# connortannahill/MM-ADMM

Measured on AMD Instinct MI355X. Metric: ADMM iterations/sec on 1M-node 2D mesh; achieved HBM GB/s in SpMV, higher is better.
Workload: dtype f64

## Files before the change

include/mmadmm.h:

```cpp
#ifndef MMADMM_H
#define MMADMM_H
#include <stdint.h>

#ifdef __cplusplus
extern "C" {
#endif

#define MMADMM_OK 0
#define MMADMM_ERR_INVALID 1
#define MMADMM_ERR_HIP 2
#define MMADMM_ERR_INVERTED 3
#define MMADMM_ERR_IO 4
#define MMADMM_ERR_RCCL 5
#define MMADMM_ERR_NOCONV 6
#define MMADMM_ERR_NONFINITE 7

#define MMADMM_BOUNDARY_FREE 0
#define MMADMM_BOUNDARY_FIXED 1
#define MMADMM_INTERIOR 2

typedef struct mmadmm_engine* mmadmm_handle;
typedef struct mmadmm_meshbuf* mmadmm_mesh;

typedef void (*mmadmm_monitor_fn)(int dim, const double* x, double* M_rowmajor, void* user);

typedef struct mmadmm_params {
  double dt;
  double tau;
  double rho;
  int grad_use;
  int device;
  int rank;
  int nranks;
  int partition;
} mmadmm_params;

typedef struct mmadmm_stats {
  long long steps;
  long long admm_iters;
  long long bfgs_iters;
  int max_bfgs;
  double last_primal;
  double last_dual;
  double t_prox_ms;
  double t_xupdate_ms;
  double t_step_ms;
  long long n_prox;
  long long n_xupdate;
  long long n_steps_timed;
  double prox_bytes;
  double xupdate_bytes;
  long long newton_iters;
  long long jacobians;
  long long cg_iters;
  double t_jac_ms;
  double t_solve_ms;
  double t_be_ms;
  long long regrids;
  long long regrid_rows;
  double regrid_gather_bytes;
  long long regrid_cand;
  long long regrid_fallbacks;
  int monitor_iso;
  double t_exchange_ms;
  long long n_exchange;
  double halo_send_bytes;
  double halo_recv_bytes;
  int interior_nodes;
  int overlap;
} mmadmm_stats;

int mmadmm_regrid(mmadmm_handle h, double t);
int mmadmm_set_regrid(mmadmm_handle h, int every_step);

int mmadmm_regrid_values(mmadmm_handle h, const double* M);
int mmadmm_regrid_values_device(mmadmm_handle h, const double* d_M, void* producer_stream);
int mmadmm_regrid_field(mmadmm_handle h, const double* u, double alpha);
int mmadmm_regrid_field_device(mmadmm_handle h, const double* d_u, double alpha, void* producer_stream);
int mmadmm_field_hessian(mmadmm_handle h, const double* u, double* H);
int mmadmm_field_hessian_device(mmadmm_handle h, const double* d_u, double* d_H, void* stream);
int mmadmm_get_device(mmadmm_handle h, const char* what, double* d_out, void* consumer_stream);
int mmadmm_field_monitor(int dim, int nP, const double* Xp, int nF, const int32_t* F, const double* u,
                         double alpha, double* H, double* M);

int mmadmm_regrid_field_huang(mmadmm_handle h, const double* u, double alpha, double* alpha_used);
int mmadmm_regrid_field_huang_device(mmadmm_handle h, const double* d_u, double alpha, void* producer_stream,
                                     double* alpha_used);
int mmadmm_field_solve_info(mmadmm_handle h, int* passes, int* syncs);
int mmadmm_field_monitor_huang(int dim, int nP, const double* Xp, int nF, const int32_t* F, const double* u,
                               double alpha, double* alpha_used, double* H, double* M);
int mmadmm_field_root(int n, int count, const double* d, double* out);

int mmadmm_regrid_fields(mmadmm_handle h, int C, const double* U, const double* w, double alpha);
int mmadmm_regrid_fields_device(mmadmm_handle h, int C, const double* d_U, const double* w, double alpha,
                                void* producer_stream);
int mmadmm_regrid_fields_huang(mmadmm_handle h, int C, const double* U, const double* w, double alpha,
                               double* alpha_used);
int mmadmm_regrid_fields_huang_device(mmadmm_handle h, int C, const double* d_U, const double* w, double alpha,
                                      void* producer_stream, double* alpha_used);
int mmadmm_field_hessians(mmadmm_handle h, int C, const double* U, const double* w, double* H, double* A);
int mmadmm_field_hessians_device(mmadmm_handle h, int C, const double* d_U, const double* w, double* d_H, double* d_A,
                                 void* stream);
int mmadmm_fields_monitor(int dim, int nP, const double* Xp, int nF, const int32_t* F, int C, const double* U,
                          const double* w, double alpha, int normalise, double* alpha_used, double* H, double* A,
                          double* M);

int mmadmm_transfer(mmadmm_handle h, const double* Xold, const double* Xnew, int C, const double* uold, double* unew,
                    int32_t* where, int* counts);
int mmadmm_transfer_device(mmadmm_handle h, const double* d_Xold, const double* d_Xnew, int C, const double* d_uold,
                           double* d_unew, int32_t* d_where, int* counts, void* stream);
int mmadmm_transfer_field(int dim, int nP, const double* Xold, int nF, const int32_t* F, const double* Xnew, int C,
                          const double* uold, double* unew, int32_t* where, int* counts);
int mmadmm_face_neighbours(int dim, int nP, int nF, const int32_t* F, int32_t* nbr);

#define MMADMM_QUALITY_IDENTITY 0
#define MMADMM_QUALITY_VALUES 1
#define MMADMM_QUALITY_LAST 2
int mmadmm_quality(mmadmm_handle h, const double* X, int source, const double* M, double* q, double* summary);
int mmadmm_quality_device(mmadmm_handle h, const double* d_X, int source, const double* d_M, double* d_q,
                          double* summary, void* stream);
int mmadmm_mesh_quality(int dim, int nP, const double* Xp, const double* Xc, int nF, const int32_t* F,
                        const double* Ehat, const double* M, double* q, double* summary);

const char* mmadmm_last_error(void);
int mmadmm_version(void);
int mmadmm_build_info(char* out, int len);

int mmadmm_builtin_monitor(int dim, int mon_type, mmadmm_monitor_fn* fn, void** user);
int mmadmm_monitor_grid(int dim, int nP, const double* Xp, mmadmm_monitor_fn fn, void* user, int* rows,
                        double* vals);

int mmadmm_mesh_reorient(int dim, int nP, const double* Xp, int nF, int32_t* F);

int mmadmm_create(int dim, int nP, const double* Xp, const double* Xc, int nF, const int32_t* F,
                  const int32_t* mask, const mmadmm_params* p, mmadmm_monitor_fn fn, void* user,
                  mmadmm_handle* out);
int mmadmm_step(mmadmm_handle h, int n_iters, double tol, double* Ih, int* admm_iters);
int mmadmm_euler_step(mmadmm_handle h, double* Ih);
int mmadmm_backward_euler_step(mmadmm_handle h, double dt, double tol, double* Ih, int* newton_iters);
int mmadmm_get_jacobian(mmadmm_handle h, long long* nnz, int32_t* ia, int32_t* ja, double* a);
int mmadmm_be_begin(mmadmm_handle h, double dt, double* Ih);
int mmadmm_be_residual(mmadmm_handle h, double dt, double* F, double* norm1, double* Ih);
int mmadmm_be_fsubjac(mmadmm_handle h, double* a);
int mmadmm_be_add(mmadmm_handle h, const double* dx);
int mmadmm_energy(mmadmm_handle h, double* E);
int mmadmm_done(mmadmm_handle h);
int mmadmm_get(mmadmm_handle h, const char* what, double* out);
int mmadmm_get_simplices(mmadmm_handle h, int32_t* F);
int mmadmm_sizes(mmadmm_handle h, int* nP, int* nF, int* grid_rows);
int mmadmm_set_timing(mmadmm_handle h, int on);
int mmadmm_stats_get(mmadmm_handle h, mmadmm_stats* s);
int mmadmm_stats_reset(mmadmm_handle h);
int mmadmm_options_get(mmadmm_handle h, char* buf, int cap);
int mmadmm_sync(mmadmm_handle h);
int mmadmm_destroy(mmadmm_handle h);

int mmadmm_mesh_rect(int dim, int nx, int ny, int nz, double xa, double xb, double ya, double yb,
                     double za, double zb, int btype, mmadmm_mesh* out);
int mmadmm_mesh_levelset2d(int nx, int ny, double xa, double xb, double ya, double yb, int btype,
                           int compact_mask, mmadmm_mesh* out);
int mmadmm_mesh_levelset3d(int nx, int ny, int nz, double xa, double xb, double ya, double yb, double za,
                           double zb, int btype, int compact_mask, mmadmm_mesh* out);
int mmadmm_mesh_shoulder(int dim, int nx, int ny, int nz, double xa, double xb, double ya, double yb, double za,
                         double zb, int btype, mmadmm_mesh* out);
int mmadmm_mesh_reference_points(mmadmm_mesh h, double* Xc);
int mmadmm_mesh_hexdisc(int N, double r, double cx, double cy, int btype, mmadmm_mesh* out);
int mmadmm_mesh_read(int dim, const char* tri, const char* pnts, const char* mask, mmadmm_mesh* out);
int mmadmm_mesh_sizes(mmadmm_mesh m, int* dim, int* nP, int* nF, int* mask_len);
int mmadmm_mesh_copy(mmadmm_mesh m, double* Xp, int32_t* F, int32_t* mask);
int mmadmm_mesh_free(mmadmm_mesh m);
int mmadmm_write_points(const char* path, int dim, int nP, const double* Xp);
int mmadmm_write_simplices(const char* path, int dim, int nF, const int32_t* F);

int mmadmm_debug_blockgrad(mmadmm_handle h, int s, const double* z, const double* dxpu, int flags,
                           double* out);

#define MMADMM_PART_RCB 0
#define MMADMM_PART_RANGES 1
#define MMADMM_UNIQUE_ID_BYTES 128
typedef struct mmadmm_comm_s* mmadmm_comm;
typedef struct mmadmm_plan_s* mmadmm_plan;
int mmadmm_layout_check(unsigned* host_word);
int mmadmm_comm_unique_id(void* out, int len);
int mmadmm_comm_create_rccl(int nranks, int rank, const void* uid, int device, mmadmm_comm* out);
int mmadmm_comm_create_rccl_timeout(int nranks, int rank, const void* uid, int device, double timeout_s,
                                    mmadmm_comm* out);
int mmadmm_comm_create_loopback(int nranks, mmadmm_comm* out);
typedef int (*mmadmm_allgather_fn)(void* user, const double* send, double* recv, long long count);
typedef int (*mmadmm_exchange_fn)(void* user, int npeers, const int* peer_rank, const double* send,
                                  const long long* send_off, const long long* send_count, double* recv,
                                  const long long* recv_off, const long long* recv_count);
int mmadmm_comm_create_host(int nranks, int rank, mmadmm_allgather_fn allgather, mmadmm_exchange_fn exchange,
                            void* user, mmadmm_comm* out);
int mmadmm_comm_destroy(mmadmm_comm c);
int mmadmm_comm_nranks(mmadmm_comm c, int* nranks);
int mmadmm_create_partitioned(int dim, int nP, const double* Xp, const double* Xc, int nF, const int32_t* F,
                              const int32_t* mask, const mmadmm_params* p, mmadmm_monitor_fn fn, void* user,
                              mmadmm_comm comm, mmadmm_handle* out);
int mmadmm_local_nodes(mmadmm_handle h, int* n_local, int32_t* global_ids);
int mmadmm_plan_create(int dim, int nP, const double* Xp, int nF, const int32_t* F, int nranks, int rank, int method,
                       mmadmm_plan* out);
int mmadmm_plan_sizes(mmadmm_plan h, int* nLocalNodes, int* nLocalSimplices, int* nSources, int* nSend, int* nRecv,
                      int* nPeers, int* nInterface);
int mmadmm_plan_get(mmadmm_plan h, int32_t* localNodes, int32_t* localSimplices, int32_t* incPtr, int32_t* incSrc,
                    int32_t* sendOff, int32_t* peers);
int mmadmm_plan_destroy(mmadmm_plan h);

int mmadmm_devmath(int op, int n, const double* in, double* out);

#ifdef __cplusplus
}
#endif
#endif
```

mm-admm_amd/csrc/host/engine.cpp:

```cpp
#include <algorithm>
#include <chrono>
#include <cmath>
#include <cstring>
#include <limits>
#include <memory>
#include <mutex>
#include <string>
#include <vector>

#include "../../../include/mmx_sparse.h"
#include "../kernels/admm_kernels.h"
#include "../kernels/field_kernels.h"
#include "../kernels/quality_kernels.h"
#include "../kernels/regrid_kernels.h"
#include "../kernels/transfer_kernels.h"
#include "comm.h"
#include "common.h"
#include "partition.h"
#include "transfer.h"
#include "xup_records.h"

#define MMX_SP(expr)                                                                     \
  do {                                                                                   \
    const int rc_ = (expr);                                                              \
    if (rc_ != MMADMM_OK) throw ::mmx::Error(rc_, std::string(#expr) + ": " + mmadmm_last_error()); \
  } while (0)

namespace mmx {

namespace {
thread_local std::string g_last_error;
}
void set_last_error(const std::string& msg) { g_last_error = msg; }


struct EngineBase {
  virtual ~EngineBase() = default;
  int dim = 2;
  virtual void step(int nIters, double tol, double* Ih, int* iters) = 0;
  virtual double eulerStep() = 0;
  virtual double backwardEulerStep(double dt, double tol, int* newton) = 0;
  virtual void jacobian(long long* nnz, int32_t* ia, int32_t* ja, double* a) = 0;
  virtual void newtonOp(int op, double dt, const double* in, double* out, double* sc) = 0;
  virtual double energy() = 0;
  virtual void done() = 0;
  virtual void get(const std::string& what, double* out) = 0;
  virtual void getSimplices(int32_t* F) = 0;
  virtual void localNodes(int* n, int32_t* ids) = 0;
  virtual void sizes(int* nP, int* nF, int* gridRows) = 0;
  virtual void setTiming(bool on) = 0;
  virtual void stats(mmadmm_stats* s) = 0;
  virtual void resetStats() = 0;
  virtual void sync() = 0;
  virtual void regrid(double t) = 0;
  virtual void setRegrid(bool on) = 0;
  virtual void regridFrom(int src, const double* p, bool onDevice, double alpha, void* stream) = 0;
  virtual void fieldHessian(const double* u, double* H, bool onDevice, void* stream) = 0;
  virtual void regridFromFields(int src, const double* U, int C, const double* w, bool onDevice, double alpha,
                                void* stream) = 0;
  virtual void fieldHessians(const double* U, int C, const double* w, double* H, double* A, bool onDevice,
                             void* stream) = 0;
  virtual double fieldAlphaUsed() const = 0;
  virtual void fieldSolveInfo(int* passes, int* syncs) const = 0;
  virtual void getDevice(const std::string& what, double* dOut, void* stream) = 0;
  virtual void transfer(const double* Xold, const double* Xnew, int C, const double* uold, double* unew, int32_t* where,
                        int* counts, bool onDevice, void* stream) = 0;
  virtual void quality(const double* X, int source, const double* M, double* q, double* summary, bool onDevice,
                       void* stream) = 0;
  virtual void debugBlockGrad(int s, const double* z, const double* dx, int flags, double* out) = 0;
  virtual std::string options() const = 0;
};

enum MonSource {
  kMonBuiltin7 = 0,
  kMonCallback = 1,
  kMonValues = 2,
  kMonField = 3,
  kMonFieldHuang = 4,
  kMonFields = 5,
  kMonFieldsHuang = 6
};

void reorient_simplices(int D, const double* Vp, int nF, int32_t* F) {
  for (int s = 0; s < nF; ++s) {
    double E[3][3] = {{0}};
    const int32_t* f = F + (size_t)s * (D + 1);
    for (int j = 0; j < D; ++j)
      for (int r = 0; r < D; ++r) E[r][j] = Vp[(size_t)f[j + 1] * D + r] - Vp[(size_t)f[0] * D + r];
    double det;
    if (D == 2) {
      det = E[0][0] * E[1][1] - E[1][0] * E[0][1];
    } else {
      const double h0 = E[0][0] * (E[1][1] * E[2][2] - E[1][2] * E[2][1]);
      const double h1 = E[0][1] * (E[1][0] * E[2][2] - E[1][2] * E[2][0]);
      const double h2 = E[0][2] * (E[1][0] * E[2][1] - E[1][1] * E[2][0]);
      det = h0 - h1 + h2;
    }
    if (det < 0) std::swap(F[(size_t)s * (D + 1) + 1], F[(size_t)s * (D + 1) + 2]);
  }
}

template <int D>
class Engine final : public EngineBase {
 public:
  static constexpr int K = D * (D + 1);

  Engine(int nP, const double* Xp, const double* Xc, int nF, const int32_t* F, const int32_t* mask,
         const mmadmm_params& p, mmadmm_monitor_fn fn, void* user, Comm* comm)
      : Fh_(orientedSimplices(nP, Xp, nF, F)),
        plan_(make_partition_plan(D, nP, Xp, nF, Fh_.data(), std::max(1, p.nranks), p.nranks > 1 ? p.rank : 0,
                                  p.partition)),
        knobs_(EngineKnobs::from_env(D, (int)plan_.localSimplices.size(), std::max(1, p.nranks))) {
    dim = D;
    prm_ = p;
    nranks_ = std::max(1, p.nranks);
    rank_ = nranks_ > 1 ? p.rank : 0;
    comm_ = comm;
    nP_ = (int)plan_.localNodes.size();
    nF_ = (int)plan_.localSimplices.size();
    maxBlocks_ = std::max<size_t>(4096, std::max((nF_ + 15) / 16, (nP_ + 255) / 256 + 16));
    knobs_.check_xup_sweep(maxBlocks_);
    if (nranks_ > 1 && !comm_) throw Error(MMADMM_ERR_INVALID, "partitioned engine needs a communicator");
    if (p.device >= 0) MMX_HIP(hipSetDevice(p.device));
    MMX_HIP(hipStreamCreateWithFlags(&st_, hipStreamNonBlocking));
    if (nranks_ > 1) {
      MMX_HIP(hipStreamCreateWithFlags(&st2_, hipStreamNonBlocking));
      MMX_HIP(hipEventCreateWithFlags(&evProx_, hipEventDisableTiming));
      MMX_HIP(hipEventCreateWithFlags(&evEx_, hipEventDisableTiming));
    }
    compMesh_ = (Xc != nullptr);
    std::vector<double> Vp(Xp, Xp + (size_t)nP * D);
    maskH_.assign(mask, mask + nP);
    build_monitor_grid(D, Vp.data(), nP, fn, user, grid_);
    monFn_ = fn;
    monUser_ = user;
    const double w = 0.5 * sqrt(p.rho);
    w_ = w;
    double Ehat[3][3] = {{0}};
    if (D == 2) {
      Ehat[0][0] = 1.0;
      Ehat[1][0] = 0.0;
      Ehat[0][1] = 1.0 / 2.0;
      Ehat[1][1] = sqrt(3) / 2.0;
    } else {
      const double v[3][3] = {{-2.0, 0.0, -2.0}, {0.0, -2.0, -2.0}, {-2.0, -2.0, 0.0}};
      for (int r = 0; r < 3; ++r)
        for (int c = 0; c < 3; ++c) Ehat[r][c] = v[r][c];
    }
    const double dFact = (D == 2) ? 2.0 : 6.0;
    const double s1 = pow((dFact / std::abs(hostDet(Ehat))), 1.0 / ((double)D));
    for (int r = 0; r < D; ++r)
      for (int c = 0; c < D; ++c) Ehat[r][c] *= s1;
    const double s2 = (double)pow(nF, 1.0 / D);
    for (int r = 0; r < D; ++r)
      for (int c = 0; c < D; ++c) Ehat[r][c] /= s2;
    for (int r = 0; r < D; ++r)
      for (int c = 0; c < D; ++c) EhatH_[r * D + c] = Ehat[r][c];
    const double d = (double)D, pp = 1.5;
    powd_ = pow(d, d * pp / 2.0);
    if (nranks_ > 1) {
      std::vector<std::vector<int>> owned(nranks_);
      for (int v = 0; v < nP; ++v) owned[plan_.nodeOwner[v]].push_back(v);
      size_t mx = 1;
      for (auto& o : owned) mx = std::max(mx, o.size());
      maxOwned_ = (int)mx;
      std::vector<int> all((size_t)nranks_ * mx, -1), mine;
      for (int q = 0; q < nranks_; ++q) std::copy(owned[q].begin(), owned[q].end(), all.begin() + (size_t)q * mx);
      for (int v : owned[rank_])
        mine.push_back((int)(std::lower_bound(plan_.localNodes.begin(), plan_.localNodes.end(), v) - plan_.localNodes.begin()));
      nOwned_ = (int)mine.size();
      ownAllGid_.upload(all.data(), all.size(), st_);
      ownAllGidH_ = all;
      ownLocal_.upload(mine.data(), std::max<size_t>(mine.size(), 1), st_);
      streamWait();
    }
    const int nl = nP_;
    std::vector<double> invdiag(nl);
    const double dtsq = p.dt * p.dt;
    for (int v = 0; v < nl; ++v) {
      double S = 0.0;
      for (int c = 0; c < plan_.valence[v]; ++c) S = (c == 0) ? (w * w) * 1.0 : S + (w * w) * 1.0;
      invdiag[v] = 1.0 / (p.tau + dtsq * S);
    }
    std::vector<uint8_t> sbits(nF_), interior(nl);
    for (int v = 0; v < nl; ++v) interior[v] = maskH_[plan_.localNodes[v]] == MMADMM_INTERIOR ? 1 : 0;
    for (int s = 0; s < nF_; ++s) {
      unsigned b = 0;
      for (int n = 0; n < D + 1; ++n) {
        const int t = maskH_[plan_.localNodes[plan_.Flocal[(size_t)s * (D + 1) + n]]];
        if (t == MMADMM_BOUNDARY_FIXED) b |= 1u << n;
        if (t != MMADMM_INTERIOR) b |= 1u << (4 + n);
      }
      sbits[s] = (uint8_t)b;
    }
    std::vector<double> Vl((size_t)nl * D), Vcl;
    for (int v = 0; v < nl; ++v)
      for (int c = 0; c < D; ++c) Vl[(size_t)v * D + c] = Vp[(size_t)plan_.localNodes[v] * D + c];
    if (compMesh_) {
      Vcl.resize((size_t)nl * D);
      for (int v = 0; v < nl; ++v)
        for (int c = 0; c < D; ++c) Vcl[(size_t)v * D + c] = Xc[(size_t)plan_.localNodes[v] * D + c];
    }
    F_.upload(plan_.Flocal.data(), plan_.Flocal.size(), st_);
    sbits_.upload(sbits.data(), sbits.size(), st_);
    interior_.upload(interior.data(), interior.size(), st_);
    incPtr_.upload(plan_.incPtr.data(), plan_.incPtr.size(), st_);
    incOff_.upload(plan_.incSrc.data(), plan_.incSrc.size(), st_);
    if (knobs_.tslot) tslot_.alloc(std::max<size_t>((size_t)nF_ * K, 1));
    {
      std::vector<long long> key(nl);
      for (int v = 0; v < nl; ++v) {
        long long k = (long long)nF_;
        for (int t = plan_.incPtr[v]; t < plan_.incPtr[v + 1]; ++t)
          if (plan_.incSrc[t] >= 0) k = std::min<long long>(k, plan_.incSrc[t] / K);
        key[v] = k;
      }
      std::vector<int32_t> inner, bound;
      for (int v = 0; v < nl; ++v) {
        bool remote = false;
        for (int t = plan_.incPtr[v]; t < plan_.incPtr[v + 1]; ++t) remote |= plan_.incSrc[t] < 0;
        (remote && knobs_.overlap ? bound : inner).push_back(v);
      }
      nInner_ = (int)inner.size();
      const bool slabs = knobs_.xupOrder;
      auto order = [&](std::vector<int32_t>& ord) {
        const int n = (int)ord.size();
        if (slabs) {
          const int n8 = ((n + 255) / 256 + 7) / 8 * 256;
          std::stable_sort(ord.begin(), ord.end(), [&](int a, int b) { return Vl[(size_t)a * D + 1] < Vl[(size_t)b * D + 1]; });
          for (int c = 0; c < 8; ++c) {
            const int lo = std::min(n, c * n8), hi = std::min(n, (c + 1) * n8);
            std::stable_sort(ord.begin() + lo, ord.begin() + hi, [&](int a, int b) { return key[a] < key[b]; });
          }
        } else {
          std::stable_sort(ord.begin(), ord.end(), [&](int a, int b) { return key[a] < key[b]; });
        }
      };
      order(inner);
      order(bound);
      std::vector<int32_t> ord(inner);
      ord.insert(ord.end(), bound.begin(), bound.end());
      nodeOrder_.upload(ord.data(), std::max<size_t>(ord.size(), 1), st_);
      XupRecords recs;
      if (knobs_.xupRec) {
        const int ch = std::max(D == 2 ? MMX_XU_CH2D : 8, knobs_.xupCh);
        recs = build_xup_records(nl, ord.data(), plan_.incPtr.data(), plan_.incSrc.data(), invdiag.data(), ch);
        xrec_.upload(recs.rec.data(), recs.rec.size(), st_);
        xinv_.upload(recs.invdiag.data(), recs.invdiag.size(), st_);
        xslot_.upload(recs.slot.data(), recs.slot.size(), st_);
        xslotStride_ = (int)recs.stride;
        xslotCh_ = ch;
        const int chs = D == 2 ? MMX_XU_CH2D : knobs_.xupCh;
        xupTail_ = 0;
        for (int v = 0; v < nl; ++v) xupTail_ += std::max(0, plan_.incPtr[v + 1] - plan_.incPtr[v] - chs);
      }
      streamWait();
    }
    invdiag_.upload(invdiag.data(), invdiag.size(), st_);
    if (compMesh_) Vc_.upload(Vcl.data(), Vcl.size(), st_);
    uploadGridCoords();
    gvals_.upload(grid_.vals.data(), grid_.vals.size(), st_);
    if (D == 3) {
      gpad_.alloc(gvals_.n / 9 * 10);
      launch_pad_rows(gvals_.p, (long long)(gvals_.n / 9), gpad_.p, st_);
    }
    updateIso();
    Vp_.upload(Vl.data(), Vl.size(), st_);
    x_.upload(Vl.data(), Vl.size(), st_);
    xPrev_.upload(Vl.data(), Vl.size(), st_);
    xBar_.upload(Vl.data(), Vl.size(), st_);
    if (nranks_ > 1) {
      expOff_.upload(plan_.sendOff.data(), std::max<size_t>(plan_.sendOff.size(), 1), st_);
      export_.alloc((size_t)std::max<size_t>(plan_.sendOff.size(), 1) * D);
      remote_.alloc((size_t)std::max(plan_.recvRows, 1) * D);
    }
    z_.alloc((size_t)nF_ * K * (kZUInterleaved ? 2 : 1));
    gcache_.alloc((size_t)nF_ * K);
    tieList_.alloc((size_t)nF_ / 16 + 1);
    tieCount_.alloc(3);
    MMX_HIP(hipMemsetAsync(tieCount_.p, 0, 3 * sizeof(unsigned), st_));
    if (!kZUInterleaved) u_.alloc((size_t)nF_ * K);
    gs_.alloc((size_t)nF_ * K);
    clearU();
    {
      const size_t nB = (size_t)((nF_ + 255) / 256) * 256 * K * K;
      B_.alloc(nB);
      MMX_HIP(hipMemsetAsync(B_.p, 0, nB * sizeof(double), st_));
      launch_bkinv_identity<D>(nF_, B_.p, st_);
      if (prox_double_buffered(D, knobs_.prox2dWave)) B2_.alloc(nB);
    }
    partA_.alloc(maxBlocks_ * kNumPartials);
    partB_.alloc(maxBlocks_ * kNumPartials);
    redScratch_.alloc((size_t)kRedSets * kRedSplit * kNumPartials);
    red_.scratch = redScratch_.p;
    red_.splitMin = knobs_.redSplitMin;
    resultsCap_ = 0;
    ensureResults(64);
    m_ = makeView();
    launch_gather_z<D>(m_, x_.p, z_.p, st_);
    streamWait();
    MMX_HIP(hipGetLastError());
  }

  ~Engine() override {
    if (rgHost_) (void)hipHostFree(rgHost_);
    if (fldStH_) (void)hipHostFree(fldStH_);
    if (qlRecH_) (void)hipHostFree(qlRecH_);
    if (rgnHost_) (void)hipHostFree(rgnHost_);
    if (jac_) (void)mmx_matrix_destroy(jac_);
    for (auto& e : evPool_) (void)hipEventDestroy(e);
    if (evSync_) (void)hipEventDestroy(evSync_);
    if (evIn_) (void)hipEventDestroy(evIn_);
    if (evOut_) (void)hipEventDestroy(evOut_);
    if (resH_) (void)hipHostFree(resH_);
    if (evProx_) (void)hipEventDestroy(evProx_);
    if (evEx_) (void)hipEventDestroy(evEx_);
    for (hipStream_t s : {st2_, st_})
      if (s) {
        staging_forget(s);
        (void)hipStreamDestroy(s);
      }
  }

  void step(int nIters, double tol, double* Ih, int* itersOut) override {
    if (nIters < 1) throw Error(MMADMM_ERR_INVALID, "step: nIters must be >= 1");
    if (regridEachStep_) regrid(stepsTaken_ * prm_.dt);
    ensureResults(nIters);
    const bool timing = timing_;
    hipEvent_t eStep0 = nullptr, eStep1 = nullptr;
    if (timing) {
      eStep0 = nextEvent();
      MMX_HIP(hipEventRecord(eStep0, st_));
    }
    const double dtOverTau = prm_.dt / prm_.tau;
    const bool fusePred = knobs_.zx && knobs_.fusePred && !knobs_.prox2dWave && !(prm_.grad_use || stepsTaken_ <= 2);
    if (prm_.grad_use || stepsTaken_ <= 2) {
      int nb = 0;
      launch_grad_simplex<D>(m_, x_.p, gs_.p, true, partA_.p, &nb, st_);
      exchange(1);
      launch_predict<D>(m_, knobs_, 0, gs_.p, x_.p, xPrev_.p, xBar_.p, dtOverTau, st_);
    } else if (!fusePred) {
      launch_predict<D>(m_, knobs_, 1, nullptr, x_.p, xPrev_.p, xBar_.p, dtOverTau, st_);
    }
    const double* zsrc = stepsTaken_ == 0 ? xPrev_.p : xBar_.p;
    const bool zFromX = knobs_.zx && !knobs_.prox2dWave;
    if (!stepTaken_) clearU();
    if (zFromX)
      m_.zx = zsrc;
    else
      launch_gather_z<D>(m_, zsrc, z_.p, st_);
    gcacheValid_ = false;
    if (!zFromX) m_.zx = nullptr;
    StepScalars sc{prm_.tau, prm_.dt * prm_.dt, w_, dtOverTau};
    int nbx = 0, nbp = 0;
    if (fusePred) {
      m_.predPrev = xPrev_.p;
      m_.predBar = xBar_.p;
    }
    PackZX pz;
    if (zFromX) {
      pz.F = F_.p;
      pz.zx = zsrc;
      if (fusePred) {
        pz.x = x_.p;
        pz.xPrev = xPrev_.p;
      }
    }
    xupdateHalo(sc, &nbx, false, false, pz);
    m_.predPrev = m_.predBar = nullptr;
    const bool early = tol >= 0;
    int done = 0;
    double primal = 0, dual = 0;
    const bool deferRed = !early && nIters <= kDeferMax;
    const size_t slice = maxBlocks_ * kNumPartials;
    if (deferRed && partA_.n < slice * nIters) partA_.alloc(slice * std::max(nIters, 10));
    int firstDeferred = 0;
    hipEvent_t prevEnd = nullptr;
    for (int i = 0; i < nIters; ++i) {
      hipEvent_t a0 = nullptr, a1 = nullptr, b1 = nullptr;
      if (timing) {
        a0 = prevEnd;
        if (!a0) {
          a0 = nextEvent();
          MMX_HIP(hipEventRecord(a0, st_));
        }
      }
      const bool firstProx = !hessComputed_;
      const bool swapB = prox_double_buffered(D, knobs_.prox2dWave) && hessComputed_;
      if (hessComputed_) {
        tiePar_ ^= 1;
        std::swap(m_.tieCount, m_.tieStale);
      }
      m_.gcSkip = (D == 2 && knobs_.gcSkip && !early && i == nIters - 1) ? 1 : 0;
      launch_prox<D>(m_, knobs_, !hessComputed_, gcacheValid_, early ? tol / 100 : 1e-3 / 100, x_.p, z_.p, uPtr(), B_.p,
                     swapB ? B2_.p : B_.p, partA_.p + (deferRed ? slice * i : 0), &nbp, st_);
      m_.zx = nullptr;
      if (swapB) std::swap(B_.p, B2_.p);
      gcacheValid_ = !m_.gcSkip;
      if (timing) {
        a1 = nextEvent();
        MMX_HIP(hipEventRecord(a1, st_));
      }
      hessComputed_ = true;
      stepTaken_ = true;
      const bool resid = early || i == nIters - 1;
      xupdateHalo(sc, &nbx, resid, true, PackZX{});
      if (timing) {
        b1 = nextEvent();
        MMX_HIP(hipEventRecord(b1, st_));
        timed_.push_back({a0, a1, b1});
      }
      prevEnd = b1;
      if (deferRed) {
        if (firstProx && i < nIters - 1) {
          prevEnd = nullptr;
          launch_reduce_partials(partA_.p + slice * i, nbp, res_ + (size_t)i * 2 * kNumPartials, st_, red_);
          firstDeferred = i + 1;
        } else if (i == nIters - 1) {
          const int i0 = firstProx ? i : firstDeferred;
          launch_reduce_steps(partA_.p + slice * i0, slice, nbp, partB_.p, nbx, nIters - i0,
                              res_ + (size_t)i0 * 2 * kNumPartials, st_, red_);
        }
      } else if (resid) {
        prevEnd = nullptr;
        launch_reduce_partials2(partA_.p, nbp, res_ + (size_t)i * 2 * kNumPartials, partB_.p, nbx,
                                res_ + (size_t)i * 2 * kNumPartials + kNumPartials, st_, red_);
      } else {
        prevEnd = nullptr;
        launch_reduce_partials(partA_.p, nbp, res_ + (size_t)i * 2 * kNumPartials, st_, red_);
      }
      done = i + 1;
      if (early) {
        std::vector<double> rv;
        fetchResults(res_ + (size_t)i * 2 * kNumPartials, 1, rv);
        const double* r = rv.data();
        primal = sqrt(r[kNumPartials + 2]);
        dual = sqrt(r[1]);
        if (r[4] > 0 || (primal < tol && dual < tol)) break;
      }
    }
    MMX_HIP(hipMemcpyAsync(Vp_.p, x_.p, (size_t)nP_ * D * sizeof(double), hipMemcpyDeviceToDevice, st_));
    vpVersion_++;
    if (timing) {
      eStep1 = nextEvent();
      MMX_HIP(hipEventRecord(eStep1, st_));
    }
    fetchResults(res_, done, hostRes_);
    MMX_HIP(hipGetLastError());
    bool bad = false;
    long long bf = 0;
    int mx = 0;
    for (int i = 0; i < done; ++i) {
      const double* r = &hostRes_[(size_t)i * 2 * kNumPartials];
      bad |= r[4] > 0;
      bf += (long long)r[3];
      mx = std::max(mx, (int)r[5]);
    }
#ifdef MMX_HINT_PROBE
    {
      double hits = 0;
      for (int i = 0; i < done; ++i) hits += hostRes_[(size_t)i * 2 * kNumPartials + 2];
      fprintf(stderr, "[hint-probe] step %lld: %.0f hits of %.0f lookups in %d proxes\n", (long long)stepsTaken_, hits,
              3.0 * nF_ * done, done);
    }
#endif
    const double* last = &hostRes_[(size_t)(done - 1) * 2 * kNumPartials];
    primal = sqrt(last[kNumPartials + 2]);
    dual = sqrt(last[1]);
    st_stats_.admm_iters += done;
    st_stats_.bfgs_iters += bf;
    st_stats_.max_bfgs = mx;
    st_stats_.last_primal = primal;
    st_stats_.last_dual = dual;
    st_stats_.steps += 1;
    if (timing) {
      stepEv_.push_back({eStep0, eStep1});
      if (evUsed_ >= kEvResolve) resolveTimed();
    }
    stepsTaken_++;
    if (bad) throwBad("in prox");
    if (Ih) *Ih = hostRes_[0];
    if (itersOut) *itersOut = done;
  }

  double eulerStep() override {
    clearInvFlag();
    int nb = 0;
    launch_grad_simplex<D>(m_, x_.p, gs_.p, false, partA_.p, &nb, st_);
    launch_reduce_partials(partA_.p, nb, res_, st_, red_);
    exchange(1);
    launch_euler_apply<D>(m_, knobs_, gs_.p, x_.p, prm_.dt / prm_.tau, st_);
    std::vector<double> rv;
    fetchResults(res_, 1, rv);
    const double* r = rv.data();
    if (r[4] > 0) throwBad("in the explicit Euler gradient");
    return r[0];
  }

  double backwardEulerStep(double dtBE, double tol, int* newtonOut) override {
    if (nranks_ > 1) throw Error(MMADMM_ERR_INVALID, "backward Euler runs on one rank (no element partition)");
    const auto tStep = Clock::now();
    const int n = nP_ * D;
    ensureJacobian();
    const double dtot = dtBE / prm_.tau;
    const double SAFETY_FAC = 1.0 / 10.0;
    const int MAX_ITERS = 1000;
    clearInvFlag();
    MMX_HIP(hipMemcpyAsync(xn_.p, x_.p, (size_t)n * sizeof(double), hipMemcpyDeviceToDevice, st_));
    int nb = 0, nb2 = 0;
    launch_grad_simplex<D>(m_, x_.p, gs_.p, false, partA_.p, &nb, st_);
    launch_euler_apply<D>(m_, knobs_, gs_.p, x_.p, dtot, st_);
    if (!beStepTaken_) buildJacobian(dtBE);
    int nIter = 0;
    double Ih = 0.0, normPrev = INFINITY;
    std::vector<double> rv;
    void* mst = nullptr;
    MMX_SP(mmx_matrix_stream(jac_, &mst));
    do {
      launch_grad_simplex<D>(m_, x_.p, gs_.p, false, partA_.p, &nb, st_);
      launch_be_residual<D>(m_, knobs_, gs_.p, x_.p, xn_.p, dtot, rhs_.p, partB_.p, &nb2, st_);
      launch_reduce_partials2(partA_.p, nb, res_, partB_.p, nb2, res_ + kNumPartials, st_, red_);
      fetchResults(res_, 1, rv);
      if (rv[4] > 0) throwBad("in backward Euler");
      Ih = rv[0];
      const double norm = rv[kNumPartials];
      if (norm < SAFETY_FAC * tol) break;
      if (!beStepTaken_ || std::fabs(norm - normPrev) / norm < 0.25) {
        buildJacobian(dtBE);
        beStepTaken_ = true;
      }
      waitStream();
      const auto tSolve = Clock::now();
      MMX_SP(mmx_matrix_set_rhs_device(jac_, rhs_.p));
      int cgIter = 0;
      MMX_SP(mmx_matrix_solve_device(jac_, &jprm_, dx_.p, &cgIter, 0));
      st_stats_.t_solve_ms += msSince(tSolve);
      if (cgIter > 0) st_stats_.cg_iters += cgIter;
      if (cgIter <= 0)
        throw Error(MMADMM_ERR_NOCONV, "backward Euler: CG-STAB did not converge (reference: assert(cgIter > 0))");
      launch_add_inplace(n, x_.p, dx_.p, st_);
      nIter++;
      normPrev = norm;
    } while (nIter < MAX_ITERS);
    streamWait();
    st_stats_.steps += 1;
    st_stats_.newton_iters += nIter;
    st_stats_.t_be_ms += msSince(tStep);
    if (newtonOut) *newtonOut = nIter;
    return Ih;
  }

  void newtonOp(int op, double dt, const double* in, double* out, double* sc) override {
    if (nranks_ > 1) throw Error(MMADMM_ERR_INVALID, "backward Euler runs on one rank (no element partition)");
    ensureJacobian();
    const int n = nP_ * D;
    std::vector<double> rv;
    int nb = 0, nb2 = 0;
    if (op == 0 || op == 1) clearInvFlag();
    if (op == 0) {
      MMX_HIP(hipMemcpyAsync(xn_.p, x_.p, (size_t)n * sizeof(double), hipMemcpyDeviceToDevice, st_));
      launch_grad_simplex<D>(m_, x_.p, gs_.p, false, partA_.p, &nb, st_);
      launch_reduce_partials(partA_.p, nb, res_, st_, red_);
      launch_euler_apply<D>(m_, knobs_, gs_.p, x_.p, dt / prm_.tau, st_);
      fetchResults(res_, 1, rv);
      if (rv[4] > 0) throwBad("in backward Euler");
      if (sc) sc[0] = rv[0];
    } else if (op == 1) {
      launch_grad_simplex<D>(m_, x_.p, gs_.p, false, partA_.p, &nb, st_);
      launch_be_residual<D>(m_, knobs_, gs_.p, x_.p, xn_.p, dt / prm_.tau, rhs_.p, partB_.p, &nb2, st_);
      launch_reduce_partials2(partA_.p, nb, res_, partB_.p, nb2, res_ + kNumPartials, st_, red_);
      fetchResults(res_, 1, rv);
      if (rv[4] > 0) throwBad("in backward Euler");
      std::vector<double> r((size_t)n);
      MMX_HIP(hipMemcpyAsync(r.data(), rhs_.p, (size_t)n * sizeof(double), hipMemcpyDeviceToHost, st_));
      streamWait();
      for (int i = 0; i < n; ++i) out[i] = -r[i];
      if (sc) {
        sc[0] = rv[0];
        sc[1] = rv[kNumPartials];
      }
    } else if (op == 2) {
      const double h = 10.0 * sqrt(std::numeric_limits<double>::epsilon());
      launch_fd_jac<D>(m_, Vp_.p, h, dv_.p, st_, fdWork_.p);
      clearInvFlag();
      if (jraw_.n != jja_.n) jraw_.alloc(std::max<size_t>(jja_.n, 1));
      launch_jac_assemble<D>(m_, knobs_, jia_.p, jja_.p, dv_.p, 1.0, jraw_.p, st_, false, maxColNodes_);
      MMX_HIP(hipMemcpyAsync(out, jraw_.p, jja_.n * sizeof(double), hipMemcpyDeviceToHost, st_));
      streamWait();
    } else if (op == 3) {
      MMX_HIP(hipMemcpyAsync(dx_.p, in, (size_t)n * sizeof(double), hipMemcpyHostToDevice, st_));
      launch_add_inplace(n, x_.p, dx_.p, st_);
      streamWait();
    } else {
      throw Error(MMADMM_ERR_INVALID, "newtonOp: unknown op");
    }
  }

  void jacobian(long long* nnz, int32_t* ia, int32_t* ja, double* a) override {
    if (!jac_) throw Error(MMADMM_ERR_INVALID, "no Jacobian yet: run a backward Euler step first");
    if (nnz) *nnz = (long long)jja_.n;
    if (ia) MMX_HIP(hipMemcpyAsync(ia, jia_.p, jia_.n * sizeof(int32_t), hipMemcpyDeviceToHost, st_));
    if (ja) MMX_HIP(hipMemcpyAsync(ja, jja_.p, jja_.n * sizeof(int32_t), hipMemcpyDeviceToHost, st_));
    if (a) MMX_HIP(hipMemcpyAsync(a, jval_.p, jval_.n * sizeof(double), hipMemcpyDeviceToHost, st_));
    streamWait();
  }

  double energy() override {
    int nb = 0;
    launch_energy<D>(m_, Vp_.p, partA_.p, &nb, st_);
    clearInvFlag();
    launch_reduce_partials(partA_.p, nb, res_, st_, red_);
    std::vector<double> rv;
    fetchResults(res_, 1, rv);
    return rv[0];
  }

  void done() override {
    MMX_HIP(hipMemcpyAsync(Vp_.p, x_.p, (size_t)nP_ * D * sizeof(double), hipMemcpyDeviceToDevice, st_));
    vpVersion_++;
    streamWait();
  }

  void get(const std::string& what, double* out) override {
    const DevBuf<double>* b = nullptr;
    if (what == "x") b = &x_;
    else if (what == "xPrev") b = &xPrev_;
    else if (what == "xBar") b = &xBar_;
    else if (what == "z" || what == "u") {
      if (!kZUInterleaved) {
        b = what == "z" ? &z_ : &u_;
      } else {
        std::vector<double> h(z_.n);
        MMX_HIP(hipMemcpyAsync(h.data(), z_.p, z_.n * sizeof(double), hipMemcpyDeviceToHost, st_));
        streamWait();
        const int sh = what == "u" ? D : 0;
        for (int s = 0; s < nF_; ++s)
          for (int i = 0; i < K; ++i) out[(size_t)s * K + i] = h[(size_t)s * 2 * K + (i / D) * 2 * D + i % D + sh];
        return;
      }
    }
    else if (what == "points") b = &Vp_;
    else if (what == "hess") b = &B_;
    else if (what == "gs") b = &gs_;
    else if (what == "grid") {
      if (gridOnDevice_) {
        MMX_HIP(hipMemcpyAsync(out, gvals_.p, gvals_.n * sizeof(double), hipMemcpyDeviceToHost, st_));
        streamWait();
      } else {
        std::memcpy(out, grid_.vals.data(), grid_.vals.size() * sizeof(double));
      }
      return;
    } else if (what == "Ehat") {
      std::memcpy(out, EhatH_, D * D * sizeof(double));
      return;
    } else {
      throw Error(MMADMM_ERR_INVALID, "mmadmm_get: unknown field '" + what + "'");
    }
    if (b == &B_) {
      std::vector<double> h(b->n);
      MMX_HIP(hipMemcpyAsync(h.data(), b->p, b->n * sizeof(double), hipMemcpyDeviceToHost, st_));
      streamWait();
      for (int s = 0; s < nF_; ++s)
        for (int ij = 0; ij < K * K; ++ij) out[(size_t)s * K * K + ij] = h[bIndex(s, ij)];
      return;
    }
    MMX_HIP(hipMemcpyAsync(out, b->p, b->n * sizeof(double), hipMemcpyDeviceToHost, st_));
    streamWait();
  }

  static size_t bIndex(int s, int ij) {
    if (D == 3 && MMX_B3_PAIRS) return ((size_t)(s >> 6) * K * K + (ij & ~1)) * 64 + 2 * (s & 63) + (ij & 1);
    return ((size_t)(s >> 6) * K * K + ij) * 64 + (s & 63);
  }

  void getSimplices(int32_t* F) override {
    for (size_t i = 0; i < plan_.Flocal.size(); ++i) F[i] = plan_.localNodes[plan_.Flocal[i]];
  }

  void localNodes(int* n, int32_t* ids) override {
    if (n) *n = nP_;
    if (ids) std::memcpy(ids, plan_.localNodes.data(), plan_.localNodes.size() * sizeof(int32_t));
  }

  void sizes(int* nP, int* nF, int* gridRows) override {
    if (nP) *nP = nP_;
    if (nF) *nF = nF_;
    if (gridRows) *gridRows = (int)(grid_.vals.size() / (D * D));
  }

  void setTiming(bool on) override {
    resolveTimed();
    timing_ = on;
  }

  void stats(mmadmm_stats* s) override {
    resolveTimed();
    *s = st_stats_;
    const double nF = nF_, nP = nP_;
    const double ts = knobs_.tslot ? 1.0 : 0.0;
    s->prox_bytes = nF * (4.0 * (D + 1) + 1 + 8.0 * (2 * K + K * K) * 2 + 8.0 * K * 2 + ts * 8.0 * K) +
                    nP * 8.0 * D;
    const double ch = D == 2 ? MMX_XU_CH2D : knobs_.xupCh;
    const double fixed = knobs_.xupRec ? nP * (4.0 * kXupRecInts + 8.0 + 4.0 * ch) + 4.0 * (double)xupTail_
                                 : 4.0 * (nP + 1) + 4.0 * (D + 1) * nF + 8.0 * nP;
    s->xupdate_bytes = fixed + (16.0 - 8.0 * ts) * K * nF + 8.0 * D * nP * 2;
    s->monitor_iso = iso_ ? 1 : 0;
    s->halo_send_bytes = 8.0 * D * (double)plan_.sendOff.size();
    s->halo_recv_bytes = nranks_ > 1 ? 8.0 * D * (double)plan_.recvRows : 0.0;
    s->interior_nodes = nInner_;
    s->overlap = knobs_.overlap;
  }

  std::string options() const override { return knobs_.text(); }

  void resetStats() override {
    resolveTimed();
    const mmadmm_stats z{};
    st_stats_ = z;
  }

  void resolveTimed() {
    if (stepEv_.empty() && timed_.empty() && exEv_.empty()) return;
    streamWait();
    float ms = 0;
    for (auto& p : stepEv_) {
      MMX_HIP(hipEventElapsedTime(&ms, p.first, p.second));
      st_stats_.t_step_ms += ms;
      st_stats_.n_steps_timed += 1;
    }
    if (st2_) MMX_HIP(hipStreamSynchronize(st2_));
    for (auto& p : exEv_) {
      MMX_HIP(hipEventElapsedTime(&ms, p.first, p.second));
      st_stats_.t_exchange_ms += ms;
      st_stats_.n_exchange += 1;
    }
    exEv_.clear();
    for (auto& t : timed_) {
      MMX_HIP(hipEventElapsedTime(&ms, t.a0, t.a1));
      st_stats_.t_prox_ms += ms;
      st_stats_.n_prox += 1;
      MMX_HIP(hipEventElapsedTime(&ms, t.a1, t.b1));
      st_stats_.t_xupdate_ms += ms;
      st_stats_.n_xupdate += 1;
    }
    stepEv_.clear();
    timed_.clear();
    evUsed_ = 0;
  }

  void sync() override { streamWait(); }

  void debugBlockGrad(int s, const double* z, const double* dx, int flags, double* out) override {
    if (s < 0 || s >= nF_) throw Error(MMADMM_ERR_INVALID, "debug_blockgrad: simplex out of range");
    DevBuf<double> dz, ddx, dout;
    dz.upload(z, K, st_);
    ddx.upload(dx, K, st_);
    dout.alloc(K + 2);
    launch_debug_blockgrad<D>(m_, s, dz.p, ddx.p, dout.p, flags, st_);
    MMX_HIP(hipMemcpyAsync(out, dout.p, (K + 2) * sizeof(double), hipMemcpyDeviceToHost, st_));
    streamWait();
  }

 private:
  struct Timed {
    hipEvent_t a0, a1, b1;
  };

  void profMark(const char* what, std::chrono::steady_clock::time_point& t) const {
    if (!knobs_.schedProf) return;
    const auto now = std::chrono::steady_clock::now();
    fprintf(stderr, "[sched] engine %s %.3f s\n", what, std::chrono::duration<double>(now - t).count());
    t = now;
  }
  void ensureJacobian() {
    if (jac_) return;
    auto tp = std::chrono::steady_clock::now();
    const int n = nP_ * D;
    mmx_struc sp = nullptr;
    MMX_SP(mmx_struc_create(n, 0, &sp));
    std::vector<int32_t> ia(n + 1), ja;
    long long nnz = 0;
    int rc = mmx_struc_mesh_pattern(sp, D, (int)(Fh_.size() / (D + 1)), Fh_.data());
    if (rc == MMADMM_OK) rc = mmx_struc_pack(sp);
    if (rc == MMADMM_OK) rc = mmx_struc_get(sp, nullptr, &nnz, nullptr, nullptr);
    if (rc == MMADMM_OK) {
      ja.resize(nnz);
      rc = mmx_struc_get(sp, nullptr, &nnz, ia.data(), ja.data());
    }
    profMark("pattern", tp);
    int dev = prm_.device;
    if (dev < 0) MMX_HIP(hipGetDevice(&dev));
    if (rc == MMADMM_OK) rc = mmx_matrix_create_from_struc(dev, sp, &jac_);
    (void)mmx_struc_destroy(sp);
    profMark("matrix create", tp);
    if (rc != MMADMM_OK) throw Error(rc, std::string("backward Euler Jacobian: ") + mmadmm_last_error());
    mmx_param_iter_mesh(&jprm_);
    maxColNodes_ = 0;
    for (int r = 0; r < n; ++r) maxColNodes_ = std::max(maxColNodes_, (ia[r + 1] - ia[r]) / D);
    jia_.upload(ia.data(), ia.size(), st_);
    jja_.upload(ja.data(), ja.size(), st_);
    jval_.alloc(std::max<size_t>(nnz, 1));
    dv_.alloc(std::max<size_t>((size_t)nF_ * (D + 1) * D * K, 1));
    if (knobs_.fdjFast) fdWork_.alloc((size_t)nF_ * (D + 1) + 1);
    xn_.alloc((size_t)n);
    rhs_.alloc((size_t)n);
    dx_.alloc((size_t)n);
    streamWait();
  }

  void buildJacobian(double dtBE) {
    if (jacVp_ == vpVersion_ && jacDt_ == dtBE) return;
    jacVp_ = vpVersion_;
    jacDt_ = dtBE;
    const auto t0 = Clock::now();
    auto tp = t0;
    const double h = 10.0 * sqrt(std::numeric_limits<double>::epsilon());
    launch_fd_jac<D>(m_, Vp_.p, h, dv_.p, st_, fdWork_.p);
    clearInvFlag();
    launch_jac_assemble<D>(m_, knobs_, jia_.p, jja_.p, dv_.p, dtBE / prm_.tau, jval_.p, st_, true, maxColNodes_);
    streamWait();
    profMark("FD Jacobian + assembly", tp);
    MMX_SP(mmx_matrix_set_values_device(jac_, jval_.p));
    if (!jacFactored_) {
      MMX_SP(mmx_matrix_sfac(jac_, &jprm_));
      jacFactored_ = true;
      profMark("sfac", tp);
    }
    streamWait();
    st_stats_.jacobians += 1;
    st_stats_.t_jac_ms += msSince(t0);
  }
  using Clock = std::chrono::steady_clock;
  static double msSince(Clock::time_point t) {
    return std::chrono::duration<double, std::milli>(Clock::now() - t).count();
  }

  static double hostDet(const double (&a)[3][3]) {
    if (D == 2) return a[0][0] * a[1][1] - a[1][0] * a[0][1];
    const double h0 = a[0][0] * (a[1][1] * a[2][2] - a[1][2] * a[2][1]);
    const double h1 = a[0][1] * (a[1][0] * a[2][2] - a[1][2] * a[2][0]);
    const double h2 = a[0][2] * (a[1][0] * a[2][1] - a[1][1] * a[2][0]);
    return h0 - h1 + h2;
  }

  void exchange(int mode, const PackZX& pz = {}, hipStream_t st = nullptr) {
    if (nranks_ == 1) return;
    if (!st) st = st_;
    hipEvent_t e0 = nullptr, e1 = nullptr;
    if (timing_ && mode == 0) {
      e0 = nextEvent();
      MMX_HIP(hipEventRecord(e0, st));
    }
    launch_pack_export<D>(mode, (int)plan_.sendOff.size(), expOff_.p, z_.p, uPtr(), gs_.p, w_, export_.p, st, pz);
    comm_->exchange(rank_, export_.p, remote_.p, plan_.peers, D, st);
    if (e0) {
      e1 = nextEvent();
      MMX_HIP(hipEventRecord(e1, st));
      exEv_.push_back({e0, e1});
    }
  }

  void xupdateHalo(const StepScalars& sc, int* nbx, bool resid, bool useTs, const PackZX& pz) {
    if (!knobs_.overlap) {
      exchange(0, pz);
      launch_xupdate<D>(m_, knobs_, sc, xBar_.p, z_.p, uPtr(), x_.p, partB_.p, nbx, resid, st_, useTs);
      return;
    }
    MMX_HIP(hipEventRecord(evProx_, st_));
    DeviceMesh<D> mi = m_;
    mi.xupHi = nInner_;
    int nb1 = 0, nb2 = 0;
    launch_xupdate<D>(mi, knobs_, sc, xBar_.p, z_.p, uPtr(), x_.p, partB_.p, &nb1, resid, st_, useTs);
    MMX_HIP(hipStreamWaitEvent(st2_, evProx_, 0));
    exchange(0, pz, st2_);
    MMX_HIP(hipEventRecord(evEx_, st2_));
    MMX_HIP(hipStreamWaitEvent(st_, evEx_, 0));
    DeviceMesh<D> mb = m_;
    mb.xupLo = nInner_;
    launch_xupdate<D>(mb, knobs_, sc, xBar_.p, z_.p, uPtr(), x_.p, partB_.p + (size_t)nb1 * kNumPartials, &nb2, resid,
                      st_, useTs);
    *nbx = nb1 + nb2;
  }

  void waitStream() {
    if (!knobs_.spin) {
      streamWait();
      return;
    }
    if (!evSync_) MMX_HIP(hipEventCreateWithFlags(&evSync_, hipEventDisableTiming));
    MMX_HIP(hipEventRecord(evSync_, st_));
    hipError_t r;
    while ((r = hipEventQuery(evSync_)) == hipErrorNotReady) __builtin_ia32_pause();
    MMX_HIP(r);
  }

  void streamWait() {
    if (nranks_ > 1 && comm_)
      comm_->wait(st_);
    else
      MMX_HIP(hipStreamSynchronize(st_));
  }

  void fetchResults(const double* dev, int rows, std::vector<double>& out) {
    const size_t cnt = (size_t)rows * 2 * kNumPartials;
    out.resize(cnt);
    if (resH_) {
      waitStream();
      std::memcpy(out.data(), resH_ + (dev - res_), cnt * sizeof(double));
      return;
    }
    if (nranks_ == 1) {
      MMX_HIP(hipMemcpyAsync(out.data(), dev, cnt * sizeof(double), hipMemcpyDeviceToHost, st_));
      streamWait();
      return;
    }
    if (resAll_.n < cnt * nranks_) resAll_.alloc(cnt * nranks_);
    comm_->allgather(rank_, dev, resAll_.p, cnt, st_);
    std::vector<double> all(cnt * nranks_);
    MMX_HIP(hipMemcpyAsync(all.data(), resAll_.p, all.size() * sizeof(double), hipMemcpyDeviceToHost, st_));
    streamWait();
    for (size_t i = 0; i < cnt; ++i) {
      const bool isMax = (i % kNumPartials) == 5;
      double v = all[i];
      for (int q = 1; q < nranks_; ++q) v = isMax ? std::max(v, all[(size_t)q * cnt + i]) : v + all[(size_t)q * cnt + i];
      out[i] = v;
    }
  }

  void setRegrid(bool on) override { regridEachStep_ = on; }

  void regrid(double t) override {
    if (nranks_ > 1) {
      const bool all = knobs_.regridGatherAll;
      if (!all && regridNear(t)) return;
      st_stats_.regrid_fallbacks += all ? 0 : 1;
    }
    regridAll(t);
  }

  void afterProducer(void* stream) {
    if (!stream) return;
    if (!evIn_) MMX_HIP(hipEventCreateWithFlags(&evIn_, hipEventDisableTiming));
    MMX_HIP(hipEventRecord(evIn_, (hipStream_t)stream));
    MMX_HIP(hipStreamWaitEvent(st_, evIn_, 0));
  }
  void beforeConsumer(void* stream) {
    if (!stream) {
      streamWait();
      return;
    }
    if (!evOut_) MMX_HIP(hipEventCreateWithFlags(&evOut_, hipEventDisableTiming));
    MMX_HIP(hipEventRecord(evOut_, st_));
    MMX_HIP(hipStreamWaitEvent((hipStream_t)stream, evOut_, 0));
  }
  void singleRankOnly(const char* what) const {
    if (nranks_ > 1) throw Error(MMADMM_ERR_INVALID, std::string(what) + ": single rank only (no element partition)");
  }
  void fieldScratch() {
    if (fldE_.p) return;
    fldE_.alloc(std::max<size_t>(field_ebuf_doubles<D>(nF_), 1));
    fldG_.alloc((size_t)nP_ * D);
  }
  void fieldsScratch(int C) {
    fieldScratch();
    if (fldGP_.n < (size_t)C * nP_ * D) fldGP_.alloc((size_t)C * nP_ * D);
  }
  void huangScratch() {
    if (fldA_.p) return;
    fldA_.alloc((size_t)nP_ * D * D);
    fldL_.alloc((size_t)nP_ * (D + 1));
    fldPart_.alloc((size_t)2 * field_solve_blocks(nP_));
    fldSt_.alloc(1);
    MMX_HIP(hipHostMalloc((void**)&fldStH_, sizeof(FieldSolve), hipHostMallocDefault));
  }
  void fieldHuangMonitor(const double* X) {
    fieldScratch();
    huangScratch();
    launch_field_huang_recover<D>(X, srcPtr_, F_.p, nF_, incPtr_.p, incOff_.p, nodeOrder_.p, nP_, fldE_.p, fldG_.p,
                                  fldA_.p, fldL_.p, st_);
    huangSolveAndFinish();
  }
  void fieldsHuangMonitor(const double* X) {
    fieldsScratch(srcC_);
    huangScratch();
    launch_fields_recover<D>(X, srcPtr_, srcC_, srcW_.data(), F_.p, nF_, incPtr_.p, incOff_.p, nodeOrder_.p, nP_,
                             fldE_.p, fldGP_.p, nullptr, fldA_.p, kFieldsHuang, 1.0, fldL_.p, st_);
    huangSolveAndFinish();
  }
  void huangSolveAndFinish() {
    launch_field_solve_set(fldSt_.p, srcAlpha_, st_);
    fldAlphaUsed_ = srcAlpha_;
    fldPasses_ = fldSyncs_ = 0;
    if (!(srcAlpha_ > 0.0)) {
      do {
        launch_field_solve_passes<D>(fldL_.p, nP_, fldSt_.p, fldPart_.p, kFieldBatch, st_);
        MMX_HIP(hipGetLastError());
        MMX_HIP(hipMemcpyAsync(fldStH_, fldSt_.p, sizeof(FieldSolve), hipMemcpyDeviceToHost, st_));
        streamWait();
        fldSyncs_++;
      } while (fldStH_->phase != kFieldDone);
      fldAlphaUsed_ = fldStH_->alpha;
      fldPasses_ = fldStH_->passes;
    }
    launch_field_huang_final<D>(fldA_.p, fldL_.p, nP_, fldSt_.p, rgMon_.p, st_);
  }
  double fieldAlphaUsed() const override { return fldAlphaUsed_; }
  void fieldSolveInfo(int* passes, int* syncs) const override {
    if (passes) *passes = fldPasses_;
    if (syncs) *syncs = fldSyncs_;
  }

  void regridFrom(int src, const double* p, bool onDevice, double alpha, void* stream) override {
    singleRankOnly(src == kMonFieldHuang ? "mmadmm_regrid_field_huang"
                   : src == kMonField    ? "mmadmm_regrid_field"
                                         : "mmadmm_regrid_values");
    const size_t n = (size_t)nP_ * (src == kMonValues ? D * D : 1);
    if (!onDevice) {
      if (fldIn_.n < n) fldIn_.alloc(n);
      MMX_HIP(hipMemcpyAsync(fldIn_.p, p, n * sizeof(double), hipMemcpyHostToDevice, st_));
      streamWait();
      p = fldIn_.p;
    } else {
      afterProducer(stream);
    }
    srcPtr_ = p;
    srcAlpha_ = alpha;
    regridAll(0.0, (MonSource)src);
    srcPtr_ = nullptr;
    if (onDevice && !knobs_.iso) streamWait();
  }

  void regridFromFields(int src, const double* U, int C, const double* w, bool onDevice, double alpha,
                        void* stream) override {
    singleRankOnly(src == kMonFieldsHuang ? "mmadmm_regrid_fields_huang" : "mmadmm_regrid_fields");
    const size_t n = (size_t)nP_ * C;
    if (!onDevice) {
      if (fldIn_.n < n) fldIn_.alloc(n);
      MMX_HIP(hipMemcpyAsync(fldIn_.p, U, n * sizeof(double), hipMemcpyHostToDevice, st_));
      streamWait();
      U = fldIn_.p;
    } else {
      afterProducer(stream);
    }
    srcPtr_ = U;
    srcAlpha_ = alpha;
    srcC_ = C;
    srcW_.assign(w, w + C);
    regridAll(0.0, (MonSource)src);
    srcPtr_ = nullptr;
    if (onDevice && !knobs_.iso) streamWait();
  }

  void fieldHessians(const double* U, int C, const double* w, double* H, double* A, bool onDevice,
// ... 448 lines not shown
    const int nbe = part ? std::max(1, std::min(256, (nF_ + 255) / 256)) : 0;
    double* extPart = rgPart_.p + (size_t)512 * 2 * D;
    if (part) {
      launch_rows_gather(D, ownLocal_.p, nOwned_, Vp_.p, rgSend_.p, st_);
      comm_->allgather(rank_, rgSend_.p, rgRecv_.p, (size_t)maxOwned_ * D, st_);
      launch_rows_scatter(D, ownAllGid_.p, nranks_ * maxOwned_, rgRecv_.p, rgXg_.p, st_);
      X = rgXg_.p;
      launch_bbox<D>(Vp_.p, nP_, rgPart_.p + (size_t)256 * 2 * D, nbl, st_);
      launch_extent<D>(Vp_.p, F_.p, nF_, extPart, nbe, st_);
    }
    launch_bbox<D>(X, nG, rgPart_.p, nb, st_);
    MMX_HIP(hipMemcpyAsync(rgHost_, rgPart_.p, sizeof(double) * nb * 2 * D, hipMemcpyDeviceToHost, st_));
    if (part) {
      MMX_HIP(hipMemcpyAsync(rgHost_ + (size_t)256 * 2 * D, rgPart_.p + (size_t)256 * 2 * D, sizeof(double) * nbl * 2 * D,
                             hipMemcpyDeviceToHost, st_));
      MMX_HIP(hipMemcpyAsync(rgHost_ + (size_t)512 * 2 * D, extPart, sizeof(double) * nbe * D, hipMemcpyDeviceToHost,
                             st_));
    }
    streamWait();
    double lo[3] = {INFINITY, INFINITY, INFINITY}, hi[3] = {-INFINITY, -INFINITY, -INFINITY};
    double llo[3] = {INFINITY, INFINITY, INFINITY}, lhi[3] = {-INFINITY, -INFINITY, -INFINITY};
    for (int b = 0; b < nb; ++b)
      for (int d = 0; d < D; ++d) {
        lo[d] = std::min(lo[d], rgHost_[(size_t)b * 2 * D + d]);
        hi[d] = std::max(hi[d], rgHost_[(size_t)b * 2 * D + D + d]);
      }
    for (int b = 0; b < nbl; ++b)
      for (int d = 0; d < D; ++d) {
        llo[d] = std::min(llo[d], rgHost_[(size_t)(256 + b) * 2 * D + d]);
        lhi[d] = std::max(lhi[d], rgHost_[(size_t)(256 + b) * 2 * D + D + d]);
      }
    if (part) {
      for (int d = 0; d < D; ++d) extMax_[d] = 0.0;
      for (int b = 0; b < nbe; ++b)
        for (int d = 0; d < D; ++d) extMax_[d] = std::max(extMax_[d], rgHost_[(size_t)512 * 2 * D + (size_t)b * D + d]);
    }
    grid_geometry(D, nG, lo, hi, grid_);
    uploadGridCoords();
    CellGrid cg{};
    const int gn[3] = {grid_.nx, grid_.ny, grid_.nz};
    cg.hmin = INFINITY;
    for (int d = 0; d < 3; ++d) {
      const double ext = d < D ? hi[d] - lo[d] : 0.0;
      cg.lo[d] = d < D ? lo[d] : 0.0;
      cg.n[d] = (d < D && ext > 0) ? std::max(1, gn[d] / 2) : 1;
      cg.inv[d] = (d < D && ext > 0) ? cg.n[d] / ext : 0.0;
      if (d < D && ext > 0) cg.hmin = std::min(cg.hmin, ext / cg.n[d]);
    }
    if (!(cg.hmin < INFINITY)) cg.hmin = 0.0;
    const int ncell = cg.n[0] * cg.n[1] * cg.n[2];
    if ((int)rgStarts_.n < ncell + 1) {
      rgCounts_.alloc(ncell + 1);
      rgStarts_.alloc(ncell + 1);
      rgFill_.alloc(ncell);
      rgScanBytes_ = bin_scan_bytes(ncell);
      rgScan_.alloc(std::max<size_t>(rgScanBytes_, 1));
    }
    launch_bin<D>(X, nG, cg, rgCellOf_.p, rgCounts_.p, rgStarts_.p, rgFill_.p, rgNodes_.p, rgScan_.p, rgScanBytes_,
                  st_);
    if (src == kMonCallback && builtin_monitor_kind(monFn_, monUser_) == 7) src = kMonBuiltin7;
    if (src == kMonValues) {
      MMX_HIP(hipMemcpyAsync(rgMon_.p, srcPtr_, (size_t)nG * DD * sizeof(double), hipMemcpyDeviceToDevice, st_));
    } else if (src == kMonField) {
      fieldScratch();
      launch_field_hessian<D>(X, srcPtr_, F_.p, nF_, incPtr_.p, incOff_.p, nodeOrder_.p, nP_, fldE_.p, fldG_.p,
                              srcAlpha_, nullptr, rgMon_.p, st_);
    } else if (src == kMonFieldHuang) {
      fieldHuangMonitor(X);
    } else if (src == kMonFields) {
      fieldsScratch(srcC_);
      launch_fields_recover<D>(X, srcPtr_, srcC_, srcW_.data(), F_.p, nF_, incPtr_.p, incOff_.p, nodeOrder_.p, nP_,
                               fldE_.p, fldGP_.p, nullptr, rgMon_.p, kFieldsPlain, srcAlpha_, nullptr, st_);
    } else if (src == kMonFieldsHuang) {
      fieldsHuangMonitor(X);
    } else if (src == kMonBuiltin7) {
      double c[3];
      moving_bump_centre(t, c);
      launch_monitor_tv<D>(X, nG, c, rgMon_.p, st_);
    } else {
      std::vector<double> Xh((size_t)nG * D), mv((size_t)nG * DD);
      MMX_HIP(hipMemcpyAsync(Xh.data(), X, Xh.size() * sizeof(double), hipMemcpyDeviceToHost, st_));
      streamWait();
      for (int v = 0; v < nG; ++v) {
        double M[9];
        for (int i = 0; i < DD; ++i) M[i] = 0.0;
        monFn_(D, &Xh[(size_t)v * D], M, monUser_);
        std::memcpy(&mv[(size_t)v * DD], M, DD * sizeof(double));
      }
      MMX_HIP(hipMemcpyAsync(rgMon_.p, mv.data(), mv.size() * sizeof(double), hipMemcpyHostToDevice, st_));
      streamWait();
    }
    const int passes = (D == 2) ? 5 : 2;
    const int gn3[3] = {grid_.nx, grid_.ny, D == 3 ? grid_.nz : 0};
    GridBox R{{0, 0, 0}, {gn3[0], gn3[1], gn3[2]}};
    if (part) {
      for (int d = 0; d < D; ++d) {
        const std::vector<double>& g = d == 0 ? grid_.gx : d == 1 ? grid_.gy : grid_.gz;
        const double h = g[1] - g[0];
        const int M = (int)std::ceil(2.0 * extMax_[d] / h) + 2;
        R.lo[d] = std::max(0, std::min(gn3[d], (int)std::floor((llo[d] - g[0]) / h) - M));
        R.hi[d] = std::max(0, std::min(gn3[d], (int)std::floor((lhi[d] - g[0]) / h) + 1 + M));
      }
    }
    auto widen = [&](const GridBox& b, int w) {
      GridBox o = b;
      for (int d = 0; d < D; ++d) {
        o.lo[d] = std::max(0, b.lo[d] - w);
        o.hi[d] = std::min(gn3[d], b.hi[d] + w);
      }
      return o;
    };
    const GridBox H = widen(R, part ? passes : 0);
    launch_nn_fill<D>(X, cg, rgStarts_.p, rgNodes_.p, gx_.p, gy_.p, D == 3 ? gz_.p : gy_.p, grid_.nx, grid_.ny,
                      grid_.nz, rgMon_.p, rgTmp_.p, H, st_);
    double* cur = rgTmp_.p;
    double* oth = part ? rgTmp2_.p : gvals_.p;
    for (int it = 0; it < passes; ++it) {
      launch_smooth<D>(cur, oth, grid_.nx, grid_.ny, grid_.nz, widen(R, part ? passes - 1 - it : 0), st_);
      std::swap(cur, oth);
    }
    if (part) {
      launch_box_commit<D>(cur, gvals_.p, D == 3 ? gpad_.p : nullptr, grid_.nx, grid_.ny, grid_.nz, R, st_);
    } else {
      if (cur != gvals_.p)
        MMX_HIP(hipMemcpyAsync(gvals_.p, cur, gvals_.n * sizeof(double), hipMemcpyDeviceToDevice, st_));
      if (D == 3) launch_pad_rows(gvals_.p, (long long)(gvals_.n / 9), gpad_.p, st_);
    }
    st_stats_.regrid_rows = (long long)(H.hi[0] - H.lo[0] + 1) * (H.hi[1] - H.lo[1] + 1) * (H.hi[2] - H.lo[2] + 1);
    st_stats_.regrid_gather_bytes = part ? (double)nranks_ * maxOwned_ * D * sizeof(double) : 0.0;
    st_stats_.regrid_cand = part ? nG : 0;
    MMX_HIP(hipGetLastError());
    gridOnDevice_ = true;
    updateIso();
    m_ = makeView();
    st_stats_.regrids += 1;
  }

  DeviceMesh<D> makeView() const {
    DeviceMesh<D> m{};
    m.nP = nP_;
    m.nF = nF_;
    m.F = F_.p;
    m.sbits = sbits_.p;
    m.nodeInterior = interior_.p;
    m.inc_ptr = incPtr_.p;
    m.inc_off = incOff_.p;
    m.remote = nranks_ > 1 ? remote_.p : nullptr;
    m.tslot = knobs_.tslot ? tslot_.p : nullptr;
    m.gcache = gcache_.p;
    m.tieList = tieList_.p;
    m.tieCount = tieCount_.p + tiePar_;
    m.tieStale = tieCount_.p + (tiePar_ ^ 1);
    m.invFlag = tieCount_.p + 2;
    m.nodeOrder = nodeOrder_.p;
    m.xupLo = 0;
    m.xupHi = nP_;
    m.prox2dWave = knobs_.prox2dWave;
    m.xupSweep = knobs_.xupSweep;
    m.xupCh = knobs_.xupCh;
    m.xupEarly = knobs_.xupEarly;
    m.forceTie = knobs_.forceTie;
    m.monHint = knobs_.monHint;
    if (knobs_.xupRec) {
      m.xrec = xrec_.p;
      m.xinv = xinv_.p;
      m.xslot = xslot_.p;
      m.xslotStride = xslotStride_;
      m.xslotCh = xslotCh_;
    }
    m.invdiag = invdiag_.p;
    m.Vc = compMesh_ ? Vc_.p : nullptr;
    m.gx = gx_.p;
    m.gy = gy_.p;
    m.gz = (D == 3) ? gz_.p : gy_.p;
    m.gvals = gvals_.p;
    m.gpad = (D == 3) ? gpad_.p : nullptr;
    for (int a = 0; a < 3; ++a) m.gcell[a] = (D == 3) ? gcell_[a].p : nullptr;
    m.giso = iso_ ? giso_.p : nullptr;
    m.gnx = grid_.nx;
    m.gny = grid_.ny;
    m.gnz = grid_.nz;
    m.ghx = grid_.gx[1] - grid_.gx[0];
    m.ghy = grid_.gy[1] - grid_.gy[0];
    m.ghz = (D == 3) ? grid_.gz[1] - grid_.gz[0] : 1.0;
    m.grhx = 1.0 / m.ghx;
    m.grhy = 1.0 / m.ghy;
    m.grhz = 1.0 / m.ghz;
    const int ns[3] = {grid_.nx, grid_.ny, grid_.nz};
    double* A[3] = {&m.gax, &m.gay, &m.gaz};
    double* SP[3] = {&m.gspx, &m.gspy, &m.gspz};
    double* NS[3] = {&m.gnsx, &m.gnsy, &m.gnsz};
    double* RNS[3] = {&m.grnsx, &m.grnsy, &m.grnsz};
    for (int d = 0; d < 3; ++d) {
      const bool on = d < D;
      *A[d] = on ? grid_.lo[d] : 0.0;
      *SP[d] = on ? grid_.hi[d] - grid_.lo[d] : 0.0;
      *NS[d] = on ? (double)ns[d] : 1.0;
      *RNS[d] = 1.0 / *NS[d];
    }
    for (int i = 0; i < D * D; ++i) m.Ehat[i] = EhatH_[i];
    m.powd = powd_;
    m.w = w_;
    m.compMesh = compMesh_ ? 1 : 0;
    return m;
  }

  void ensureResults(int nIters) {
    if (nIters <= resultsCap_) return;
    resultsCap_ = std::max(nIters, 64);
    const size_t n = (size_t)resultsCap_ * 2 * kNumPartials;
    if (nranks_ == 1 && knobs_.spin) {
      if (resH_) MMX_HIP(hipHostFree(resH_));
      resH_ = nullptr;
      MMX_HIP(hipHostMalloc((void**)&resH_, n * sizeof(double), hipHostMallocMapped));
      MMX_HIP(hipHostGetDevicePointer((void**)&res_, resH_, 0));
    } else {
      results_.alloc(n);
      res_ = results_.p;
    }
  }

  void clearInvFlag() { MMX_HIP(hipMemsetAsync(tieCount_.p + 2, 0, sizeof(unsigned), st_)); }

  [[noreturn]] void throwBad(const char* where) {
    unsigned flag = 0;
    MMX_HIP(hipMemcpyAsync(&flag, tieCount_.p + 2, sizeof(unsigned), hipMemcpyDeviceToHost, st_));
    streamWait();
    if (flag) {
      MMX_HIP(hipMemsetAsync(tieCount_.p + 2, 0, sizeof(unsigned), st_));
      streamWait();
      throw Error(MMADMM_ERR_INVERTED, std::string("inverted element ") + where + " (reference: assert(Edet > 0))");
    }
    if (nranks_ > 1 && regridEachStep_)
      throw Error(MMADMM_ERR_NONFINITE, std::string("non-finite energy ") + where +
                                            ": a monitor evaluation left this rank's regrid box (no element inverted)");
    throw Error(MMADMM_ERR_NONFINITE, std::string("non-finite energy ") + where +
                                          " without an inverted element (a monitor value that is not finite)");
  }

  hipEvent_t nextEvent() {
    if (evUsed_ == evPool_.size()) {
      hipEvent_t e;
      MMX_HIP(hipEventCreateWithFlags(&e, hipEventDisableSystemFence));
      evPool_.push_back(e);
    }
    return evPool_[evUsed_++];
  }

  static std::vector<int32_t> orientedSimplices(int nP, const double* Xp, int nF, const int32_t* F) {
    std::vector<int32_t> Fh(F, F + (size_t)nF * (D + 1));
    for (int32_t v : Fh)
      if (v < 0 || v >= nP) throw Error(MMADMM_ERR_INVALID, "simplex vertex id out of range");
    reorient_simplices(D, Xp, nF, Fh.data());
    return Fh;
  }

  std::vector<int32_t> Fh_;
  PartitionPlan plan_;
  const EngineKnobs knobs_;
  int nP_ = 0, nF_ = 0;
  mmadmm_params prm_{};
  bool compMesh_ = false;
  double w_ = 0, powd_ = 0;
  double EhatH_[9] = {0};
  std::vector<int32_t> maskH_;
  HostGrid grid_;
  mmadmm_monitor_fn monFn_ = nullptr;
  void* monUser_ = nullptr;
  bool regridEachStep_ = false, gridOnDevice_ = false;
  DevBuf<double> rgPart_, rgMon_, rgTmp_, rgTmp2_, rgXg_, rgSend_, rgRecv_;
  DevBuf<double> fldE_, fldG_, fldIn_, fldOut_;
  DevBuf<double> fldGP_;
  int srcC_ = 1;
  std::vector<double> srcW_;
  static constexpr int kFieldBatch = 64;
  DevBuf<double> fldA_, fldL_, fldPart_;
  DevBuf<FieldSolve> fldSt_;
  FieldSolve* fldStH_ = nullptr;
  double fldAlphaUsed_ = 1.0;
  int fldPasses_ = 0, fldSyncs_ = 0;
  std::vector<int32_t> trNbrH_;
  DevBuf<int32_t> trNbr_, trWhere_, trCnt_;
  DevBuf<double> trStage_;
  DevBuf<double> qlE_, qlC_, qlPart_, qlRec_, qlStage_;
  double* qlRecH_ = nullptr;
  const double* srcPtr_ = nullptr;
  double srcAlpha_ = 1.0;
  hipEvent_t evIn_ = nullptr, evOut_ = nullptr;
  double extMax_[3] = {0.0, 0.0, 0.0};
  DevBuf<int> ownLocal_, ownAllGid_;
  std::vector<int> ownAllGidH_, ownGidH_;
  DevBuf<double> rgnPart_, rgnSmallS_, rgnSmallR_, rgnSbox_, rgnSend_, rgnRecv_, rgnCandX_, rgnMon_;
  DevBuf<int> rgnCnt_, rgnGid_, rgnOwnGid_, rgnCandGid_, rgnCellOf_, rgnNodes_;
  double* rgnHost_ = nullptr;
  int nOwned_ = 0, maxOwned_ = 1;
  DevBuf<int> rgCellOf_, rgNodes_, rgCounts_, rgStarts_, rgFill_;
  DevBuf<unsigned char> rgScan_;
  size_t rgScanBytes_ = 0;
  double* rgHost_ = nullptr;
  hipStream_t st_ = nullptr;
  hipStream_t st2_ = nullptr;
  hipEvent_t evProx_ = nullptr, evEx_ = nullptr;
  int nInner_ = 0;
  std::vector<std::pair<hipEvent_t, hipEvent_t>> exEv_;
  DevBuf<int32_t> F_, incPtr_, incOff_;
  DevBuf<double> tslot_;
  DevBuf<uint8_t> sbits_, interior_;
  DevBuf<double> gcell_[3];
  DevBuf<double> giso_;
  DevBuf<int> isoFlag_;
  bool iso_ = false;
  std::vector<double> gcellH_[3];
  DevBuf<double> invdiag_, Vc_, gx_, gy_, gz_, gvals_, Vp_, x_, xPrev_, xBar_, z_, u_, gs_, B_, B2_, gcache_, gpad_;
  DevBuf<double> partA_, partB_, results_, export_, remote_, resAll_, redScratch_;
  RedWork red_;
  DevBuf<int32_t> expOff_, tieList_, nodeOrder_;
  DevBuf<int32_t> xrec_, xslot_;
  DevBuf<double> xinv_;
  int xslotStride_ = 0, xslotCh_ = 0;
  long long xupTail_ = 0;
  DevBuf<unsigned> tieCount_;
  int tiePar_ = 0;
  Comm* comm_ = nullptr;
  int rank_ = 0, nranks_ = 1;
  int resultsCap_ = 0;
  std::vector<double> hostRes_;
  DeviceMesh<D> m_{};
  bool hessComputed_ = false, stepTaken_ = false, gcacheValid_ = false;
  mmx_matrix jac_ = nullptr;
  mmx_param_iter jprm_{};
  bool beStepTaken_ = false, jacFactored_ = false;
  long long vpVersion_ = 0, jacVp_ = -1;
  double jacDt_ = 0.0;
  DevBuf<int32_t> jia_, jja_;
  DevBuf<double> jval_, jraw_, dv_, xn_, rhs_, dx_;
  DevBuf<unsigned> fdWork_;
  int maxColNodes_ = 65;
  int stepsTaken_ = 0;
  size_t maxBlocks_ = 1;
  static constexpr int kDeferMax = 64;
  bool timing_ = false;
  std::vector<hipEvent_t> evPool_;
  size_t evUsed_ = 0;
  static constexpr bool kZUInterleaved = (D == 2) && MMX_ZU_INTER;
  double* uPtr() const { return kZUInterleaved ? z_.p + D : u_.p; }
  void clearU() {
    if (kZUInterleaved)
      MMX_HIP(hipMemsetAsync(z_.p, 0, z_.n * sizeof(double), st_));
    else
      MMX_HIP(hipMemsetAsync(u_.p, 0, u_.n * sizeof(double), st_));
  }
  double* res_ = nullptr;
  double* resH_ = nullptr;
  hipEvent_t evSync_ = nullptr;
  std::vector<Timed> timed_;
  std::vector<std::pair<hipEvent_t, hipEvent_t>> stepEv_;
  static constexpr size_t kEvResolve = 4096;
  mmadmm_stats st_stats_{};
};

}

using mmx::EngineBase;
using mmx::Error;
using mmx::guarded;

struct mmadmm_engine {
  std::unique_ptr<EngineBase> e;
};

static EngineBase& eng(mmadmm_handle h) {
  if (!h || !h->e) throw Error(MMADMM_ERR_INVALID, "null engine handle");
  return *h->e;
}

extern "C" {

const char* mmadmm_last_error(void) { return mmx::g_last_error.c_str(); }
int mmadmm_version(void) { return 100; }

int mmadmm_mesh_reorient(int dim, int nP, const double* Xp, int nF, int32_t* F) {
  return guarded([&] {
    if ((dim != 2 && dim != 3) || nP < 1 || nF < 0 || !Xp || (nF > 0 && !F))
      throw Error(MMADMM_ERR_INVALID, "mmadmm_mesh_reorient: bad arguments");
    for (long long i = 0; i < (long long)nF * (dim + 1); ++i)
      if (F[i] < 0 || F[i] >= nP) throw Error(MMADMM_ERR_INVALID, "simplex vertex id out of range");
    mmx::reorient_simplices(dim, Xp, nF, F);
  });
}

int mmadmm_create(int dim, int nP, const double* Xp, const double* Xc, int nF, const int32_t* F, const int32_t* mask,
                  const mmadmm_params* p, mmadmm_monitor_fn fn, void* user, mmadmm_handle* out) {
  return guarded([&] {
    if (!out) throw Error(MMADMM_ERR_INVALID, "mmadmm_create: out is NULL");
    *out = nullptr;
    if ((dim != 2 && dim != 3) || nP < dim + 1 || nF < 1 || !Xp || !F || !mask || !p || !fn)
      throw Error(MMADMM_ERR_INVALID, "mmadmm_create: bad arguments");
    if (!(p->dt > 0) || !(p->tau > 0) || !(p->rho > 0))
      throw Error(MMADMM_ERR_INVALID, "mmadmm_create: dt, tau, rho must be positive");
    if (p->nranks > 1) throw Error(MMADMM_ERR_INVALID, "mmadmm_create: use mmadmm_create_partitioned for nranks > 1");
    mmx::check_kernel_layout(mmx::kLayoutWord);
    int ndev = 0;
    if (hipGetDeviceCount(&ndev) != hipSuccess || ndev == 0)
      throw Error(MMADMM_ERR_HIP, "mmadmm_create: no HIP device (the engine has no CPU fallback)");
    auto* h = new mmadmm_engine();
    try {
      if (dim == 2)
        h->e.reset(new mmx::Engine<2>(nP, Xp, Xc, nF, F, mask, *p, fn, user, nullptr));
      else
        h->e.reset(new mmx::Engine<3>(nP, Xp, Xc, nF, F, mask, *p, fn, user, nullptr));
    } catch (...) {
      delete h;
      throw;
    }
    *out = h;
  });
}

int mmadmm_create_partitioned(int dim, int nP, const double* Xp, const double* Xc, int nF, const int32_t* F,
                              const int32_t* mask, const mmadmm_params* p, mmadmm_monitor_fn fn, void* user,
                              mmadmm_comm comm, mmadmm_handle* out) {
  return guarded([&] {
    if (!out) throw Error(MMADMM_ERR_INVALID, "mmadmm_create_partitioned: out is NULL");
    *out = nullptr;
    if ((dim != 2 && dim != 3) || nP < dim + 1 || nF < 1 || !Xp || !F || !mask || !p || !fn)
      throw Error(MMADMM_ERR_INVALID, "mmadmm_create_partitioned: bad arguments");
    if (!(p->dt > 0) || !(p->tau > 0) || !(p->rho > 0))
      throw Error(MMADMM_ERR_INVALID, "mmadmm_create_partitioned: dt, tau, rho must be positive");
    if (p->nranks < 1 || p->rank < 0 || p->rank >= p->nranks)
      throw Error(MMADMM_ERR_INVALID, "mmadmm_create_partitioned: bad rank / nranks");
    mmx::Comm* c = mmx::comm_of(comm);
    if (p->nranks > 1 && (!c || c->nranks != p->nranks))
      throw Error(MMADMM_ERR_INVALID, "mmadmm_create_partitioned: communicator missing or of another size");
    mmx::check_kernel_layout(mmx::kLayoutWord);
    int ndev = 0;
    if (hipGetDeviceCount(&ndev) != hipSuccess || ndev == 0)
      throw Error(MMADMM_ERR_HIP, "mmadmm_create_partitioned: no HIP device (the engine has no CPU fallback)");
    auto* h = new mmadmm_engine();
    try {
      if (dim == 2)
        h->e.reset(new mmx::Engine<2>(nP, Xp, Xc, nF, F, mask, *p, fn, user, c));
      else
        h->e.reset(new mmx::Engine<3>(nP, Xp, Xc, nF, F, mask, *p, fn, user, c));
    } catch (...) {
      delete h;
      throw;
    }
    *out = h;
  });
}

int mmadmm_local_nodes(mmadmm_handle h, int* n_local, int32_t* global_ids) {
  return guarded([&] { eng(h).localNodes(n_local, global_ids); });
}

int mmadmm_step(mmadmm_handle h, int n_iters, double tol, double* Ih, int* admm_iters) {
  return guarded([&] { eng(h).step(n_iters, tol, Ih, admm_iters); });
}
int mmadmm_euler_step(mmadmm_handle h, double* Ih) {
  return guarded([&] {
    const double r = eng(h).eulerStep();
    if (Ih) *Ih = r;
  });
}
int mmadmm_backward_euler_step(mmadmm_handle h, double dt, double tol, double* Ih, int* newton_iters) {
  return guarded([&] {
    if (!(dt > 0)) throw mmx::Error(MMADMM_ERR_INVALID, "backward Euler: dt must be > 0");
    const double r = eng(h).backwardEulerStep(dt, tol, newton_iters);
    if (Ih) *Ih = r;
  });
}
int mmadmm_be_begin(mmadmm_handle h, double dt, double* Ih) {
  return guarded([&] {
    if (!(dt > 0)) throw mmx::Error(MMADMM_ERR_INVALID, "backward Euler: dt must be > 0");
    double sc[2] = {0.0, 0.0};
// ... 256 lines not shown
```

mm-admm_amd/csrc/host/knobs.h:

```cpp
#pragma once
#include <climits>
#include <cstdio>
#include <cstdlib>
#include <cstring>
#include <stdexcept>
#include <string>

namespace mmx {

constexpr int kTslot2dMax = 2 * 2048 * 64;
constexpr int kXupEarlyDefault = 1;
constexpr int kRedSplitMin = 4096;
constexpr int kProxBlock = 64;
constexpr int kSweepGrid = 128;
constexpr int kFacWaveChunk = 0;
constexpr int kChainImportLat = 8;
constexpr int kFacImpRows = 384;
constexpr int kFacRMax = 4;

inline int env_int(const char* name, int dflt, int lo = INT_MIN, int hi = INT_MAX) {
  const char* e = std::getenv(name);
  if (!e) return dflt;
  const int v = std::atoi(e);
  return v < lo ? lo : v > hi ? hi : v;
}
inline int env_flag(const char* name, bool dflt) { return env_int(name, dflt ? 1 : 0) != 0 ? 1 : 0; }
inline int env_word(const char* name, const char* words) {
  const char* e = std::getenv(name);
  if (!e) return 0;
  const size_t n = std::strlen(e);
  int i = 0;
  for (const char* w = words; *w; ++i) {
    const char* bar = std::strchr(w, '|');
    const size_t len = bar ? (size_t)(bar - w) : std::strlen(w);
    if (len == n && std::strncmp(w, e, n) == 0) return i;
    w += len + (bar ? 1 : 0);
  }
  return 0;
}
inline int env_set(const char* name) { return std::getenv(name) != nullptr ? 1 : 0; }
inline double env_double(const char* name, double dflt) {
  const char* e = std::getenv(name);
  return e ? std::atof(e) : dflt;
}

namespace knobs_detail {
inline int snap_xup_ch(int c) { return c >= 24 ? 24 : c >= 16 ? 16 : 8; }
inline int one_of3(int v, int a, int b, int c, int dflt) { return (v == a || v == b || v == c) ? v : dflt; }
inline int in_range_or(int v, int lo, int hi, int dflt) { return (v < lo || v > hi) ? dflt : v; }
inline void put(std::string& s, const char* name, const char* words, int v) {
  s += name;
  s += '=';
  if (!words) {
    s += std::to_string(v);
  } else {
    const char* w = words;
    for (int i = 0; i < v; ++i) w = std::strchr(w, '|') + 1;
    const char* bar = std::strchr(w, '|');
    s.append(w, bar ? (size_t)(bar - w) : std::strlen(w));
  }
  s += '\n';
}
inline void put(std::string& s, const char* name, const char*, double v) {
  char b[64];
  std::snprintf(b, sizeof b, "%.17g", v);
  s += name;
  s += '=';
  s += b;
  s += '\n';
}
inline int copy_out(const std::string& s, char* buf, int cap) {
  if (buf && cap > 0) {
    const size_t n = s.size() < (size_t)cap - 1 ? s.size() : (size_t)cap - 1;
    std::memcpy(buf, s.data(), n);
    buf[n] = 0;
  }
  return (int)s.size() + 1;
}
}

#define MMX_ENGINE_KNOBS(X) \
   \
   \
  X(int, tslot, "MMX_TSLOT", nullptr, env_flag("MMX_TSLOT", D == 3 || nF <= kTslot2dMax)) \
   \
  X(int, spin, "MMX_SPIN", nullptr, env_flag("MMX_SPIN", true)) \
   \
  X(int, zx, "MMX_ZX", nullptr, env_flag("MMX_ZX", true)) \
   \
  X(int, overlap, "MMX_OVERLAP", nullptr, nranks > 1 && env_flag("MMX_OVERLAP", true)) \
   \
  X(int, fusePred, "MMX_FUSE_PRED", nullptr, env_flag("MMX_FUSE_PRED", true)) \
   \
  X(int, gcSkip, "MMX_GC_SKIP", nullptr, env_flag("MMX_GC_SKIP", true)) \
   \
  X(int, xupOrder, "MMX_XUP_ORDER", nullptr, env_int("MMX_XUP_ORDER", D == 3) == 1) \
   \
  X(int, xupRec, "MMX_XUP_REC", nullptr, env_flag("MMX_XUP_REC", true)) \
   \
  X(int, xupCh, "MMX_XUP_CH", nullptr, knobs_detail::snap_xup_ch(env_int("MMX_XUP_CH", 8))) \
   \
   \
   \
  X(int, xupSweep, "MMX_XUP_SWEEP", nullptr, env_int("MMX_XUP_SWEEP", D == 3 ? 1 : (k.xupRec ? 2 : 0), 0)) \
   \
  X(int, xupEarly, "MMX_XUP_EARLY", nullptr, env_flag("MMX_XUP_EARLY", kXupEarlyDefault != 0)) \
   \
  X(int, xupSweepResid, "MMX_XUP_SWEEP_RESID", nullptr, env_flag("MMX_XUP_SWEEP_RESID", true)) \
   \
   \
  X(int, xcdMap, "MMX_XCD_MAP", nullptr, env_int("MMX_XCD_MAP", 1)) \
   \
  X(int, prox2dWave, "MMX_PROX2D", "lds|wave", D == 2 && env_word("MMX_PROX2D", "lds|wave")) \
   \
  X(int, prox3dQuad, "MMX_PROX3D", "wave|quad", env_word("MMX_PROX3D", "wave|quad")) \
   \
  X(int, proxBlock, "MMX_PROX_BLOCK", nullptr, knobs_detail::one_of3(env_int("MMX_PROX_BLOCK", 0), 64, 128, 256, kProxBlock)) \
   \
  X(int, gradCache, "MMX_GRAD_CACHE", nullptr, env_int("MMX_GRAD_CACHE", 1)) \
   \
  X(int, forceTie, "MMX_FORCE_TIE", nullptr, env_int("MMX_FORCE_TIE", 0)) \
   \
  X(int, monHint, "MMX_MON_HINT", nullptr, knobs_detail::in_range_or(env_int("MMX_MON_HINT", 1), 0, 3, 1)) \
   \
  X(int, iso, "MMX_ISO", nullptr, env_flag("MMX_ISO", true)) \
   \
  X(int, redSplitMin, "MMX_RED_SPLIT_MIN", nullptr, env_int("MMX_RED_SPLIT_MIN", kRedSplitMin)) \
   \
  X(int, regridGatherAll, "MMX_REGRID_GATHER", "near|all", env_word("MMX_REGRID_GATHER", "near|all")) \
   \
  X(double, regridMargin, "MMX_REGRID_MARGIN", nullptr, env_double("MMX_REGRID_MARGIN", 1.0)) \
   \
  X(int, fdjFast, "MMX_FDJ_FAST", nullptr, env_flag("MMX_FDJ_FAST", true)) \
   \
  X(int, jacAssembleEntry, "MMX_JAC_ASSEMBLE", "auto|entry", env_word("MMX_JAC_ASSEMBLE", "auto|entry")) \
   \
  X(int, schedProf, "MMX_SCHED_PROF", nullptr, env_set("MMX_SCHED_PROF"))

#define MMX_CHAIN_KNOBS(X) \
   \
  X(int, importLat, "MMX_CHAIN_LAT", nullptr, env_int("MMX_CHAIN_LAT", kChainImportLat, 0)) \
   \
  X(int, e48, "MMX_CHAIN_E48", nullptr, env_flag("MMX_CHAIN_E48", true)) \
   \
  X(int, pair, "MMX_CHAIN_PAIR", nullptr, env_flag("MMX_CHAIN_PAIR", true)) \
   \
  X(int, align, "MMX_CHAIN_ALIGN", nullptr, env_int("MMX_CHAIN_ALIGN", -1)) \
   \
  X(int, facR, "MMX_FAC_R", nullptr, env_int("MMX_FAC_R", kFacRMax)) \
   \
  X(int, facRI, "MMX_FAC_RI", nullptr, env_int("MMX_FAC_RI", kFacImpRows, 1, kFacImpRows)) \
   \
  X(int, schedProf, "MMX_SCHED_PROF", nullptr, env_set("MMX_SCHED_PROF"))

#define MMX_MATRIX_KNOBS(X) \
   \
  X(int, spmv, "MMX_SPMV", nullptr, env_int("MMX_SPMV", 2) == 1 ? 1 : 2) \
   \
  X(int, spin, "MMX_SPIN", nullptr, env_flag("MMX_SPIN", true)) \
   \
  X(int, sweepLevel, "MMX_SWEEP", "chain|level", env_word("MMX_SWEEP", "chain|level")) \
   \
   \
  X(int, factor, "MMX_FACTOR", "auto|level|global|wave", env_word("MMX_FACTOR", "auto|level|global|wave")) \
   \
   \
  X(int, factorGran, "MMX_FACTOR_GRAN", nullptr, env_int("MMX_FACTOR_GRAN", 0) == 1) \
   \
  X(int, chainProf, "MMX_CHAIN_PROF", nullptr, env_int("MMX_CHAIN_PROF", 0)) \
   \
  X(int, chainTrim, "MMX_CHAIN_TRIM", nullptr, env_flag("MMX_CHAIN_TRIM", true)) \
   \
  X(int, bwdGran, "MMX_BWD_GRAN", nullptr, env_flag("MMX_BWD_GRAN", true)) \
   \
  X(int, cgsUnfuse, "MMX_CGS_UNFUSE", nullptr, env_flag("MMX_CGS_UNFUSE", true)) \
   \
  X(int, sweepGrid, "MMX_SWEEP_GRID", nullptr, env_int("MMX_SWEEP_GRID", 0) > 0 ? env_int("MMX_SWEEP_GRID", 0) : kSweepGrid) \
   \
  X(int, facWg, "MMX_FAC_WG", nullptr, env_int("MMX_FAC_WG", 4) == 8 ? 8 : 4) \
   \
  X(int, facChunk, "MMX_FAC_CHUNK", nullptr, env_int("MMX_FAC_CHUNK", kFacWaveChunk, 0))

#define MMX_KNOB_FIELD(type, member, name, words, parse) type member;
#define MMX_KNOB_PARSE(type, member, name, words, parse) k.member = (parse);
#define MMX_KNOB_PUT(type, member, name, words, parse) knobs_detail::put(s, name, words, member);

struct EngineKnobs {
  MMX_ENGINE_KNOBS(MMX_KNOB_FIELD)

  static EngineKnobs from_env(int D, int nF, int nranks) {
    EngineKnobs k{};
    MMX_ENGINE_KNOBS(MMX_KNOB_PARSE)
    return k;
  }
  std::string text() const {
    std::string s;
    MMX_ENGINE_KNOBS(MMX_KNOB_PUT)
    return s;
  }
  int xup_sweep_max(size_t maxBlocks) const { return (int)(maxBlocks / 256 / (overlap ? 2 : 1)); }
  void check_xup_sweep(size_t maxBlocks) const {
    if (xupSweep > xup_sweep_max(maxBlocks))
      throw std::invalid_argument("MMX_XUP_SWEEP=" + std::to_string(xupSweep) + " is above " +
                                  std::to_string(xup_sweep_max(maxBlocks)) +
                                  ", what this mesh's partial-sum buffer holds");
  }
};

struct ChainKnobs {
  MMX_CHAIN_KNOBS(MMX_KNOB_FIELD)

  static ChainKnobs from_env() {
    ChainKnobs k{};
    MMX_CHAIN_KNOBS(MMX_KNOB_PARSE)
    return k;
  }
  std::string text() const {
    std::string s;
    MMX_CHAIN_KNOBS(MMX_KNOB_PUT)
    return s;
  }
};

struct MatrixKnobs {
  MMX_MATRIX_KNOBS(MMX_KNOB_FIELD)
  ChainKnobs sched;

  static MatrixKnobs from_env() {
    MatrixKnobs k{};
    MMX_MATRIX_KNOBS(MMX_KNOB_PARSE)
    k.sched = ChainKnobs::from_env();
    return k;
  }
  std::string text() const {
    std::string s;
    MMX_MATRIX_KNOBS(MMX_KNOB_PUT)
    return s + sched.text();
  }
};

}
```

mm-admm_amd/csrc/kernels/admm_kernels.h:

```cpp
#pragma once
#include <hip/hip_runtime.h>
#include <stdint.h>

#include "../host/knobs.h"
#include "layout.h"

namespace mmx {

constexpr int kNumPartials = kLayoutPartials;

template <int D>
struct DeviceMesh {
  int nP, nF;
  const int* F;
  const uint8_t* sbits;
  const uint8_t* nodeInterior;
  const int* inc_ptr;
  const int* inc_off;
  const double* remote;
  double* tslot;
  const double* zx;
  double* predPrev;
  double* predBar;
  double* gcache;
  int* tieList;
  unsigned* tieCount;
  unsigned* tieStale;
  unsigned* invFlag;
  int xupCh;
  int xupSweep;
  int forceTie;
  int monHint;
  const int* nodeOrder;
  int xupLo, xupHi;
  const double* invdiag;
  const int* xrec;
  const double* xinv;
  const int* xslot;
  int xslotStride, xslotCh;
  int xupEarly;
  int gcSkip;
  const double* Vc;
  const double* gx;
  const double* gy;
  const double* gz;
  const double* gvals;
  const double* gpad;
  const double* gcell[3];
  const double* giso;
  int gnx, gny, gnz;
  double ghx, ghy, ghz, grhx, grhy, grhz;
  double gax, gay, gaz, gspx, gspy, gspz, gnsx, gnsy, gnsz, grnsx, grnsy, grnsz;
  double Ehat[9];
  double powd, w;
  int compMesh;
  int prox2dWave;
};

struct StepScalars {
  double tau, dtsq, w, dt_over_tau;
};

template <int D>
void launch_gather_z(const DeviceMesh<D>& m, const double* x, double* z, hipStream_t st);
template <int D>
void launch_grad_simplex(const DeviceMesh<D>& m, const double* x, double* gs, bool zeroFixed,
                         double* partials, int* nblocks, hipStream_t st);
template <int D>
void launch_predict(const DeviceMesh<D>& m, const EngineKnobs& k, int mode, const double* gs, double* x, double* xPrev,
                    double* xBar, double dt_over_tau, hipStream_t st);
template <int D>
void launch_xupdate(const DeviceMesh<D>& m, const EngineKnobs& k, const StepScalars& sc, const double* xBar,
                    const double* z, const double* u, double* x, double* partials, int* nblocks,
                    bool resid, hipStream_t st, bool useTslot = false);
void launch_pad_rows(const double* vals, long long rows, double* pad, hipStream_t st);
template <int D>
void launch_iso_compact(const double* vals, long long points, double* iso, int* notIso, hipStream_t st);
template <int D>
void launch_bkinv_identity(int nF, double* B, hipStream_t st);

bool prox_double_buffered(int D, bool wave2d);
template <int D>
void launch_prox(const DeviceMesh<D>& m, const EngineKnobs& k, bool first, bool useCache, double tol, const double* x,
                 double* z, double* u, const double* Bin, double* Bout, double* partials, int* nblocks, hipStream_t st);
template <int D>
void launch_energy(const DeviceMesh<D>& m, const double* x, double* partials, int* nblocks,
                   hipStream_t st);
template <int D>
void launch_euler_apply(const DeviceMesh<D>& m, const EngineKnobs& k, const double* gs, double* x, double dt_over_tau,
                        hipStream_t st);
constexpr int kRedSplit = 32;
constexpr int kRedSets = 66;
struct RedWork {
  double* scratch = nullptr;
  int splitMin = kRedSplitMin;
};
void launch_reduce_partials(const double* partials, int nblocks, double* out, hipStream_t st, const RedWork& w = {});
void launch_reduce_steps(const double* partA, size_t stride, int nbA, const double* partB, int nbB, int n,
                         double* results, hipStream_t st, const RedWork& w = {});
void launch_reduce_partials2(const double* partials, int nblocks, double* out, const double* partials2, int nblocks2,
                             double* out2, hipStream_t st, const RedWork& w = {});
struct PackZX {
  const int* F = nullptr;
  const double* zx = nullptr;
  const double* x = nullptr;
  const double* xPrev = nullptr;
};
template <int D>
void launch_pack_export(int mode, int nExp, const int* expOff, const double* z, const double* u, const double* gs,
                        double w, double* out, hipStream_t st, const PackZX& zx = {});

template <int D>
void launch_fd_jac(const DeviceMesh<D>& m, const double* Vp, double h, double* dv, hipStream_t st,
                   unsigned* work = nullptr);
template <int D>
void launch_jac_assemble(const DeviceMesh<D>& m, const EngineKnobs& k, const int* ia, const int* ja, const double* dv,
                         double dt_over_tau, double* a, hipStream_t st, bool finish = true, int maxColNodes = 65);
template <int D>
void launch_be_residual(const DeviceMesh<D>& m, const EngineKnobs& k, const double* gs, const double* x,
                        const double* xn, double dt_over_tau, double* rhs, double* partials, int* nblocks, hipStream_t st);
void launch_add_inplace(int n, double* x, const double* dx, hipStream_t st);

template <int D>
void launch_debug_blockgrad(const DeviceMesh<D>& m, int s, const double* z, const double* dx, double* out,
                            int flags, hipStream_t st);

void launch_devmath(int op, int n, const double* in, double* out, hipStream_t st);

}
```

mm-admm_amd/csrc/kernels/admm_kernels_prox.hip:

```cpp
#include <cstdio>
#include <vector>

#include "admm_prox_common.h"

namespace mmx {
template <int K>
struct RegB {
  static constexpr bool kRowFence = false;
  static constexpr int kHeld = 0;
  static constexpr bool kCarry = false;
  static constexpr bool kRolled = false;
  static constexpr int kPipe = 0;
  static constexpr int kPipe1 = 0, kPipe2 = 0, kPipe3 = 0;
  static constexpr bool kPre = false;
  double* b;
  __device__ __forceinline__ double get(int i, int j) const { return b[i * K + j]; }
  __device__ __forceinline__ double heldRow(int, int) const { return 0.0; }
  __device__ __forceinline__ void holdRow(int, int, double) const {}
  __device__ __forceinline__ void set(int i, int j, double v) const { b[i * K + j] = v; }
  __device__ __forceinline__ void advance() {}
  __device__ __forceinline__ void fresh() {}
};
template <int K, int STRIDE = kLdsStride>
struct LdsB {
  static constexpr bool kRowFence = true;
  static constexpr int kHeld = 0;
  static constexpr bool kCarry = false;
  static constexpr bool kRolled = true;
  static constexpr int kPipe = 0;
  static constexpr int kPipe1 = 0, kPipe2 = 0, kPipe3 = 0;
  static constexpr bool kPre = false;
  double* base;
  __device__ __forceinline__ double get(int i, int j) const { return base[(i * K + j) * STRIDE]; }
  __device__ __forceinline__ double heldRow(int, int) const { return 0.0; }
  __device__ __forceinline__ void holdRow(int, int, double) const {}
  __device__ __forceinline__ void set(int i, int j, double v) const { base[(i * K + j) * STRIDE] = v; }
  __device__ __forceinline__ void advance() {}
  __device__ __forceinline__ void fresh() {}
};
typedef __attribute__((address_space(1))) double gdouble;
#ifndef MMX_WAVE_CARRY
#define MMX_WAVE_CARRY 1
#endif
#ifndef MMX_WAVE_HELD
#define MMX_WAVE_HELD 6
#endif
#ifndef MMX_ROW_PIPE
#define MMX_ROW_PIPE 2
#endif
typedef __attribute__((address_space(3))) double ldouble;

#ifndef MMX_WAVE_DMA
#define MMX_WAVE_DMA 1
#endif
#ifndef MMX_ROW_PIPE_FULL
#define MMX_ROW_PIPE_FULL 3
#endif
#ifndef MMX_ROW_PIPE1
#define MMX_ROW_PIPE1 6
#endif
#ifndef MMX_ROW_PIPE2
#define MMX_ROW_PIPE2 6
#endif
#ifndef MMX_ROW_PIPE3
#define MMX_ROW_PIPE3 2
#endif
template <int K, int PIPE = MMX_ROW_PIPE>
struct WaveB {
  static constexpr bool k2 = (K == 6);
  static constexpr bool kRowFence = true;
  static constexpr bool kRolled = true;
  static constexpr int kPipe = k2 ? 0 : PIPE;
  static constexpr int kPipe1 = k2 ? 0 : MMX_ROW_PIPE1, kPipe2 = k2 ? 0 : MMX_ROW_PIPE2, kPipe3 = k2 ? 0 : MMX_ROW_PIPE3;
  static constexpr int kHeld = k2 ? K : MMX_WAVE_HELD;
  static constexpr bool kCarry = !k2 && MMX_WAVE_CARRY;
  static constexpr bool kPre = MMX_WAVE_DMA && kHeld > 0;
  static constexpr bool kPairs = !k2 && MMX_B3_PAIRS;
  static constexpr int kLaneMul = kPairs ? 2 : 1;
  static __device__ __forceinline__ int eo(int e) { return kPairs ? (e & ~1) * 64 + (e & 1) : e * 64; }
  const gdouble* rd;
  gdouble* wr;
  ldouble* held;
  __device__ __forceinline__ double get(int i, int j) const { return rd[eo(i * K + j)]; }
  __device__ __forceinline__ double heldRow(int i, int j) const { return held[eo(i * K + j)]; }
  __device__ __forceinline__ void holdRow(int i, int j, double v) const { held[eo(i * K + j)] = v; }
  __device__ __forceinline__ void set(int i, int j, double v) const { __builtin_nontemporal_store(v, &wr[eo(i * K + j)]); }
  __device__ __forceinline__ void advance() { rd = wr; }
  __device__ __forceinline__ void fresh() { asm volatile("" : "+v"(rd), "+v"(wr)::"memory"); }
};

#define MMX_ROW_FENCE(BA) \
  if constexpr (BA::kRowFence) __builtin_amdgcn_sched_barrier(0)

#ifdef MMX_WAVE_PROF
__device__ unsigned long long* g_wprof;
#define WPROF(slot, dep)                                                                     \
  do {                                                                                       \
    asm volatile("" ::"v"(dep));                                                             \
    __builtin_amdgcn_sched_barrier(0);                                                       \
    const unsigned long long t_ = __builtin_readcyclecounter();                              \
    if (threadIdx.x == 0 && g_wprof) g_wprof[(size_t)blockIdx.x * 8 + (slot)] = t_;          \
    __builtin_amdgcn_sched_barrier(0);                                                       \
  } while (0)
#else
#define WPROF(slot, dep) \
  do {                   \
  } while (0)
#endif

template <int K, class BA>
__device__ __forceinline__ void load_row(const BA& B, int i, double (&r)[K]) {
#pragma unroll
  for (int j = 0; j < K; ++j) r[j] = B.get(i, j);
}
template <int K, int PIPE, class BA>
__device__ __forceinline__ void next_row(const BA& B, int i, double (&row)[K], double (&rn)[PIPE > 0 ? PIPE : 1][K],
                                         bool held = false) {
  if (held && i < BA::kHeld) {
#pragma unroll
    for (int j = 0; j < K; ++j) row[j] = B.heldRow(i, j);
  } else if constexpr (PIPE > 0) {
#pragma unroll
    for (int j = 0; j < K; ++j) row[j] = rn[0][j];
#pragma unroll
    for (int d = 0; d + 1 < PIPE; ++d)
#pragma unroll
      for (int j = 0; j < K; ++j) rn[d][j] = rn[d + 1][j];
    if (i + PIPE < K) load_row<K>(B, i + PIPE, rn[PIPE - 1]);
  } else {
    load_row<K>(B, i, row);
  }
}
template <int K, int PIPE, class BA>
__device__ __forceinline__ void start_rows(const BA& B, double (&rn)[PIPE > 0 ? PIPE : 1][K], int first = 0) {
#pragma unroll
  for (int d = 0; d < PIPE; ++d)
    if (first + d < K) load_row<K>(B, first + d, rn[d]);
}

template <int D, bool EXACT, class BA, int K>
__device__ __forceinline__ void bfgs_update_row(BA& B, int i, double pki, const double (&row)[K], const double (&yk)[K],
                                                const double (&pk)[K], const double (&yB)[K], double c1, double c2,
                                                double rc2, unsigned& eBy, double& fin) {
  double nrow[K], ykr[K];
#pragma unroll
  for (int q = 0; q < K; ++q) {
    ykr[q] = yk[q];
    if constexpr (D == 3) asm volatile("" : "+v"(ykr[q]));
  }
#pragma unroll
  for (int j = 0; j < K; ++j) {
    double by = row[0] * (ykr[0] * pk[j]);
#pragma unroll
// ... 191 lines not shown
            next_row<K, kP3>(B, i + u, rows[u], rn3, true);
          }
          bfgs_update_rows<D, EXACT, UR>(B, i, pki, rows, yk, pk, yB, c1, c2, rc2, eBy, fin);
        }
      }
    } else {
      start_rows<K, kPipe>(B, rn);
#pragma unroll
      for (int i = 0; i < K; ++i) {
        MMX_ROW_FENCE(BA);
        double row[K];
        next_row<K, kPipe>(B, i, row, rn);
        bfgs_update_row<D, EXACT>(B, i, pk[i], row, yk, pk, yB, c1, c2, rc2, eBy, fin);
      }
    }
    MMX_ROW_FENCE(BA);
    if constexpr (BA::kPipe > 0 && !EXACT) {
      if (iter == 0) WPROF(5, fin);
    }
    B.advance();
    if constexpr (!EXACT) {
      unsigned ePY = 0u;
#pragma unroll
      for (int k = 0; k < K; ++k) ePY = max(ePY, max(mk_exp(pk[k], 450), mk_exp(yB[k], 450)));
      if (!(c2 >= 0x1p-100 && c2 <= 0x1p100) || eBy > 1799u || ePY > 899u || fin != 0.0) *tie = true;
      if (*tie) break;
    }
#pragma unroll
    for (int i = 0; i < K; ++i) G[i] = G1[i];
    if (Ix < tol) break;
  }
  return (iter == 50) ? 50 : iter + 1;
}

template <int D, bool FIRST, int ISO = -1>
__device__ __forceinline__ void prox_simplex(const DeviceMesh<D>& m, double tol, const double* __restrict__ x,
                                             double* __restrict__ zg, double* __restrict__ ug,
                                             const double* Bin, double* Bout, bool useCache, int s,
                                             double (&pv)[6]) {
  constexpr int K = D * (D + 1);
  const GridView<D> g = gridOf<D, ISO>(m);
  const FunctionalConsts<D> fc = constsOf<D>(m);
  int f[D + 1];
  loadVerts<D>(m, s, f);
  const unsigned bits = m.sbits[s];
  const unsigned fixedBits = bits & 0xF;
  double xi[K];
  loadXi<D>(m, f, xi);
  double dx[K], z[K], zold[K];
  gatherX<D>(x, f, dx);
  double* zs = zg + zu_base<D>(s);
  double* us = ug + zu_base<D>(s);
  if (m.zx)
    gatherX<D>(m.zx, f, z);
  else
#pragma unroll
    for (int i = 0; i < K; ++i) z[i] = zs[zu_i<D>(i)];
#pragma unroll
  for (int i = 0; i < K; ++i) {
    dx[i] = dx[i] + us[zu_i<D>(i)];
    zold[i] = z[i];
  }
  double B[K * K];
  if constexpr (!FIRST) {
#pragma unroll
    for (int i = 0; i < K * K; ++i) B[i] = Bin[bidx<D>(s, i)];
  }
  double G[K], G1[K], Igt;
  bool bad = false;
  (void)G1;
  double* gc = m.gcache + (size_t)s * K;
  entry_grad<D>(g, fc, z, xi, dx, gc, !FIRST && useCache, G, Igt, bad);
  zeroFixed<D>(G, fixedBits);
  const double Ihsave = Igt;
  if constexpr (FIRST) {
    const double h = 2.0 * cr_sqrt(2.220446049250313080847e-16);
    double zp[K];
#pragma unroll
    for (int i = 0; i < K; ++i) zp[i] = z[i];
    for (int i = 0; i < K; i++) {
      zp[i] += h;
      double Ig2;
      blockGrad<D, true, true>(g, fc, zp, xi, dx, G1, Ig2);
      zeroFixed<D>(G1, fixedBits);
#pragma unroll
      for (int r = 0; r < K; ++r) B[r * K + i] = (G1[r] - G[r]) / h;
      zp[i] = z[i];
    }
#pragma unroll
    for (int n = 0; n < D + 1; n++)
      if (bits & (1u << (4 + n)))
#pragma unroll
        for (int c = 0; c < D; c++) B[(D * n + c) * K + D * n + c] = 1.0;
    invertK<K>(B);
  }
  RegB<K> Bacc{B};
  const int its = bfgs_iterations<D>(Bacc, g, fc, z, xi, dx, G, fixedBits, tol, bad, gc);
  double dual2 = 0.0;
  double un[K];
#pragma unroll
  for (int i = 0; i < K; ++i) {
    zs[zu_i<D>(i)] = z[i];
    un[i] = dx[i] - z[i];
    us[zu_i<D>(i)] = un[i];
    const double d = z[i] - zold[i];
    dual2 += d * d;
  }
  write_tslot<D>(m, s, z, un);
#pragma unroll
  for (int i = 0; i < K * K; ++i) Bout[bidx<D>(s, i)] = B[i];
  pv[0] = Ihsave;
  pv[1] = dual2;
  pv[3] = (double)its;
  pv[4] = bad ? 1.0 : 0.0;
  pv[5] = (double)its;
}

template <int D, bool FIRST, int ISO = -1>
__global__ void __launch_bounds__(kBlock) k_prox(DeviceMesh<D> m, double tol, const double* __restrict__ x,
                                                  double* __restrict__ zg, double* __restrict__ ug,
                                                  const double* Bin, double* Bout, double* __restrict__ partials,
                                                  int useCache) {
  const int s = blockIdx.x * kBlock + threadIdx.x;
  double pv[6] = {0, 0, 0, 0, 0, 0};
  if (s < m.nF) prox_simplex<D, FIRST, ISO>(m, tol, x, zg, ug, Bin, Bout, useCache != 0, s, pv);
  block_partials<6>(pv, partials);
}

template <int D, int BS>
__global__ void __launch_bounds__(BS) k_prox_fix(DeviceMesh<D> m, double tol, const double* __restrict__ x,
                                                 double* __restrict__ zg, double* __restrict__ ug,
                                                 const double* Bin, double* Bout, double* __restrict__ partials) {
  const unsigned n = *m.tieCount;
  for (unsigned i = blockIdx.x; i < n; i += gridDim.x) {
    const int b = m.tieList[i];
    const int s = b * BS + (int)threadIdx.x;
    double pv[6] = {0, 0, 0, 0, 0, 0};
    if (s < m.nF) prox_simplex<D, false>(m, tol, x, zg, ug, Bin, Bout, false, s, pv);
    block_partials<6, BS>(pv, partials, b);
    __syncthreads();
  }
  rearm_tie_queue(m.tieStale);
}

#ifndef MMX_ZU_NT
#define MMX_ZU_NT 0
#endif
#ifndef MMX_LDS_DMA
#define MMX_LDS_DMA 0
#endif
#ifndef MMX_MON_HINT_BUILD
#define MMX_MON_HINT_BUILD 1
#endif
template <int D, int BS>
__global__ void __launch_bounds__(BS, 2) k_prox_lds(DeviceMesh<D> m, double tol, const double* __restrict__ x,
                                                        double* __restrict__ zg, double* __restrict__ ug,
                                                        double* __restrict__ Bg, double* __restrict__ partials,
                                                        int useCache) {
  constexpr int K = D * (D + 1), KK = K * K;
  static_assert(BS % 64 == 0, "whole wave blocks per chunk");
  __shared__ __attribute__((aligned(16))) double lds[KK * BS];
  const int tid = threadIdx.x;
  const int lb = (int)blockIdx.x;
  const int s0 = lb * BS;
  const int nIn = min(BS, m.nF - s0);
  const bool act = tid < nIn;
  const int s = act ? s0 + tid : s0;
  int f[D + 1];
  loadVerts<D>(m, s, f);
  const unsigned fixedBits = m.sbits[s] & 0xF;
  double* zs = zg + zu_base<D>(s);
  double* us = ug + zu_base<D>(s);
  double* gc = m.gcache + (size_t)s * K;
  double z[K], z0[K], dx[K], gcv[K];
  if (m.zx)
    gatherX<D>(m.zx, f, z);
  else
#pragma unroll
    for (int i = 0; i < K; ++i) z[i] = zs[zu_i<D>(i)];
#pragma unroll
  for (int i = 0; i < K; ++i) {
    z0[i] = z[i];
    dx[i] = us[zu_i<D>(i)];
  }
  if (useCache) {
#pragma unroll
    for (int i = 0; i < K; ++i) gcv[i] = gc[i];
  }
  double* chunk = Bg + (size_t)s0 * KK;
  constexpr int NL = KK / 2;
  v2nt cv[MMX_LDS_DMA ? 1 : NL];
  if constexpr (!MMX_LDS_DMA) {
#pragma unroll
    for (int r = 0; r < NL; ++r) cv[r] = __builtin_nontemporal_load(reinterpret_cast<const v2nt*>(chunk) + tid + r * BS);
  }
  constexpr bool kHint = (D == 2) && MMX_MON_HINT_BUILD == 1;
  constexpr bool kTouch = (D == 2) && MMX_MON_HINT_BUILD == 2;
  MonHint2 hint;
#ifdef MMX_HINT_PROBE
  hint.hits = 0;
#endif
  if constexpr (kHint || kTouch) {
    if (m.giso && m.monHint > 0) {
      monHintRequest(gridOf<D>(m), z, m.monHint, hint);
    } else {
      hint.cell[0] = hint.cell[1] = hint.cell[2] = -1;
    }
  }
  double xi[K], dxv[K];
  loadXi<D>(m, f, xi);
  gatherX<D>(x, f, dxv);
  if constexpr (MMX_LDS_DMA) {
    __builtin_amdgcn_sched_barrier(0);
    const char* src = reinterpret_cast<const char*>(chunk) + tid * 16;
    const int wofs = __builtin_amdgcn_readfirstlane((tid >> 6) * 1024);
#pragma unroll
    for (int r = 0; r < NL; ++r)
      __builtin_amdgcn_global_load_lds(src + r * BS * 16,
                                       (__attribute__((address_space(3))) void*)(reinterpret_cast<char*>(lds) + wofs + r * BS * 16),
                                       16, 0, 0);
    __builtin_amdgcn_sched_barrier(0);
    __builtin_amdgcn_s_waitcnt(0);
  } else {
#pragma unroll
    for (int r = 0; r < NL; ++r) reinterpret_cast<v2nt*>(lds)[tid + r * BS] = cv[r];
  }
#pragma unroll
  for (int i = 0; i < K; ++i) dx[i] = dxv[i] + dx[i];
  __syncthreads();
  if constexpr (kTouch) {
    if (hint.cell[0] >= 0)
#pragma unroll
      for (int i = 0; i < 12; ++i) asm volatile("" ::"v"(hint.v[i]));
  }
  double pv[6] = {0, 0, 0, 0, 0, 0};
  bool tie = false;
  if (act) {
    const GridView<D> g = gridOf<D>(m);
    const FunctionalConsts<D> fc = constsOf<D>(m);
    double G[K], Igt;
    bool bad = false;
    entry_grad<D, false>(g, fc, z, xi, dx, gcv, useCache != 0, G, Igt, bad, &tie);
    zeroFixed<D>(G, fixedBits);
    const double Ihsave = Igt;
    LdsB<K, 64> Bacc{lds + (tid >> 6) * KK * 64 + (tid & 63)};
    const int its =
        tie ? 0
            : bfgs_iterations<D, LdsB<K, 64>, false, kHint>(Bacc, g, fc, z, xi, dx, G, fixedBits, tol, bad,
                                                            m.gcSkip ? nullptr : m.gcache + (size_t)s * K, &tie,
                                                            kHint ? &hint : nullptr);
#ifdef MMX_HINT_PROBE
    if constexpr (kHint) pv[2] = (double)hint.hits;
#endif
    double dual2 = 0.0;
#pragma unroll
    for (int i = 0; i < K; ++i) {
      const double d = z[i] - z0[i];
      dual2 += d * d;
    }
    pv[0] = Ihsave;
    pv[1] = dual2;
    pv[3] = (double)its;
    pv[4] = bad ? 1.0 : 0.0;
    pv[5] = (double)its;
  }
  if (m.forceTie > 0 && tid == 0 && (int)((unsigned)lb % (unsigned)m.forceTie) == 0) tie = true;
  if (__syncthreads_or(tie ? 1 : 0)) {
    if (tid == 0) m.tieList[atomicAdd(m.tieCount, 1u)] = lb;
    return;
  }
  if (act) {
    double un[K];
#pragma unroll
    for (int i = 0; i < K; ++i) {
      un[i] = dx[i] - z[i];
      if constexpr (MMX_ZU_NT) {
        __builtin_nontemporal_store(z[i], &zs[zu_i<D>(i)]);
        __builtin_nontemporal_store(un[i], &us[zu_i<D>(i)]);
      } else {
        zs[zu_i<D>(i)] = z[i];
        us[zu_i<D>(i)] = un[i];
      }
    }
    write_tslot<D>(m, s, z, un);
  }
#pragma unroll
  for (int r = 0; r < NL; ++r)
    __builtin_nontemporal_store(reinterpret_cast<const v2nt*>(lds)[tid + r * BS], reinterpret_cast<v2nt*>(chunk) + tid + r * BS);
  block_partials<6, BS>(pv, partials, lb);
}

#ifndef MMX_WAVE_OCC
#define MMX_WAVE_OCC 1
#endif
#ifndef MMX_WAVE_OCC2
#define MMX_WAVE_OCC2 2
#endif
#ifndef MMX_WAVE_PERSIST
#define MMX_WAVE_PERSIST 0
#endif
#ifndef MMX_HELD_DMA_CPOL
#define MMX_HELD_DMA_CPOL 2
#endif
#ifndef MMX_WAVE_XCD
#define MMX_WAVE_XCD 1
#endif
template <int D, bool COMP, bool EXACT, bool ISO = false, bool DRAIN = true>
__device__ __forceinline__ void prox_wave_block(const DeviceMesh<D>& m, double tol, const double* __restrict__ x,
                                                double* __restrict__ zg, double* __restrict__ ug, const double* Bin,
                                                double* Bout, double* __restrict__ partials, int useCache, int lb,
                                                double* ldsHeld) {
  constexpr int K = D * (D + 1), KK = K * K;
  const int tid = threadIdx.x;
  const int s0 = lb * 64;
  const bool act = s0 + tid < m.nF;
  const int s = act ? s0 + tid : s0;
  if constexpr (!EXACT) WPROF(0, s);
  int f[D + 1];
  loadVerts<D>(m, s, f);
  const unsigned fixedBits = m.sbits[s] & 0xF;
  double* zs = zg + zu_base<D>(s);
  double* us = ug + zu_base<D>(s);
  double* gc = m.gcache + (size_t)s * K;
  double z[K], dx[K], gcv[K];
  if (m.zx)
    gatherX<D>(m.zx, f, z);
  else
#pragma unroll
    for (int i = 0; i < K; ++i) z[i] = zs[zu_i<D>(i)];
#pragma unroll
  for (int i = 0; i < K; ++i) dx[i] = us[zu_i<D>(i)];
  if (!EXACT && useCache) {
#pragma unroll
    for (int i = 0; i < K; ++i) gcv[i] = gc[i];
  }
  double xi[K];
  if constexpr (COMP) gatherX<D>(m.Vc, f, xi);
  {
    double dxv[K];
    gatherX<D>(x, f, dxv);
#pragma unroll
    for (int i = 0; i < K; ++i) dx[i] = dxv[i] + dx[i];
    if constexpr (WaveB<K>::kPre) {
      __builtin_amdgcn_sched_barrier(0);
      const char* src = reinterpret_cast<const char*>(Bin + (size_t)lb * KK * 64) + tid * 16;
      char* dst = reinterpret_cast<char*>(ldsHeld);
#pragma unroll
      for (int c = 0; c < WaveB<K>::kHeld * K * 64 * 8 / 1024; ++c)
        __builtin_amdgcn_global_load_lds(src + c * 1024, (__attribute__((address_space(3))) void*)(dst + c * 1024),
                                         16, 0, MMX_HELD_DMA_CPOL);
    }
  }
  double pv[6] = {0, 0, 0, 0, 0, 0};
  bool tie = false;
  if (act) {
    GridView<D> g = gridOf<D>(m);
    if constexpr (ISO)
      __builtin_assume(g.iso != nullptr);
    else
      g.iso = nullptr;
    FunctionalConsts<D> fc = constsOf<D>(m);
    fc.compMesh = COMP ? 1 : 0;
    double G[K], Igt;
    bool bad = false;
    entry_grad<D, EXACT>(g, fc, z, xi, dx, gcv, !EXACT && useCache != 0, G, Igt, bad, &tie);
    zeroFixed<D>(G, fixedBits);
    const double Ihsave = Igt;
    if constexpr (!EXACT) WPROF(1, G[K - 1]);
    const size_t gb = (size_t)lb * KK * 64 + WaveB<K>::kLaneMul * tid;
    int its;
    {
      using WB = WaveB<K, ISO ? MMX_ROW_PIPE : MMX_ROW_PIPE_FULL>;
      WB Bacc{(const gdouble*)(Bin + gb), (gdouble*)(Bout + gb), (ldouble*)(ldsHeld + WaveB<K>::kLaneMul * tid)};
      its = tie ? 0 : bfgs_iterations<D, WB, EXACT>(Bacc, g, fc, z, xi, dx, G, fixedBits, tol, bad, gc, &tie);
    }
    double dual2 = 0.0, z0[K];
    if (m.zx)
      gatherX<D>(m.zx, f, z0);
    else
#pragma unroll
      for (int i = 0; i < K; ++i) z0[i] = zs[zu_i<D>(i)];
#pragma unroll
    for (int i = 0; i < K; ++i) {
      const double d = z[i] - z0[i];
      dual2 += d * d;
    }
    pv[0] = Ihsave;
    pv[1] = dual2;
    pv[3] = (double)its;
    pv[4] = bad ? 1.0 : 0.0;
    pv[5] = (double)its;
  }
  if constexpr (!EXACT) {
    if (m.forceTie > 0 && tid == 0 && (int)((unsigned)lb % (unsigned)m.forceTie) == 0) tie = true;
    if (__syncthreads_or(tie ? 1 : 0)) {
      if (tid == 0) m.tieList[atomicAdd(m.tieCount, 1u)] = lb;
      __builtin_amdgcn_s_waitcnt(0);
      return;
    }
  }
  if (act) {
    double un[K];
#pragma unroll
    for (int i = 0; i < K; ++i) {
      zs[zu_i<D>(i)] = z[i];
      un[i] = dx[i] - z[i];
      us[zu_i<D>(i)] = un[i];
    }
    write_tslot<D>(m, s, z, un);
  }
  block_partials<6, 64>(pv, partials, lb);
  if constexpr (!EXACT && DRAIN) {
    __builtin_amdgcn_s_waitcnt(0);
    WPROF(6, pv[0]);
  }
}

template <int D, bool COMP, bool ISO = false>
__global__ void __launch_bounds__(64, D == 2 ? MMX_WAVE_OCC2 : MMX_WAVE_OCC) k_prox_wave(DeviceMesh<D> m, double tol, const double* __restrict__ x,
                                                     double* __restrict__ zg, double* __restrict__ ug,
                                                     const double* Bin, double* Bout, double* __restrict__ partials,
                                                     int useCache) {
  constexpr int K = D * (D + 1);
  __shared__ __attribute__((aligned(16))) double ldsHeld[WaveB<K>::kHeld > 0 ? WaveB<K>::kHeld * K * 64 : 2];
#if MMX_WAVE_PERSIST
  if constexpr (D == 3) {
    const int nb = (m.nF + 63) / 64, g8 = max(1, (int)gridDim.x / 8), c = (int)(blockIdx.x % 8), j = (int)(blockIdx.x / 8);
    const int q = nb / 8, r = nb % 8, lo = c * q + min(c, r), hi = lo + q + (c < r ? 1 : 0);
    for (int lb = lo + j; lb < hi; lb += g8) {
      prox_wave_block<D, COMP, false, ISO, false>(m, tol, x, zg, ug, Bin, Bout, partials, useCache, lb, ldsHeld);
    }
    return;
  }
#endif
  const int lb = MMX_WAVE_XCD ? logical_block_any() : (int)blockIdx.x;
  prox_wave_block<D, COMP, false, ISO>(m, tol, x, zg, ug, Bin, Bout, partials, useCache, lb, ldsHeld);
}

template <int D, bool COMP, bool ISO = false>
__global__ void __launch_bounds__(64, D == 2 ? MMX_WAVE_OCC2 : MMX_WAVE_OCC) k_prox_wave_fix(DeviceMesh<D> m, double tol,
                                                         const double* __restrict__ x, double* __restrict__ zg,
                                                         double* __restrict__ ug, const double* Bin, double* Bout,
                                                         double* __restrict__ partials) {
  constexpr int K = D * (D + 1);
  __shared__ __attribute__((aligned(16))) double ldsHeld[WaveB<K>::kHeld > 0 ? WaveB<K>::kHeld * K * 64 : 2];
  const unsigned n = *m.tieCount;
  for (unsigned i = blockIdx.x; i < n; i += gridDim.x) {
    prox_wave_block<D, COMP, true, ISO>(m, tol, x, zg, ug, Bin, Bout, partials, 0, m.tieList[i], ldsHeld);
    __syncthreads();
  }
  rearm_tie_queue(m.tieStale);
}

template <int D>
__global__ void k_bkinv_identity(int nF, double* B) {
  constexpr int K = D * (D + 1);
  const long long t = (long long)blockIdx.x * blockDim.x + threadIdx.x;
  if (t >= (long long)nF * K) return;
  const int s = (int)(t / K), i = (int)(t % K);
  B[bidx<D>(s, i * K + i)] = 1.0;
}
template <int D>
void launch_bkinv_identity(int nF, double* B, hipStream_t st) {
  constexpr int K = D * (D + 1);
  const long long n = (long long)nF * K;
  if (n > 0) hipLaunchKernelGGL(k_bkinv_identity<D>, dim3((unsigned)((n + kBlock - 1) / kBlock)), dim3(kBlock), 0, st, nF, B);
}
template void launch_bkinv_identity<2>(int, double*, hipStream_t);
template void launch_bkinv_identity<3>(int, double*, hipStream_t);
bool prox_double_buffered(int D, bool wave2d) { return D == 3 || wave2d; }
#ifdef MMX_WAVE_PROF
static unsigned long long* g_wprofHost = nullptr;
static size_t g_wprofN = 0;
static void wprof_arm(int nblocks) {
  if (g_wprofN >= (size_t)nblocks * 8) return;
  if (g_wprofHost) (void)hipFree(g_wprofHost);
  g_wprofN = (size_t)nblocks * 8;
  (void)hipMalloc((void**)&g_wprofHost, g_wprofN * sizeof(unsigned long long));
  (void)hipMemset(g_wprofHost, 0, g_wprofN * sizeof(unsigned long long));
  (void)hipMemcpyToSymbol(HIP_SYMBOL(g_wprof), &g_wprofHost, sizeof(g_wprofHost));
}
#endif
template <int D>
void launch_prox(const DeviceMesh<D>& m, const EngineKnobs& k, bool first, bool useCache, double tol, const double* x,
                 double* z, double* u, const double* Bin, double* Bout, double* partials, int* nblocks,
                 hipStream_t st) {
#ifdef MMX_WAVE_PROF
  if (D == 3 && !first) wprof_arm((m.nF + 63) / 64);
#endif
  const int uc = (useCache && k.gradCache) ? 1 : 0;
  *nblocks = nblk(m.nF);
  if (m.nF == 0) return;
  if (first) {
    dispatch_iso<D>(m, [&](auto iso) {
      hipLaunchKernelGGL((k_prox<D, true, decltype(iso)::value>), dim3(*nblocks), dim3(kBlock), 0, st, m, tol, x, z, u,
                         Bin, Bout, partials, 0);
    });
  } else if (D == 2 && m.prox2dWave) {
    *nblocks = (m.nF + 63) / 64;
    const dim3 fg(std::min(*nblocks, kFixGrid));
    dispatch_bool(m.compMesh != 0, [&](auto c) {
      constexpr bool C = decltype(c)::value;
      hipLaunchKernelGGL((k_prox_wave<D, C>), dim3(*nblocks), dim3(64), 0, st, m, tol, x, z, u, Bin, Bout, partials, uc);
      hipLaunchKernelGGL((k_prox_wave_fix<D, C>), fg, dim3(64), 0, st, m, tol, x, z, u, Bin, Bout, partials);
    });
  } else if constexpr (D == 2) {
    double* B = Bout;
    const int bs = k.proxBlock;
    *nblocks = (m.nF + bs - 1) / bs;
    const dim3 fg(std::min(*nblocks, kFixGrid));
    if (bs == 64) {
      hipLaunchKernelGGL((k_prox_lds<D, 64>), dim3(*nblocks), dim3(64), 0, st, m, tol, x, z, u, B, partials, uc);
      hipLaunchKernelGGL((k_prox_fix<D, 64>), fg, dim3(64), 0, st, m, tol, x, z, u, B, B, partials);
    } else if (bs == 128) {
      hipLaunchKernelGGL((k_prox_lds<D, 128>), dim3(*nblocks), dim3(128), 0, st, m, tol, x, z, u, B, partials, uc);
      hipLaunchKernelGGL((k_prox_fix<D, 128>), fg, dim3(128), 0, st, m, tol, x, z, u, B, B, partials);
    } else {
      hipLaunchKernelGGL((k_prox_lds<D, 256>), dim3(*nblocks), dim3(256), 0, st, m, tol, x, z, u, B, partials, uc);
      hipLaunchKernelGGL((k_prox_fix<D, 256>), fg, dim3(256), 0, st, m, tol, x, z, u, B, B, partials);
    }
  } else {
    *nblocks = (m.nF + 63) / 64;
    const dim3 fg(std::min(*nblocks, kFixGrid));
    if (k.prox3dQuad) return launch_prox_quad(m, tol, x, z, u, Bin, Bout, partials, nblocks, uc, st);
    const dim3 wg(MMX_WAVE_PERSIST ? (std::min(*nblocks, MMX_WAVE_PERSIST) + 7) / 8 * 8 : *nblocks);
    dispatch_bool(m.compMesh != 0, [&](auto c) {
      dispatch_bool(m.giso != nullptr, [&](auto i) {
        constexpr bool C = decltype(c)::value, I = decltype(i)::value;
        hipLaunchKernelGGL((k_prox_wave<D, C, I>), wg, dim3(64), 0, st, m, tol, x, z, u, Bin, Bout, partials, uc);
        hipLaunchKernelGGL((k_prox_wave_fix<D, C, I>), fg, dim3(64), 0, st, m, tol, x, z, u, Bin, Bout, partials);
      });
    });
  }
}
template void launch_prox<2>(const DeviceMesh<2>&, const EngineKnobs&, bool, bool, double, const double*, double*,
                             double*, const double*, double*, double*, int*, hipStream_t);
template void launch_prox<3>(const DeviceMesh<3>&, const EngineKnobs&, bool, bool, double, const double*, double*,
                             double*, const double*, double*, double*, int*, hipStream_t);
}

#ifdef MMX_WAVE_PROF
extern "C" int mmx_wprof_dump(const char* path) {
  if (!mmx::g_wprofHost) return -1;
  if (hipDeviceSynchronize() != hipSuccess) return -2;
  std::vector<unsigned long long> h(mmx::g_wprofN);
  if (hipMemcpy(h.data(), mmx::g_wprofHost, h.size() * 8, hipMemcpyDeviceToHost) != hipSuccess) return -3;
  FILE* f = fopen(path, "wb");
  if (!f) return -4;
  fwrite(h.data(), 8, h.size(), f);
  fclose(f);
  return (int)(h.size() / 8);
}
#endif
extern "C" unsigned mmx_layout_admm_prox(void) { return mmx::kLayoutWord; }
```

mm-admm_amd/csrc/kernels/admm_kernels_step.hip:

```cpp
#include "admm_common.h"

namespace mmx {
template <int D>
__global__ void __launch_bounds__(kBlock) k_gather_z(DeviceMesh<D> m, const double* __restrict__ x,
                                                      double* __restrict__ z) {
  constexpr int K = D * (D + 1);
  const int s = blockIdx.x * kBlock + threadIdx.x;
  if (s >= m.nF) return;
  int f[D + 1];
  loadVerts<D>(m, s, f);
  double v[K];
  gatherX<D>(x, f, v);
#pragma unroll
  for (int i = 0; i < K; ++i) z[zu_base<D>(s) + zu_i<D>(i)] = v[i];
}

template <int D, int ISO = -1>
__global__ void __launch_bounds__(kBlock) k_grad_simplex(DeviceMesh<D> m, const double* __restrict__ x,
                                                          double* __restrict__ gs, int zeroFixedRows,
                                                          double* __restrict__ partials) {
  constexpr int K = D * (D + 1);
  const int s = blockIdx.x * kBlock + threadIdx.x;
  double pv[5] = {0, 0, 0, 0, 0};
  if (s < m.nF) {
// ... 48 lines not shown

template <int CH>
struct XupHead {
  int v, b, e;
  double inv;
  int off[CH];
};
template <int D, int CH>
__device__ __forceinline__ void xup_head_rec(const DeviceMesh<D>& m, int idx, XupHead<CH>& h) {
  const int* r = m.xrec + (size_t)idx * kXupRecInts;
  h.v = r[0];
  h.b = r[1];
  h.e = r[2];
  h.inv = m.xinv[idx];
#pragma unroll
  for (int j = 0; j < CH; ++j) h.off[j] = m.xslot[(size_t)j * m.xslotStride + idx];
}
template <int D, int CH>
__device__ __forceinline__ void xup_head_csr(const DeviceMesh<D>& m, int idx, XupHead<CH>& h) {
  h.v = m.nodeOrder ? m.nodeOrder[idx] : idx;
  h.b = m.inc_ptr[h.v];
  h.e = m.inc_ptr[h.v + 1];
  h.inv = m.invdiag[h.v];
#pragma unroll
  for (int j = 0; j < CH; ++j) h.off[j] = (h.e > h.b) ? m.inc_off[min(h.b + j, h.e - 1)] : 0;
}
template <int D, bool RESID, bool TS, int CH = 8, bool ZX = false, bool PRED = false, bool REM = false>
__device__ __forceinline__ void xupdate_node(const DeviceMesh<D>& m, const StepScalars& sc,
                                             const double* __restrict__ xBar, const double* __restrict__ z,
                                             const double* __restrict__ u, double* __restrict__ x,
                                             const XupHead<CH>& h, double (&pv)[3]) {
  {
    const int v = h.v, b = h.b, e = h.e;
    double acc[D];
#pragma unroll
    for (int c = 0; c < D; ++c) acc[c] = 0.0;
    double xb[D], zn[D];
    if constexpr (PRED) {
      double xv[D];
#pragma unroll
      for (int c = 0; c < D; ++c) {
        xv[c] = x[(size_t)v * D + c];
        xb[c] = 2 * xv[c] - m.predPrev[(size_t)v * D + c];
      }
#pragma unroll
      for (int c = 0; c < D; ++c) {
        m.predBar[(size_t)v * D + c] = xb[c];
        m.predPrev[(size_t)v * D + c] = xv[c];
      }
    } else {
#pragma unroll
      for (int c = 0; c < D; ++c) xb[c] = xBar[(size_t)v * D + c];
    }
    constexpr bool zv0 = ZX && !TS;
    if constexpr (zv0) {
      if constexpr (PRED) {
#pragma unroll
        for (int c = 0; c < D; ++c) zn[c] = xb[c];
      } else {
#pragma unroll
        for (int c = 0; c < D; ++c) zn[c] = m.zx[(size_t)v * D + c];
      }
    }
    const double inv = h.inv;
    auto addChunk = [&](int t0, const int(&off)[CH]) {
      double zv[CH][D], uv[CH][D];
#pragma unroll
      for (int j = 0; j < CH; ++j) {
        const bool loc = off[j] >= 0;
        if constexpr (TS) {
          const double* pt = loc ? m.tslot + off[j] : m.remote + (size_t)(-1 - off[j]) * D;
#pragma unroll
          for (int c = 0; c < D; ++c) zv[j][c] = pt[c];
        } else {
          const double* pz = loc ? z + zu_off<D>(off[j]) : m.remote + (size_t)(-1 - off[j]) * D;
          const double* pu = loc ? u + zu_off<D>(off[j]) : pz;
#pragma unroll
          for (int c = 0; c < D; ++c) {
            if constexpr (zv0 && REM)
              zv[j][c] = loc ? zn[c] : pz[c];
            else if constexpr (zv0)
              zv[j][c] = zn[c];
            else
              zv[j][c] = pz[c];
            uv[j][c] = pu[c];
          }
        }
      }
#pragma unroll
      for (int j = 0; j < CH; ++j) {
        if (t0 + j < e) {
#pragma unroll
          for (int c = 0; c < D; ++c) {
            if constexpr (TS)
              acc[c] += zv[j][c];
            else
              acc[c] += (off[j] >= 0) ? sc.w * (sc.w * (zv[j][c] - uv[j][c])) : zv[j][c];
          }
        }
      }
    };
    if (b < e) addChunk(b, h.off);
    for (int t0 = b + CH; t0 < e; t0 += CH) {
      int off[CH];
#pragma unroll
      for (int j = 0; j < CH; ++j) off[j] = m.inc_off[min(t0 + j, e - 1)];
      addChunk(t0, off);
    }
    double xn[D];
#pragma unroll
    for (int c = 0; c < D; ++c) {
      xn[c] = ((sc.tau * xb[c]) + sc.dtsq * acc[c]) * inv;
      x[(size_t)v * D + c] = xn[c];
    }
    if constexpr (RESID) {
      double r2 = 0.0;
      auto residChunk = [&](int t0, const int(&off)[CH]) {
        double zv[CH][D];
#pragma unroll
        for (int j = 0; j < CH; ++j) {
          const double* pz = z + zu_off<D>(off[j] >= 0 ? off[j] : 0);
#pragma unroll
          for (int c = 0; c < D; ++c) zv[j][c] = pz[c];
        }
#pragma unroll
        for (int j = 0; j < CH; ++j) {
          if (t0 + j < e && off[j] >= 0) {
#pragma unroll
            for (int c = 0; c < D; ++c) {
              const double d = xn[c] - zv[j][c];
              r2 += d * d;
            }
          }
        }
      };
      if (b < e) residChunk(b, h.off);
      for (int t0 = b + CH; t0 < e; t0 += CH) {
        int off[CH];
#pragma unroll
        for (int j = 0; j < CH; ++j) off[j] = m.inc_off[min(t0 + j, e - 1)];
        residChunk(t0, off);
      }
      pv[2] = r2;
    }
  }
}
template <int D, int CH, bool REC>
__device__ __forceinline__ void xup_head(const DeviceMesh<D>& m, int idx, XupHead<CH>& h) {
  if constexpr (REC)
    xup_head_rec<D, CH>(m, idx, h);
  else
    xup_head_csr<D, CH>(m, idx, h);
}
template <int D, bool RESID, bool TS, bool ZX = false, bool PRED = false, bool REM = false, bool REC = false>
__global__ void __launch_bounds__(kBlock) k_xupdate(DeviceMesh<D> m, StepScalars sc,
                                                     const double* __restrict__ xBar,
                                                     const double* __restrict__ z,
                                                     const double* __restrict__ u, double* __restrict__ x,
                                                     double* __restrict__ partials, int xcd) {
  constexpr int CH = (D == 2 ? MMX_XU_CH2D : 8);
  const int lb = logical_block(xcd);
  const int idx = m.xupLo + lb * kBlock + threadIdx.x;
  double pv[3] = {0, 0, 0};
  if (idx < m.xupHi) {
    XupHead<CH> h;
    xup_head<D, CH, REC>(m, idx, h);
    xupdate_node<D, RESID, TS, CH, ZX, PRED, REM>(m, sc, xBar, z, u, x, h, pv);
  }
  if constexpr (RESID) block_partials<3>(pv, partials, lb);
}
template <int D, bool TS, int CH, bool RESID = false, bool REC = false, bool EARLY = false>
__global__ void __launch_bounds__(kBlock) k_xupdate_sweep(DeviceMesh<D> m, StepScalars sc,
                                                           const double* __restrict__ xBar,
                                                           const double* __restrict__ z, const double* __restrict__ u,
                                                           double* __restrict__ x, int n8, double* __restrict__ partials) {
  static_assert(REC || !EARLY, "the early request reads the records");
  const int c = (int)(blockIdx.x % 8), w = (int)(blockIdx.x / 8), per = (int)(gridDim.x / 8);
  const int lo = m.xupLo + c * n8, hi = min(lo + n8, m.xupHi);
  double pv[3], r2 = 0.0;
  int idx = lo + w * kBlock + (int)threadIdx.x;
  if constexpr (EARLY) {
    XupHead<CH> cur, nxt;
    if (idx < hi) xup_head<D, CH, true>(m, idx, cur);
    nxt = cur;
    for (; idx < hi; idx += per * kBlock) {
      if (idx + per * kBlock < hi) xup_head<D, CH, true>(m, idx + per * kBlock, nxt);
      __builtin_amdgcn_sched_barrier(0);
      xupdate_node<D, RESID, TS, CH>(m, sc, xBar, z, u, x, cur, pv);
      if constexpr (RESID) r2 += pv[2];
      cur = nxt;
    }
  } else {
    for (; idx < hi; idx += per * kBlock) {
      XupHead<CH> h;
      xup_head<D, CH, REC>(m, idx, h);
      xupdate_node<D, RESID, TS, CH>(m, sc, xBar, z, u, x, h, pv);
      if constexpr (RESID) r2 += pv[2];
    }
  }
  if constexpr (RESID) {
    double q[3] = {0.0, 0.0, r2};
    block_partials<3>(q, partials, (int)blockIdx.x);
  }
}

template <int D, int ISO = -1>
__global__ void __launch_bounds__(kBlock) k_energy(DeviceMesh<D> m, const double* __restrict__ x,
                                                    double* __restrict__ partials) {
  constexpr int K = D * (D + 1);
  const int s = blockIdx.x * kBlock + threadIdx.x;
  double pv[5] = {0, 0, 0, 0, 0};
  if (s < m.nF) {
    int f[D + 1];
    loadVerts<D>(m, s, f);
    double z[K], xi[K], Igt;
    gatherX<D>(x, f, z);
    loadXi<D>(m, f, xi);
    const double e = blockGrad<D, false, false>(gridOf<D, ISO>(m), constsOf<D>(m), z, xi, nullptr, nullptr, Igt);
    pv[0] = e;
    pv[4] = (e == e) ? 0.0 : 1.0;
  }
  block_partials<5>(pv, partials);
}

template <int D>
__global__ void __launch_bounds__(kBlock) k_euler_apply(DeviceMesh<D> m, const double* __restrict__ gs,
                                                         double* __restrict__ x, double dt_over_tau, int xcd) {
  const int idx = logical_block(xcd) * kBlock + threadIdx.x;
  if (idx >= m.nP) return;
  const int v = m.nodeOrder ? m.nodeOrder[idx] : idx;
  double g[D];
#pragma unroll
  for (int c = 0; c < D; ++c) g[c] = 0.0;
  if (m.nodeInterior[v]) {
    const int b = m.inc_ptr[v], e = m.inc_ptr[v + 1];
    for (int t = b; t < e; ++t) {
      const int off = m.inc_off[t];
      const double* src = (off >= 0) ? gs + off : m.remote + (size_t)(-1 - off) * D;
#pragma unroll
      for (int c = 0; c < D; ++c) g[c] += src[c];
    }
  }
#pragma unroll
  for (int c = 0; c < D; ++c) x[(size_t)v * D + c] -= dt_over_tau * g[c];
}

template <int D>
__global__ void __launch_bounds__(kBlock) k_pack_export(int mode, int nExp, const int* __restrict__ expOff,
                                                         const double* __restrict__ z, const double* __restrict__ u,
                                                         const double* __restrict__ gs, double w,
                                                         double* __restrict__ out, PackZX zx) {
  constexpr int K = D * (D + 1);
  const int e = blockIdx.x * kBlock + threadIdx.x;
  if (e >= nExp) return;
  const size_t off = (size_t)expOff[e], zo = zu_off<D>(expOff[e]);
  double zv[D];
  if (mode == 0 && zx.zx) {
    const int s = expOff[e] / K, n = (expOff[e] % K) / D;
    const size_t v = (size_t)zx.F[(size_t)s * (D + 1) + n];
#pragma unroll
    for (int c = 0; c < D; ++c) zv[c] = zx.x ? 2 * zx.x[v * D + c] - zx.xPrev[v * D + c] : zx.zx[v * D + c];
  } else {
#pragma unroll
    for (int c = 0; c < D; ++c) zv[c] = z[zo + c];
  }
#pragma unroll
  for (int c = 0; c < D; ++c)
    out[(size_t)e * D + c] = (mode == 0) ? w * (w * (zv[c] - u[zo + c])) : gs[off + c];
}

constexpr int kRed = 1024;
__device__ void reduce_set(const double* __restrict__ partials, int nblocks, double* __restrict__ out);

__global__ void __launch_bounds__(kRed) k_reduce_partials(const double* __restrict__ partials, int nblocks,
                                                           double* __restrict__ out, const double* __restrict__ partials2,
                                                           int nblocks2, double* __restrict__ out2) {
  if (blockIdx.x == 1)
    reduce_set(partials2, nblocks2, out2);
  else
    reduce_set(partials, nblocks, out);
}

__global__ void __launch_bounds__(kRed) k_reduce_steps(const double* __restrict__ partA, size_t stride, int nbA,
                                                        const double* __restrict__ partB, int nbB, int n,
                                                        double* __restrict__ results) {
  const int i = blockIdx.x;
  if (i < n)
    reduce_set(partA + (size_t)i * stride, nbA, results + (size_t)i * 2 * kNumPartials);
  else
    reduce_set(partB, nbB, results + (size_t)(n - 1) * 2 * kNumPartials + kNumPartials);
}

constexpr int kRedLanes = 256;
__global__ void __launch_bounds__(kRedLanes) k_reduce_split(const double* __restrict__ partA, size_t stride, int nbA,
                                                            int nA, const double* __restrict__ partB, int nbB,
                                                            double* __restrict__ scratch) {
  __shared__ double red[kRedLanes / 64][kNumPartials];
  const int q = (int)blockIdx.x / kRedSplit, r = (int)blockIdx.x % kRedSplit;
  const bool isA = q < nA;
  const double* p = isA ? partA + (size_t)q * stride : partB;
  const int nb = isA ? nbA : nbB;
  const int per = (nb + kRedSplit - 1) / kRedSplit, lo = min(nb, r * per), hi = min(nb, lo + per);
  const int tid = (int)threadIdx.x;
  double acc[kNumPartials];
#pragma unroll
  for (int i = 0; i < kNumPartials; ++i) acc[i] = 0.0;
  for (int b = lo + tid; b < hi; b += kRedLanes)
#pragma unroll
    for (int i = 0; i < kNumPartials; ++i) {
      const double v = p[(size_t)b * kNumPartials + i];
      acc[i] = (i == 5) ? fmax(acc[i], v) : acc[i] + v;
    }
#pragma unroll
  for (int i = 0; i < kNumPartials; ++i) acc[i] = (i == 5) ? wave_max(acc[i]) : wave_sum(acc[i]);
  if ((tid & 63) == 0)
#pragma unroll
    for (int i = 0; i < kNumPartials; ++i) red[tid >> 6][i] = acc[i];
  __syncthreads();
  if (tid < kNumPartials) {
    double v = red[0][tid];
    for (int w = 1; w < kRedLanes / 64; ++w) v = (tid == 5) ? fmax(v, red[w][tid]) : v + red[w][tid];
    scratch[(size_t)blockIdx.x * kNumPartials + tid] = v;
  }
}
__global__ void __launch_bounds__(64) k_reduce_combine(const double* __restrict__ scratch, int nA,
                                                       double* __restrict__ outA, size_t outStride,
                                                       double* __restrict__ outB) {
  const int q = (int)blockIdx.x, t = (int)threadIdx.x;
  if (t >= kNumPartials) return;
  const double* base = scratch + (size_t)q * kRedSplit * kNumPartials + t;
  double acc = base[0];
  for (int k = 1; k < kRedSplit; ++k) acc = (t == 5) ? fmax(acc, base[(size_t)k * kNumPartials]) : acc + base[(size_t)k * kNumPartials];
  (q < nA ? outA + (size_t)q * outStride : outB)[t] = acc;
}

__device__ void reduce_set(const double* __restrict__ partials, int nblocks, double* __restrict__ out) {
  __shared__ double red[kRed / 64][kNumPartials];
  const int tid = threadIdx.x;
  double acc[kNumPartials];
#pragma unroll
  for (int i = 0; i < kNumPartials; ++i) acc[i] = 0.0;
  int b = tid;
  for (; b + 3 * kRed < nblocks; b += 4 * kRed) {
    double v[4][kNumPartials];
#pragma unroll
    for (int q = 0; q < 4; ++q)
#pragma unroll
      for (int i = 0; i < kNumPartials; ++i) v[q][i] = partials[(size_t)(b + q * kRed) * kNumPartials + i];
#pragma unroll
    for (int q = 0; q < 4; ++q)
#pragma unroll
      for (int i = 0; i < kNumPartials; ++i) acc[i] = (i == 5) ? fmax(acc[i], v[q][i]) : acc[i] + v[q][i];
  }
  for (; b < nblocks; b += kRed)
#pragma unroll
    for (int i = 0; i < kNumPartials; ++i) {
      const double v = partials[(size_t)b * kNumPartials + i];
      acc[i] = (i == 5) ? fmax(acc[i], v) : acc[i] + v;
    }
#pragma unroll
  for (int i = 0; i < kNumPartials; ++i) acc[i] = (i == 5) ? wave_max(acc[i]) : wave_sum(acc[i]);
  if ((tid & 63) == 0)
#pragma unroll
    for (int i = 0; i < kNumPartials; ++i) red[tid >> 6][i] = acc[i];
  __syncthreads();
  if (tid < kNumPartials) {
    double r = red[0][tid];
    for (int w = 1; w < kRed / 64; ++w) r = (tid == 5) ? fmax(r, red[w][tid]) : r + red[w][tid];
    out[tid] = r;
  }
}

template <int D>
void launch_gather_z(const DeviceMesh<D>& m, const double* x, double* z, hipStream_t st) {
  if (m.nF == 0) return;
  hipLaunchKernelGGL(k_gather_z<D>, dim3(nblk(m.nF)), dim3(kBlock), 0, st, m, x, z);
}
template <int D>
void launch_grad_simplex(const DeviceMesh<D>& m, const double* x, double* gs, bool zeroFixedRows,
                         double* partials, int* nblocks, hipStream_t st) {
  *nblocks = nblk(m.nF);
  if (m.nF == 0) return;
  dispatch_iso<D>(m, [&](auto iso) {
    hipLaunchKernelGGL((k_grad_simplex<D, decltype(iso)::value>), dim3(*nblocks), dim3(kBlock), 0, st, m, x, gs,
                       zeroFixedRows ? 1 : 0, partials);
  });
}
template <int D>
void launch_predict(const DeviceMesh<D>& m, const EngineKnobs& k, int mode, const double* gs, double* x,
                    double* xPrev, double* xBar, double dt_over_tau, hipStream_t st) {
  if (m.nP == 0) return;
  hipLaunchKernelGGL(k_predict<D>, dim3(nblk_xcd(m.nP, k.xcdMap)), dim3(kBlock), 0, st, m, mode, gs, x, xPrev, xBar,
                     dt_over_tau, k.xcdMap);
}
template <int D>
void launch_xupdate(const DeviceMesh<D>& m, const EngineKnobs& k, const StepScalars& sc, const double* xBar,
                    const double* z, const double* u, double* x, double* partials, int* nblocks, bool resid,
                    hipStream_t st, bool useTslot) {
  const int nsub = m.xupHi - m.xupLo;
  *nblocks = nblk_xcd(nsub, k.xcdMap);
  if (nsub <= 0) {
    *nblocks = 0;
    return;
  }
  const bool ts = useTslot && m.tslot;
  const bool rem = m.remote != nullptr;
  const bool rec = m.xrec != nullptr;
  auto needCols = [&](int ch) {
    if (rec && m.xslotCh < ch) throw std::logic_error("launch_xupdate: the slot table has fewer columns than the chunk");
  };
  if (m.zx && !resid && !ts) {
    needCols(D == 2 ? MMX_XU_CH2D : 8);
    dispatch_bool(m.predBar != nullptr, [&](auto pred) {
      dispatch_bool(rem, [&](auto r) {
        dispatch_bool(rec, [&](auto rc) {
          hipLaunchKernelGGL(
              (k_xupdate<D, false, false, true, decltype(pred)::value, decltype(r)::value, decltype(rc)::value>),
              dim3(*nblocks), dim3(kBlock), 0, st, m, sc, xBar, z, u, x, partials, k.xcdMap);
        });
      });
    });
    return;
  }
  if (m.predBar || m.predPrev)
    throw std::logic_error("launch_xupdate: predBar set for an x-update that cannot fuse predictX");
  const bool sweepResid = resid && ts && k.xupSweepResid;
  if (m.xupSweep > 0 && (!resid || sweepResid)) {
    const int n8 = ((nsub + kBlock - 1) / kBlock + 7) / 8 * kBlock;
    const dim3 g(256 * m.xupSweep);
    auto sweep = [&](auto tsT, auto chT, auto residT, double* part) {
      constexpr bool TS = decltype(tsT)::value, RS = decltype(residT)::value;
      constexpr int CH = decltype(chT)::value;
      needCols(CH);
      if (rec && m.xupEarly)
        hipLaunchKernelGGL((k_xupdate_sweep<D, TS, CH, RS, true, true>), g, dim3(kBlock), 0, st, m, sc, xBar, z, u, x, n8,
                           part);
      else if (rec)
        hipLaunchKernelGGL((k_xupdate_sweep<D, TS, CH, RS, true, false>), g, dim3(kBlock), 0, st, m, sc, xBar, z, u, x, n8,
                           part);
      else
        hipLaunchKernelGGL((k_xupdate_sweep<D, TS, CH, RS>), g, dim3(kBlock), 0, st, m, sc, xBar, z, u, x, n8, part);
    };
    using T = std::true_type;
    using F = std::false_type;
    if (sweepResid) {
      *nblocks = (int)g.x;
      sweep(T{}, std::integral_constant<int, 8>{}, T{}, partials);
    } else if (ts && m.xupCh >= 24)
      sweep(T{}, std::integral_constant<int, 24>{}, F{}, nullptr);
    else if (ts && m.xupCh >= 16)
      sweep(T{}, std::integral_constant<int, 16>{}, F{}, nullptr);
    else if (ts)
      sweep(T{}, std::integral_constant<int, 8>{}, F{}, nullptr);
    else
      sweep(F{}, std::integral_constant<int, (D == 2 ? MMX_XU_CH2D : 8)>{}, F{}, nullptr);
    return;
  }
  needCols(D == 2 ? MMX_XU_CH2D : 8);
  dispatch_bool(resid, [&](auto r) {
    dispatch_bool(ts, [&](auto t) {
      dispatch_bool(rec, [&](auto rc) {
        hipLaunchKernelGGL((k_xupdate<D, decltype(r)::value, decltype(t)::value, false, false, false, decltype(rc)::value>),
                           dim3(*nblocks), dim3(kBlock), 0, st, m, sc, xBar, z, u, x, partials, k.xcdMap);
      });
    });
  });
}
template <int D>
void launch_energy(const DeviceMesh<D>& m, const double* x, double* partials, int* nblocks, hipStream_t st) {
  *nblocks = nblk(m.nF);
  if (m.nF == 0) return;
  dispatch_iso<D>(m, [&](auto iso) {
    hipLaunchKernelGGL((k_energy<D, decltype(iso)::value>), dim3(*nblocks), dim3(kBlock), 0, st, m, x, partials);
  });
}
template <int D>
void launch_euler_apply(const DeviceMesh<D>& m, const EngineKnobs& k, const double* gs, double* x, double dt_over_tau,
                        hipStream_t st) {
  if (m.nP == 0) return;
  hipLaunchKernelGGL(k_euler_apply<D>, dim3(nblk_xcd(m.nP, k.xcdMap)), dim3(kBlock), 0, st, m, gs, x, dt_over_tau,
                     k.xcdMap);
}
static bool split_ok(const RedWork& w, int nblocks) { return w.scratch && nblocks >= w.splitMin; }
static void reduce_split(const double* partA, size_t stride, int nbA, int nA, double* outA, size_t outStride,
                         const double* partB, int nbB, double* outB, const RedWork& w, hipStream_t st) {
  const int sets = nA + (nbB >= 0 ? 1 : 0);
  hipLaunchKernelGGL(k_reduce_split, dim3(sets * kRedSplit), dim3(kRedLanes), 0, st, partA, stride, nbA, nA, partB,
                     nbB, w.scratch);
  hipLaunchKernelGGL(k_reduce_combine, dim3(sets), dim3(64), 0, st, w.scratch, nA, outA, outStride, outB);
}
void launch_reduce_partials(const double* partials, int nblocks, double* out, hipStream_t st, const RedWork& w) {
  if (split_ok(w, nblocks))
    reduce_split(partials, 0, nblocks, 1, out, 0, partials, -1, out, w, st);
  else
    hipLaunchKernelGGL(k_reduce_partials, dim3(1), dim3(kRed), 0, st, partials, nblocks, out, partials, nblocks, out);
}
void launch_reduce_steps(const double* partA, size_t stride, int nbA, const double* partB, int nbB, int n,
                         double* results, hipStream_t st, const RedWork& w) {
  if (split_ok(w, nbA) && n + 1 <= kRedSets)
    reduce_split(partA, stride, nbA, n, results, (size_t)2 * kNumPartials, partB, nbB,
                 results + (size_t)(n - 1) * 2 * kNumPartials + kNumPartials, w, st);
  else
    hipLaunchKernelGGL(k_reduce_steps, dim3(n + 1), dim3(kRed), 0, st, partA, stride, nbA, partB, nbB, n, results);
}
void launch_reduce_partials2(const double* partials, int nblocks, double* out, const double* partials2, int nblocks2,
                             double* out2, hipStream_t st, const RedWork& w) {
  if (split_ok(w, nblocks))
    reduce_split(partials, 0, nblocks, 1, out, 0, partials2, nblocks2, out2, w, st);
  else
    hipLaunchKernelGGL(k_reduce_partials, dim3(2), dim3(kRed), 0, st, partials, nblocks, out, partials2, nblocks2,
                       out2);
}
template <int D>
void launch_pack_export(int mode, int nExp, const int* expOff, const double* z, const double* u, const double* gs,
                        double w, double* out, hipStream_t st, const PackZX& zx) {
  if (nExp <= 0) return;
  hipLaunchKernelGGL(k_pack_export<D>, dim3((nExp + kBlock - 1) / kBlock), dim3(kBlock), 0, st, mode, nExp, expOff, z, u,
                     gs, w, out, zx);
}
#define MMX_INST(D)                                                                                                   \
  template void launch_pack_export<D>(int, int, const int*, const double*, const double*, const double*, double,      \
                                      double*, hipStream_t, const PackZX&);                                           \
  template void launch_gather_z<D>(const DeviceMesh<D>&, const double*, double*, hipStream_t);                        \
  template void launch_grad_simplex<D>(const DeviceMesh<D>&, const double*, double*, bool, double*, int*, hipStream_t); \
  template void launch_predict<D>(const DeviceMesh<D>&, const EngineKnobs&, int, const double*, double*, double*,     \
                                  double*, double, hipStream_t);                                                      \
  template void launch_xupdate<D>(const DeviceMesh<D>&, const EngineKnobs&, const StepScalars&, const double*,        \
                                  const double*, const double*, double*, double*, int*, bool, hipStream_t, bool);     \
  template void launch_energy<D>(const DeviceMesh<D>&, const double*, double*, int*, hipStream_t);                    \
  template void launch_euler_apply<D>(const DeviceMesh<D>&, const EngineKnobs&, const double*, double*, double,       \
                                      hipStream_t);
MMX_INST(2)
MMX_INST(3)
}
extern "C" unsigned mmx_layout_admm_step(void) { return mmx::kLayoutWord; }
```

mm-admm_amd/python/mmadmm_amd.py:

```python
import ctypes
import os
import time

import numpy as np

_HERE = os.path.dirname(os.path.abspath(__file__))
LIB_PATH = os.environ.get("MMADMM_LIB", os.path.join(os.path.dirname(_HERE), "lib", "libmmadmm.so"))

MMADMM_OK = 0
BOUNDARY_FREE, BOUNDARY_FIXED, INTERIOR = 0, 1, 2

c_double_p = ctypes.POINTER(ctypes.c_double)
c_int_p = ctypes.POINTER(ctypes.c_int32)
MONITOR_FN = ctypes.CFUNCTYPE(None, ctypes.c_int, c_double_p, c_double_p, ctypes.c_void_p)
c_ll_p = ctypes.POINTER(ctypes.c_longlong)
ALLGATHER_FN = ctypes.CFUNCTYPE(ctypes.c_int, ctypes.c_void_p, c_double_p, c_double_p, ctypes.c_longlong)
EXCHANGE_FN = ctypes.CFUNCTYPE(ctypes.c_int, ctypes.c_void_p, ctypes.c_int, c_int_p, c_double_p, c_ll_p, c_ll_p,
                               c_double_p, c_ll_p, c_ll_p)


class mmadmm_params(ctypes.Structure):
    _fields_ = [("dt", ctypes.c_double), ("tau", ctypes.c_double), ("rho", ctypes.c_double),
                ("grad_use", ctypes.c_int), ("device", ctypes.c_int), ("rank", ctypes.c_int),
                ("nranks", ctypes.c_int), ("partition", ctypes.c_int)]


PARTITION = {"rcb": 0, "ranges": 1}


class mmadmm_stats(ctypes.Structure):
    _fields_ = [("steps", ctypes.c_longlong), ("admm_iters", ctypes.c_longlong),
                ("bfgs_iters", ctypes.c_longlong), ("max_bfgs", ctypes.c_int),
                ("last_primal", ctypes.c_double), ("last_dual", ctypes.c_double),
                ("t_prox_ms", ctypes.c_double), ("t_xupdate_ms", ctypes.c_double),
                ("t_step_ms", ctypes.c_double), ("n_prox", ctypes.c_longlong),
                ("n_xupdate", ctypes.c_longlong), ("n_steps_timed", ctypes.c_longlong),
                ("prox_bytes", ctypes.c_double), ("xupdate_bytes", ctypes.c_double),
                ("newton_iters", ctypes.c_longlong), ("jacobians", ctypes.c_longlong),
                ("cg_iters", ctypes.c_longlong), ("t_jac_ms", ctypes.c_double), ("t_solve_ms", ctypes.c_double),
                ("t_be_ms", ctypes.c_double), ("regrids", ctypes.c_longlong), ("regrid_rows", ctypes.c_longlong),
                ("regrid_gather_bytes", ctypes.c_double), ("regrid_cand", ctypes.c_longlong),
                ("regrid_fallbacks", ctypes.c_longlong), ("monitor_iso", ctypes.c_int),
                ("t_exchange_ms", ctypes.c_double), ("n_exchange", ctypes.c_longlong),
                ("halo_send_bytes", ctypes.c_double), ("halo_recv_bytes", ctypes.c_double),
                ("interior_nodes", ctypes.c_int), ("overlap", ctypes.c_int)]

    def as_dict(self):
        return {k: getattr(self, k) for k, _ in self._fields_}


class MMADMMError(RuntimeError):
    def __init__(self, code, msg):
        super().__init__(f"mmadmm error {code}: {msg}")
        self.code = code


class InvertedElementError(MMADMMError):
    """The reference aborts on assert(Edet > 0) (src/AdaptationFunctional.cpp:174)."""


class NonFiniteEnergyError(MMADMMError):
    """MMADMM_ERR_NONFINITE: a NaN energy with no inverted element -- a monitor value that is not
    finite (on an element partition with a time-varying monitor: an evaluation outside the rank's
    rebuilt grid box)."""


_lib = None


def lib():
    global _lib
    if _lib is not None:
        return _lib
    if not os.path.exists(LIB_PATH):
        raise ImportError(f"libmmadmm.so not built ({LIB_PATH}); run `make -C mm-admm_amd`")
    L = ctypes.CDLL(LIB_PATH)
    L.mmadmm_last_error.restype = ctypes.c_char_p
    L.mmadmm_builtin_monitor.argtypes = [ctypes.c_int, ctypes.c_int, ctypes.POINTER(MONITOR_FN),
                                         ctypes.POINTER(ctypes.c_void_p)]
    L.mmadmm_create.argtypes = [ctypes.c_int, ctypes.c_int, c_double_p, c_double_p, ctypes.c_int, c_int_p,
                                c_int_p, ctypes.POINTER(mmadmm_params), MONITOR_FN, ctypes.c_void_p,
                                ctypes.POINTER(ctypes.c_void_p)]
    L.mmadmm_step.argtypes = [ctypes.c_void_p, ctypes.c_int, ctypes.c_double, c_double_p,
                              ctypes.POINTER(ctypes.c_int)]
    L.mmadmm_euler_step.argtypes = [ctypes.c_void_p, c_double_p]
    L.mmadmm_energy.argtypes = [ctypes.c_void_p, c_double_p]
    L.mmadmm_backward_euler_step.argtypes = [ctypes.c_void_p, ctypes.c_double, ctypes.c_double, c_double_p,
                                             ctypes.POINTER(ctypes.c_int)]
    L.mmadmm_get_jacobian.argtypes = [ctypes.c_void_p, ctypes.POINTER(ctypes.c_longlong), c_int_p, c_int_p,
                                      c_double_p]
    L.mmadmm_done.argtypes = [ctypes.c_void_p]
    L.mmadmm_get.argtypes = [ctypes.c_void_p, ctypes.c_char_p, c_double_p]
    L.mmadmm_get_simplices.argtypes = [ctypes.c_void_p, c_int_p]
    L.mmadmm_sizes.argtypes = [ctypes.c_void_p] + [ctypes.POINTER(ctypes.c_int)] * 3
    L.mmadmm_set_timing.argtypes = [ctypes.c_void_p, ctypes.c_int]
    L.mmadmm_stats_get.argtypes = [ctypes.c_void_p, ctypes.POINTER(mmadmm_stats)]
    L.mmadmm_stats_reset.argtypes = [ctypes.c_void_p]
    L.mmadmm_options_get.argtypes = [ctypes.c_void_p, ctypes.c_char_p, ctypes.c_int]
    L.mmadmm_sync.argtypes = [ctypes.c_void_p]
    L.mmadmm_regrid.argtypes = [ctypes.c_void_p, ctypes.c_double]
    L.mmadmm_set_regrid.argtypes = [ctypes.c_void_p, ctypes.c_int]
    L.mmadmm_regrid_values.argtypes = [ctypes.c_void_p, c_double_p]
    L.mmadmm_regrid_values_device.argtypes = [ctypes.c_void_p, ctypes.c_void_p, ctypes.c_void_p]
    L.mmadmm_regrid_field.argtypes = [ctypes.c_void_p, c_double_p, ctypes.c_double]
    L.mmadmm_regrid_field_device.argtypes = [ctypes.c_void_p, ctypes.c_void_p, ctypes.c_double, ctypes.c_void_p]
    L.mmadmm_field_hessian.argtypes = [ctypes.c_void_p, c_double_p, c_double_p]
    L.mmadmm_field_hessian_device.argtypes = [ctypes.c_void_p, ctypes.c_void_p, ctypes.c_void_p, ctypes.c_void_p]
    L.mmadmm_get_device.argtypes = [ctypes.c_void_p, ctypes.c_char_p, ctypes.c_void_p, ctypes.c_void_p]
    L.mmadmm_field_monitor.argtypes = [ctypes.c_int, ctypes.c_int, c_double_p, ctypes.c_int, c_int_p, c_double_p,
                                       ctypes.c_double, c_double_p, c_double_p]
    L.mmadmm_regrid_field_huang.argtypes = [ctypes.c_void_p, c_double_p, ctypes.c_double, c_double_p]
    L.mmadmm_regrid_field_huang_device.argtypes = [ctypes.c_void_p, ctypes.c_void_p, ctypes.c_double, ctypes.c_void_p,
                                                   c_double_p]
    L.mmadmm_field_solve_info.argtypes = [ctypes.c_void_p, c_int_p, c_int_p]
    L.mmadmm_field_monitor_huang.argtypes = [ctypes.c_int, ctypes.c_int, c_double_p, ctypes.c_int, c_int_p, c_double_p,
                                             ctypes.c_double, c_double_p, c_double_p, c_double_p]
    L.mmadmm_field_root.argtypes = [ctypes.c_int, ctypes.c_int, c_double_p, c_double_p]
    L.mmadmm_regrid_fields.argtypes = [ctypes.c_void_p, ctypes.c_int, c_double_p, c_double_p, ctypes.c_double]
    L.mmadmm_regrid_fields_device.argtypes = [ctypes.c_void_p, ctypes.c_int, ctypes.c_void_p, c_double_p,
                                              ctypes.c_double, ctypes.c_void_p]
    L.mmadmm_regrid_fields_huang.argtypes = [ctypes.c_void_p, ctypes.c_int, c_double_p, c_double_p, ctypes.c_double,
                                             c_double_p]
    L.mmadmm_regrid_fields_huang_device.argtypes = [ctypes.c_void_p, ctypes.c_int, ctypes.c_void_p, c_double_p,
                                                    ctypes.c_double, ctypes.c_void_p, c_double_p]
    L.mmadmm_field_hessians.argtypes = [ctypes.c_void_p, ctypes.c_int, c_double_p, c_double_p, c_double_p, c_double_p]
    L.mmadmm_field_hessians_device.argtypes = [ctypes.c_void_p, ctypes.c_int, ctypes.c_void_p, c_double_p,
                                               ctypes.c_void_p, ctypes.c_void_p, ctypes.c_void_p]
    L.mmadmm_fields_monitor.argtypes = [ctypes.c_int, ctypes.c_int, c_double_p, ctypes.c_int, c_int_p, ctypes.c_int,
                                        c_double_p, c_double_p, ctypes.c_double, ctypes.c_int, c_double_p, c_double_p,
                                        c_double_p, c_double_p]
    L.mmadmm_transfer.argtypes = [ctypes.c_void_p, c_double_p, c_double_p, ctypes.c_int, c_double_p, c_double_p,
                                  c_int_p, c_int_p]
    L.mmadmm_transfer_device.argtypes = [ctypes.c_void_p, ctypes.c_void_p, ctypes.c_void_p, ctypes.c_int,
                                         ctypes.c_void_p, ctypes.c_void_p, ctypes.c_void_p, c_int_p, ctypes.c_void_p]
    L.mmadmm_transfer_field.argtypes = [ctypes.c_int, ctypes.c_int, c_double_p, ctypes.c_int, c_int_p, c_double_p,
                                        ctypes.c_int, c_double_p, c_double_p, c_int_p, c_int_p]
    L.mmadmm_face_neighbours.argtypes = [ctypes.c_int, ctypes.c_int, ctypes.c_int, c_int_p, c_int_p]
    L.mmadmm_quality.argtypes = [ctypes.c_void_p, c_double_p, ctypes.c_int, c_double_p, c_double_p, c_double_p]
    L.mmadmm_quality_device.argtypes = [ctypes.c_void_p, ctypes.c_void_p, ctypes.c_int, ctypes.c_void_p,
                                        ctypes.c_void_p, c_double_p, ctypes.c_void_p]
    L.mmadmm_mesh_quality.argtypes = [ctypes.c_int, ctypes.c_int, c_double_p, c_double_p, ctypes.c_int, c_int_p,
                                      c_double_p, c_double_p, c_double_p, c_double_p]
    L.mmadmm_destroy.argtypes = [ctypes.c_void_p]
    L.mmadmm_mesh_rect.argtypes = [ctypes.c_int] * 4 + [ctypes.c_double] * 6 + [ctypes.c_int,
                                                                                 ctypes.POINTER(ctypes.c_void_p)]
    L.mmadmm_mesh_levelset2d.argtypes = [ctypes.c_int] * 2 + [ctypes.c_double] * 4 + [
        ctypes.c_int, ctypes.c_int, ctypes.POINTER(ctypes.c_void_p)]
    L.mmadmm_mesh_levelset3d.argtypes = [ctypes.c_int] * 3 + [ctypes.c_double] * 6 + [
        ctypes.c_int, ctypes.c_int, ctypes.POINTER(ctypes.c_void_p)]
    L.mmadmm_mesh_hexdisc.argtypes = [ctypes.c_int] + [ctypes.c_double] * 3 + [ctypes.c_int,
                                                                               ctypes.POINTER(ctypes.c_void_p)]
    L.mmadmm_mesh_shoulder.argtypes = [ctypes.c_int] * 4 + [ctypes.c_double] * 6 + [ctypes.c_int,
                                                                                     ctypes.POINTER(ctypes.c_void_p)]
    L.mmadmm_mesh_reference_points.argtypes = [ctypes.c_void_p, c_double_p]
    L.mmadmm_mesh_read.argtypes = [ctypes.c_int, ctypes.c_char_p, ctypes.c_char_p, ctypes.c_char_p,
                                   ctypes.POINTER(ctypes.c_void_p)]
    L.mmadmm_mesh_sizes.argtypes = [ctypes.c_void_p] + [ctypes.POINTER(ctypes.c_int)] * 4
    L.mmadmm_mesh_copy.argtypes = [ctypes.c_void_p, c_double_p, c_int_p, c_int_p]
    L.mmadmm_mesh_free.argtypes = [ctypes.c_void_p]
    L.mmadmm_write_points.argtypes = [ctypes.c_char_p, ctypes.c_int, ctypes.c_int, c_double_p]
    L.mmadmm_write_simplices.argtypes = [ctypes.c_char_p, ctypes.c_int, ctypes.c_int, c_int_p]
    L.mmadmm_debug_blockgrad.argtypes = [ctypes.c_void_p, ctypes.c_int, c_double_p, c_double_p, ctypes.c_int,
                                         c_double_p]
    L.mmadmm_devmath.argtypes = [ctypes.c_int, ctypes.c_int, c_double_p, c_double_p]
    vp = ctypes.c_void_p
    L.mmadmm_comm_unique_id.argtypes = [vp, ctypes.c_int]
    L.mmadmm_comm_create_rccl.argtypes = [ctypes.c_int, ctypes.c_int, vp, ctypes.c_int, ctypes.POINTER(vp)]
    L.mmadmm_comm_create_rccl_timeout.argtypes = [ctypes.c_int, ctypes.c_int, vp, ctypes.c_int, ctypes.c_double,
                                                  ctypes.POINTER(vp)]
    L.mmadmm_comm_create_loopback.argtypes = [ctypes.c_int, ctypes.POINTER(vp)]
    L.mmadmm_comm_destroy.argtypes = [vp]
    L.mmadmm_comm_nranks.argtypes = [vp, ctypes.POINTER(ctypes.c_int)]
    L.mmadmm_build_info.argtypes = [ctypes.c_char_p, ctypes.c_int]
    L.mmadmm_comm_create_host.argtypes = [ctypes.c_int, ctypes.c_int, ALLGATHER_FN, EXCHANGE_FN, vp, ctypes.POINTER(vp)]
    L.mmadmm_be_begin.argtypes = [vp, ctypes.c_double, c_double_p]
    L.mmadmm_be_residual.argtypes = [vp, ctypes.c_double, c_double_p, c_double_p, c_double_p]
    L.mmadmm_be_fsubjac.argtypes = [vp, c_double_p]
    L.mmadmm_be_add.argtypes = [vp, c_double_p]
    L.mmadmm_create_partitioned.argtypes = [ctypes.c_int, ctypes.c_int, c_double_p, c_double_p, ctypes.c_int, c_int_p,
                                            c_int_p, ctypes.POINTER(mmadmm_params), MONITOR_FN, vp, vp,
                                            ctypes.POINTER(vp)]
    L.mmadmm_local_nodes.argtypes = [vp, ctypes.POINTER(ctypes.c_int), c_int_p]
    L.mmadmm_plan_create.argtypes = [ctypes.c_int, ctypes.c_int, c_double_p, ctypes.c_int, c_int_p, ctypes.c_int,
                                     ctypes.c_int, ctypes.c_int, ctypes.POINTER(vp)]
    L.mmadmm_plan_sizes.argtypes = [vp] + [ctypes.POINTER(ctypes.c_int)] * 7
    L.mmadmm_plan_get.argtypes = [vp] + [c_int_p] * 6
    L.mmadmm_plan_destroy.argtypes = [vp]
    _lib = L
    return L


def build_info():
    buf = ctypes.create_string_buffer(256)
    _check(lib().mmadmm_build_info(buf, 256))
    return dict(kv.split("=", 1) for kv in buf.value.decode().split())


def _close_at_exit(obj):
# ... 881 lines not shown
```

Measured before the change: 2670.

## Run prox optimistically without fix kernel and replay from the first stuck iteration

For 2D single-rank deferred-reduction steps, the prox kernel launches without the follow-up k_prox_fix pass. Blocks that hit a tie set a device 'stuck' tag, and later prox and x-update launches bail out once it is set. After the step, the host reads the tag. If an iteration got stuck, it runs a 2D fix kernel for that iteration and replays the remaining iterations conservatively, with a back-off hold that doubles after each replay. The aim is to drop one kernel launch per iteration in the common tie-free case, at the cost of an extra host readback and full replays when ties occur.

Result: no change. 2662 (-0.3%).

```diff
diff --git a/include/mmadmm.h b/include/mmadmm.h
--- a/include/mmadmm.h
+++ b/include/mmadmm.h
@@ -68,6 +68,7 @@
   double halo_recv_bytes;
   int interior_nodes;
   int overlap;
+  long long tie_replays;
 } mmadmm_stats;
 
 int mmadmm_regrid(mmadmm_handle h, double t);
diff --git a/mm-admm_amd/csrc/host/engine.cpp b/mm-admm_amd/csrc/host/engine.cpp
--- a/mm-admm_amd/csrc/host/engine.cpp
+++ b/mm-admm_amd/csrc/host/engine.cpp
@@ -110,7 +110,8 @@
       : Fh_(orientedSimplices(nP, Xp, nF, F)),
         plan_(make_partition_plan(D, nP, Xp, nF, Fh_.data(), std::max(1, p.nranks), p.nranks > 1 ? p.rank : 0,
                                   p.partition)),
-        knobs_(EngineKnobs::from_env(D, (int)plan_.localSimplices.size(), std::max(1, p.nranks))) {
+        knobs_(EngineKnobs::from_env(D, (int)plan_.localSimplices.size(), std::max(1, p.nranks))),
+        loop_(LoopKnobs::from_env(D, std::max(1, p.nranks), knobs_)) {
     dim = D;
     prm_ = p;
     nranks_ = std::max(1, p.nranks);
@@ -277,8 +278,8 @@
     z_.alloc((size_t)nF_ * K * (kZUInterleaved ? 2 : 1));
     gcache_.alloc((size_t)nF_ * K);
     tieList_.alloc((size_t)nF_ / 16 + 1);
-    tieCount_.alloc(3);
-    MMX_HIP(hipMemsetAsync(tieCount_.p, 0, 3 * sizeof(unsigned), st_));
+    tieCount_.alloc(4);
+    MMX_HIP(hipMemsetAsync(tieCount_.p, 0, 4 * sizeof(unsigned), st_));
     if (!kZUInterleaved) u_.alloc((size_t)nF_ * K);
     gs_.alloc((size_t)nF_ * K);
     clearU();
@@ -375,10 +376,29 @@
     const size_t slice = maxBlocks_ * kNumPartials;
     if (deferRed && partA_.n < slice * nIters) partA_.alloc(slice * std::max(nIters, 10));
     int firstDeferred = 0;
+    const bool tieEligible = loop_.tieOpt && deferRed && nIters > 1;
+    const bool tieOpt = tieEligible && tieHold_ == 0;
+    if (tieEligible && tieHold_ > 0) --tieHold_;
+    unsigned* const stuckDev = tieCount_.p + 3;
+    double* const stuckOut = res_ + (size_t)resultsCap_ * 2 * kNumPartials;
+    if (tieOpt && tieDirty_) {
+      MMX_HIP(hipMemsetAsync(tieCount_.p, 0, 2 * sizeof(unsigned), st_));
+      tieDirty_ = false;
+    }
+    const bool hess0 = hessComputed_;
+    const int par0 = tiePar_;
+    const size_t timedBase = timed_.size();
+    const double proxTol = early ? tol / 100 : 1e-3 / 100;
+    auto gcSkipAt = [&](int i) { return (D == 2 && knobs_.gcSkip && !early && i == nIters - 1) ? 1 : 0; };
+    auto reduceSteps = [&](int i0, bool withStuck) {
+      launch_reduce_steps(partA_.p + slice * i0, slice, nbp, partB_.p, nbx, nIters - i0,
+                          res_ + (size_t)i0 * 2 * kNumPartials, st_, red_, withStuck ? stuckDev : nullptr,
+                          withStuck ? stuckOut : nullptr);
+    };
     hipEvent_t prevEnd = nullptr;
-    for (int i = 0; i < nIters; ++i) {
+    auto iterate = [&](int i, bool optimistic, bool timed) {
       hipEvent_t a0 = nullptr, a1 = nullptr, b1 = nullptr;
-      if (timing) {
+      if (timed) {
         a0 = prevEnd;
         if (!a0) {
           a0 = nextEvent();
@@ -391,21 +411,27 @@
         tiePar_ ^= 1;
         std::swap(m_.tieCount, m_.tieStale);
       }
-      m_.gcSkip = (D == 2 && knobs_.gcSkip && !early && i == nIters - 1) ? 1 : 0;
-      launch_prox<D>(m_, knobs_, !hessComputed_, gcacheValid_, early ? tol / 100 : 1e-3 / 100, x_.p, z_.p, uPtr(), B_.p,
-                     swapB ? B2_.p : B_.p, partA_.p + (deferRed ? slice * i : 0), &nbp, st_);
+      const bool noFix = optimistic && !firstProx;
+      if (!noFix && !firstProx) tieDirty_ = true;
+      m_.stuck = noFix ? stuckDev : nullptr;
+      m_.stuckTag = (unsigned)i + 1u;
+      m_.gcSkip = gcSkipAt(i);
+      launch_prox<D>(m_, knobs_, !hessComputed_, gcacheValid_, proxTol, x_.p, z_.p, uPtr(), B_.p,
+                     swapB ? B2_.p : B_.p, partA_.p + (deferRed ? slice * i : 0), &nbp, st_, !noFix);
       m_.zx = nullptr;
       if (swapB) std::swap(B_.p, B2_.p);
       gcacheValid_ = !m_.gcSkip;
-      if (timing) {
+      if (timed) {
         a1 = nextEvent();
         MMX_HIP(hipEventRecord(a1, st_));
       }
       hessComputed_ = true;
       stepTaken_ = true;
       const bool resid = early || i == nIters - 1;
+      if (!noFix && optimistic) m_.stuck = stuckDev;
       xupdateHalo(sc, &nbx, resid, true, PackZX{});
-      if (timing) {
+      m_.stuck = nullptr;
+      if (timed) {
         b1 = nextEvent();
         MMX_HIP(hipEventRecord(b1, st_));
         timed_.push_back({a0, a1, b1});
@@ -417,9 +443,7 @@
           launch_reduce_partials(partA_.p + slice * i, nbp, res_ + (size_t)i * 2 * kNumPartials, st_, red_);
           firstDeferred = i + 1;
         } else if (i == nIters - 1) {
-          const int i0 = firstProx ? i : firstDeferred;
-          launch_reduce_steps(partA_.p + slice * i0, slice, nbp, partB_.p, nbx, nIters - i0,
-                              res_ + (size_t)i0 * 2 * kNumPartials, st_, red_);
+          reduceSteps(firstProx ? i : firstDeferred, optimistic);
         }
       } else if (resid) {
         prevEnd = nullptr;
@@ -429,6 +453,9 @@
         prevEnd = nullptr;
         launch_reduce_partials(partA_.p, nbp, res_ + (size_t)i * 2 * kNumPartials, st_, red_);
       }
+    };
+    for (int i = 0; i < nIters; ++i) {
+      iterate(i, tieOpt, timing);
       done = i + 1;
       if (early) {
         std::vector<double> rv;
@@ -439,13 +466,44 @@
         if (r[4] > 0 || (primal < tol && dual < tol)) break;
       }
     }
-    MMX_HIP(hipMemcpyAsync(Vp_.p, x_.p, (size_t)nP_ * D * sizeof(double), hipMemcpyDeviceToDevice, st_));
+    auto stepEnd = [&] {
+      MMX_HIP(hipMemcpyAsync(Vp_.p, x_.p, (size_t)nP_ * D * sizeof(double), hipMemcpyDeviceToDevice, st_));
+      if (timing) {
+        eStep1 = nextEvent();
+        MMX_HIP(hipEventRecord(eStep1, st_));
+      }
+      fetchResults(res_, done, hostRes_);
+    };
+    stepEnd();
     vpVersion_++;
-    if (timing) {
-      eStep1 = nextEvent();
-      MMX_HIP(hipEventRecord(eStep1, st_));
-    }
-    fetchResults(res_, done, hostRes_);
+    if (const int at = tieOpt ? (int)fetchStuck(stuckOut) - 1 : -1; at >= 0) {
+      if (at >= nIters || !(hess0 || at > 0)) throw Error(MMADMM_ERR_INVALID, "step: a stuck iteration that ran no steady prox");
+      timed_.resize(std::min(timed_.size(), timedBase + (size_t)at));
+      tiePar_ = par0 ^ ((hess0 ? at + 1 : at) & 1);
+      m_.tieCount = tieCount_.p + tiePar_;
+      m_.tieStale = tieCount_.p + (tiePar_ ^ 1);
+      m_.zx = (at == 0 && zFromX) ? zsrc : nullptr;
+      m_.gcSkip = gcSkipAt(at);
+      m_.stuck = nullptr;
+      if constexpr (D == 2)
+        launch_prox_fix2d(m_, knobs_, proxTol, x_.p, z_.p, uPtr(), B_.p, partA_.p + slice * at, st_);
+      m_.zx = nullptr;
+      MMX_HIP(hipMemsetAsync(stuckDev, 0, sizeof(unsigned), st_));
+      gcacheValid_ = !m_.gcSkip;
+      xupdateHalo(sc, &nbx, at == nIters - 1, true, PackZX{});
+      if (at == nIters - 1) reduceSteps(firstDeferred, false);
+      for (int i = at + 1; i < nIters; ++i) iterate(i, false, false);
+      MMX_HIP(hipMemsetAsync(tieCount_.p, 0, 2 * sizeof(unsigned), st_));
+      tieDirty_ = false;
+      st_stats_.tie_replays += 1;
+      if (loop_.tieOpt == 2) {
+        tieHold_ = tieHoldLen_;
+        tieHoldLen_ = std::min(2 * tieHoldLen_, kTieHoldMax);
+      }
+      stepEnd();
+    } else if (tieOpt) {
+      tieHoldLen_ = kTieHold;
+    }
     MMX_HIP(hipGetLastError());
     bool bad = false;
     long long bf = 0;
@@ -711,7 +769,7 @@
     s->overlap = knobs_.overlap;
   }
 
-  std::string options() const override { return knobs_.text(); }
+  std::string options() const override { return knobs_.text() + loop_.text(); }
 
   void resetStats() override {
     resolveTimed();
@@ -899,6 +957,14 @@
       comm_->wait(st_);
     else
       MMX_HIP(hipStreamSynchronize(st_));
+  }
+
+  unsigned fetchStuck(const double* dev) {
+    if (resH_) return (unsigned)resH_[dev - res_];
+    double v = 0;
+    MMX_HIP(hipMemcpyAsync(&v, dev, sizeof(double), hipMemcpyDeviceToHost, st_));
+    streamWait();
+    return (unsigned)v;
   }
 
   void fetchResults(const double* dev, int rows, std::vector<double>& out) {
@@ -1653,6 +1719,7 @@
     m.tieCount = tieCount_.p + tiePar_;
     m.tieStale = tieCount_.p + (tiePar_ ^ 1);
     m.invFlag = tieCount_.p + 2;
+    m.xupRev = loop_.xupRev;
     m.nodeOrder = nodeOrder_.p;
     m.xupLo = 0;
     m.xupHi = nP_;
@@ -1709,7 +1776,7 @@
   void ensureResults(int nIters) {
     if (nIters <= resultsCap_) return;
     resultsCap_ = std::max(nIters, 64);
-    const size_t n = (size_t)resultsCap_ * 2 * kNumPartials;
+    const size_t n = (size_t)resultsCap_ * 2 * kNumPartials + 1;
     if (nranks_ == 1 && knobs_.spin) {
       if (resH_) MMX_HIP(hipHostFree(resH_));
       resH_ = nullptr;
@@ -1759,6 +1826,7 @@
   std::vector<int32_t> Fh_;
   PartitionPlan plan_;
   const EngineKnobs knobs_;
+  const LoopKnobs loop_;
   int nP_ = 0, nF_ = 0;
   mmadmm_params prm_{};
   bool compMesh_ = false;
@@ -1822,6 +1890,9 @@
   long long xupTail_ = 0;
   DevBuf<unsigned> tieCount_;
   int tiePar_ = 0;
+  int tieHold_ = 0;
+  int tieHoldLen_ = kTieHold;
+  bool tieDirty_ = false;
   Comm* comm_ = nullptr;
   int rank_ = 0, nranks_ = 1;
   int resultsCap_ = 0;
diff --git a/mm-admm_amd/csrc/host/knobs.h b/mm-admm_amd/csrc/host/knobs.h
--- a/mm-admm_amd/csrc/host/knobs.h
+++ b/mm-admm_amd/csrc/host/knobs.h
@@ -12,6 +12,8 @@
 constexpr int kXupEarlyDefault = 1;
 constexpr int kRedSplitMin = 4096;
 constexpr int kProxBlock = 64;
+constexpr int kTieHold = 8;
+constexpr int kTieHoldMax = 64;
 constexpr int kSweepGrid = 128;
 constexpr int kFacWaveChunk = 0;
 constexpr int kChainImportLat = 8;
@@ -137,6 +139,17 @@
    \
   X(int, schedProf, "MMX_SCHED_PROF", nullptr, env_set("MMX_SCHED_PROF"))
 
+#define MMX_LOOP_KNOBS(X) \
+   \
+   \
+   \
+   \
+   \
+  X(int, tieOpt, "MMX_TIE_OPT", nullptr, (D == 2 && nranks == 1 && !k.prox2dWave) ? knobs_detail::in_range_or(env_int("MMX_TIE_OPT", 2), 0, 2, 2) : 0) \
+   \
+   \
+  X(int, xupRev, "MMX_XUP_REV", nullptr, D == 2 && nranks == 1 && env_flag("MMX_XUP_REV", false))
+
 #define MMX_CHAIN_KNOBS(X) \
    \
   X(int, importLat, "MMX_CHAIN_LAT", nullptr, env_int("MMX_CHAIN_LAT", kChainImportLat, 0)) \
@@ -207,6 +220,23 @@
   }
 };
 
+struct LoopKnobs {
+  MMX_LOOP_KNOBS(MMX_KNOB_FIELD)
+
+  static LoopKnobs from_env(int D, int nranks, const EngineKnobs& k) {
+    LoopKnobs l{};
+#define MMX_LOOP_PARSE(type, member, name, words, parse) l.member = (parse);
+    MMX_LOOP_KNOBS(MMX_LOOP_PARSE)
+#undef MMX_LOOP_PARSE
+    return l;
+  }
+  std::string text() const {
+    std::string s;
+    MMX_LOOP_KNOBS(MMX_KNOB_PUT)
+    return s;
+  }
+};
+
 struct ChainKnobs {
   MMX_CHAIN_KNOBS(MMX_KNOB_FIELD)
 
diff --git a/mm-admm_amd/csrc/kernels/admm_kernels.h b/mm-admm_amd/csrc/kernels/admm_kernels.h
--- a/mm-admm_amd/csrc/kernels/admm_kernels.h
+++ b/mm-admm_amd/csrc/kernels/admm_kernels.h
@@ -55,6 +55,9 @@
   double powd, w;
   int compMesh;
   int prox2dWave;
+  unsigned* stuck;
+  unsigned stuckTag;
+  int xupRev;
 };
 
 struct StepScalars {
@@ -82,7 +85,10 @@
 bool prox_double_buffered(int D, bool wave2d);
 template <int D>
 void launch_prox(const DeviceMesh<D>& m, const EngineKnobs& k, bool first, bool useCache, double tol, const double* x,
-                 double* z, double* u, const double* Bin, double* Bout, double* partials, int* nblocks, hipStream_t st);
+                 double* z, double* u, const double* Bin, double* Bout, double* partials, int* nblocks, hipStream_t st,
+                 bool withFix = true);
+void launch_prox_fix2d(const DeviceMesh<2>& m, const EngineKnobs& k, double tol, const double* x, double* z, double* u,
+                       double* B, double* partials, hipStream_t st);
 template <int D>
 void launch_energy(const DeviceMesh<D>& m, const double* x, double* partials, int* nblocks,
                    hipStream_t st);
@@ -97,7 +103,8 @@
 };
 void launch_reduce_partials(const double* partials, int nblocks, double* out, hipStream_t st, const RedWork& w = {});
 void launch_reduce_steps(const double* partA, size_t stride, int nbA, const double* partB, int nbB, int n,
-                         double* results, hipStream_t st, const RedWork& w = {});
+                         double* results, hipStream_t st, const RedWork& w = {}, const unsigned* stuck = nullptr,
+                         double* stuckOut = nullptr);
 void launch_reduce_partials2(const double* partials, int nblocks, double* out, const double* partials2, int nblocks2,
                              double* out2, hipStream_t st, const RedWork& w = {});
 struct PackZX {
diff --git a/mm-admm_amd/csrc/kernels/admm_kernels_prox.hip b/mm-admm_amd/csrc/kernels/admm_kernels_prox.hip
--- a/mm-admm_amd/csrc/kernels/admm_kernels_prox.hip
+++ b/mm-admm_amd/csrc/kernels/admm_kernels_prox.hip
@@ -1,4 +1,5 @@
 #include <cstdio>
+#include <stdexcept>
 #include <vector>
 
 #include "admm_prox_common.h"
@@ -496,7 +497,7 @@
 #ifndef MMX_MON_HINT_BUILD
 #define MMX_MON_HINT_BUILD 1
 #endif
-template <int D, int BS>
+template <int D, int BS, bool STUCK = false>
 __global__ void __launch_bounds__(BS, 2) k_prox_lds(DeviceMesh<D> m, double tol, const double* __restrict__ x,
                                                         double* __restrict__ zg, double* __restrict__ ug,
                                                         double* __restrict__ Bg, double* __restrict__ partials,
@@ -510,6 +511,10 @@
   const int nIn = min(BS, m.nF - s0);
   const bool act = tid < nIn;
   const int s = act ? s0 + tid : s0;
+  if constexpr (STUCK) {
+    const unsigned stuckAt = *m.stuck;
+    if (stuckAt != 0u && stuckAt != m.stuckTag) return;
+  }
   int f[D + 1];
   loadVerts<D>(m, s, f);
   const unsigned fixedBits = m.sbits[s] & 0xF;
@@ -610,7 +615,10 @@
   }
   if (m.forceTie > 0 && tid == 0 && (int)((unsigned)lb % (unsigned)m.forceTie) == 0) tie = true;
   if (__syncthreads_or(tie ? 1 : 0)) {
-    if (tid == 0) m.tieList[atomicAdd(m.tieCount, 1u)] = lb;
+    if (tid == 0) {
+      m.tieList[atomicAdd(m.tieCount, 1u)] = lb;
+      if constexpr (STUCK) atomicMax(m.stuck, m.stuckTag);
+    }
     return;
   }
   if (act) {
@@ -828,7 +836,9 @@
 template <int D>
 void launch_prox(const DeviceMesh<D>& m, const EngineKnobs& k, bool first, bool useCache, double tol, const double* x,
                  double* z, double* u, const double* Bin, double* Bout, double* partials, int* nblocks,
-                 hipStream_t st) {
+                 hipStream_t st, bool withFix) {
+  if (!withFix && (first || D != 2 || m.prox2dWave || !m.stuck))
+    throw std::logic_error("launch_prox: only the steady k_prox_lds with DeviceMesh::stuck runs without k_prox_fix");
 #ifdef MMX_WAVE_PROF
   if (D == 3 && !first) wprof_arm((m.nF + 63) / 64);
 #endif
@@ -854,14 +864,23 @@
     *nblocks = (m.nF + bs - 1) / bs;
     const dim3 fg(std::min(*nblocks, kFixGrid));
     if (bs == 64) {
-      hipLaunchKernelGGL((k_prox_lds<D, 64>), dim3(*nblocks), dim3(64), 0, st, m, tol, x, z, u, B, partials, uc);
-      hipLaunchKernelGGL((k_prox_fix<D, 64>), fg, dim3(64), 0, st, m, tol, x, z, u, B, B, partials);
+      if (withFix)
+        hipLaunchKernelGGL((k_prox_lds<D, 64>), dim3(*nblocks), dim3(64), 0, st, m, tol, x, z, u, B, partials, uc);
+      else
+        hipLaunchKernelGGL((k_prox_lds<D, 64, true>), dim3(*nblocks), dim3(64), 0, st, m, tol, x, z, u, B, partials, uc);
+      if (withFix) hipLaunchKernelGGL((k_prox_fix<D, 64>), fg, dim3(64), 0, st, m, tol, x, z, u, B, B, partials);
     } else if (bs == 128) {
-      hipLaunchKernelGGL((k_prox_lds<D, 128>), dim3(*nblocks), dim3(128), 0, st, m, tol, x, z, u, B, partials, uc);
-      hipLaunchKernelGGL((k_prox_fix<D, 128>), fg, dim3(128), 0, st, m, tol, x, z, u, B, B, partials);
+      if (withFix)
+        hipLaunchKernelGGL((k_prox_lds<D, 128>), dim3(*nblocks), dim3(128), 0, st, m, tol, x, z, u, B, partials, uc);
+      else
+        hipLaunchKernelGGL((k_prox_lds<D, 128, true>), dim3(*nblocks), dim3(128), 0, st, m, tol, x, z, u, B, partials, uc);
+      if (withFix) hipLaunchKernelGGL((k_prox_fix<D, 128>), fg, dim3(128), 0, st, m, tol, x, z, u, B, B, partials);
     } else {
-      hipLaunchKernelGGL((k_prox_lds<D, 256>), dim3(*nblocks), dim3(256), 0, st, m, tol, x, z, u, B, partials, uc);
-      hipLaunchKernelGGL((k_prox_fix<D, 256>), fg, dim3(256), 0, st, m, tol, x, z, u, B, B, partials);
+      if (withFix)
+        hipLaunchKernelGGL((k_prox_lds<D, 256>), dim3(*nblocks), dim3(256), 0, st, m, tol, x, z, u, B, partials, uc);
+      else
+        hipLaunchKernelGGL((k_prox_lds<D, 256, true>), dim3(*nblocks), dim3(256), 0, st, m, tol, x, z, u, B, partials, uc);
+      if (withFix) hipLaunchKernelGGL((k_prox_fix<D, 256>), fg, dim3(256), 0, st, m, tol, x, z, u, B, B, partials);
     }
   } else {
     *nblocks = (m.nF + 63) / 64;
@@ -878,9 +897,21 @@
   }
 }
 template void launch_prox<2>(const DeviceMesh<2>&, const EngineKnobs&, bool, bool, double, const double*, double*,
-                             double*, const double*, double*, double*, int*, hipStream_t);
+                             double*, const double*, double*, double*, int*, hipStream_t, bool);
 template void launch_prox<3>(const DeviceMesh<3>&, const EngineKnobs&, bool, bool, double, const double*, double*,
-                             double*, const double*, double*, double*, int*, hipStream_t);
+                             double*, const double*, double*, double*, int*, hipStream_t, bool);
+void launch_prox_fix2d(const DeviceMesh<2>& m, const EngineKnobs& k, double tol, const double* x, double* z, double* u,
+                       double* B, double* partials, hipStream_t st) {
+  if (m.nF == 0) return;
+  const int bs = k.proxBlock;
+  const dim3 fg(std::min((m.nF + bs - 1) / bs, kFixGrid));
+  if (bs == 64)
+    hipLaunchKernelGGL((k_prox_fix<2, 64>), fg, dim3(64), 0, st, m, tol, x, z, u, B, B, partials);
+  else if (bs == 128)
+    hipLaunchKernelGGL((k_prox_fix<2, 128>), fg, dim3(128), 0, st, m, tol, x, z, u, B, B, partials);
+  else
+    hipLaunchKernelGGL((k_prox_fix<2, 256>), fg, dim3(256), 0, st, m, tol, x, z, u, B, B, partials);
+}
 }
 
 #ifdef MMX_WAVE_PROF
diff --git a/mm-admm_amd/csrc/kernels/admm_kernels_step.hip b/mm-admm_amd/csrc/kernels/admm_kernels_step.hip
--- a/mm-admm_amd/csrc/kernels/admm_kernels_step.hip
+++ b/mm-admm_amd/csrc/kernels/admm_kernels_step.hip
@@ -224,24 +224,32 @@
   else
     xup_head_csr<D, CH>(m, idx, h);
 }
-template <int D, bool RESID, bool TS, bool ZX = false, bool PRED = false, bool REM = false, bool REC = false>
+template <int D, bool RESID, bool TS, bool ZX = false, bool PRED = false, bool REM = false, bool REC = false,
+          bool LOOP = false>
 __global__ void __launch_bounds__(kBlock) k_xupdate(DeviceMesh<D> m, StepScalars sc,
                                                      const double* __restrict__ xBar,
                                                      const double* __restrict__ z,
                                                      const double* __restrict__ u, double* __restrict__ x,
                                                      double* __restrict__ partials, int xcd) {
   constexpr int CH = (D == 2 ? MMX_XU_CH2D : 8);
-  const int lb = logical_block(xcd);
+  int lb = logical_block(xcd);
+  unsigned stuckAt = 0u;
+  if constexpr (LOOP) {
+    if (m.stuck) stuckAt = *m.stuck;
+    if (m.xupRev) lb = (int)gridDim.x - 1 - lb;
+  }
   const int idx = m.xupLo + lb * kBlock + threadIdx.x;
   double pv[3] = {0, 0, 0};
   if (idx < m.xupHi) {
     XupHead<CH> h;
     xup_head<D, CH, REC>(m, idx, h);
+    if (stuckAt != 0u) return;
     xupdate_node<D, RESID, TS, CH, ZX, PRED, REM>(m, sc, xBar, z, u, x, h, pv);
   }
+  if (stuckAt != 0u) return;
   if constexpr (RESID) block_partials<3>(pv, partials, lb);
 }
-template <int D, bool TS, int CH, bool RESID = false, bool REC = false, bool EARLY = false>
+template <int D, bool TS, int CH, bool RESID = false, bool REC = false, bool EARLY = false, bool LOOP = false>
 __global__ void __launch_bounds__(kBlock) k_xupdate_sweep(DeviceMesh<D> m, StepScalars sc,
                                                            const double* __restrict__ xBar,
                                                            const double* __restrict__ z, const double* __restrict__ u,
@@ -251,21 +259,31 @@
   const int lo = m.xupLo + c * n8, hi = min(lo + n8, m.xupHi);
   double pv[3], r2 = 0.0;
   int idx = lo + w * kBlock + (int)threadIdx.x;
+  unsigned stuckAt = 0u;
+  int mir = -1;
+  if constexpr (LOOP) {
+    if (m.stuck) stuckAt = *m.stuck;
+    if constexpr (!RESID)
+      if (m.xupRev) mir = lo + hi - 1;
+  }
+  auto pos = [mir](int i) { return mir >= 0 ? mir - i : i; };
   if constexpr (EARLY) {
     XupHead<CH> cur, nxt;
-    if (idx < hi) xup_head<D, CH, true>(m, idx, cur);
+    if (idx < hi) xup_head<D, CH, true>(m, pos(idx), cur);
+    if (stuckAt != 0u) return;
     nxt = cur;
     for (; idx < hi; idx += per * kBlock) {
-      if (idx + per * kBlock < hi) xup_head<D, CH, true>(m, idx + per * kBlock, nxt);
+      if (idx + per * kBlock < hi) xup_head<D, CH, true>(m, pos(idx + per * kBlock), nxt);
       __builtin_amdgcn_sched_barrier(0);
       xupdate_node<D, RESID, TS, CH>(m, sc, xBar, z, u, x, cur, pv);
       if constexpr (RESID) r2 += pv[2];
       cur = nxt;
     }
   } else {
+    if (stuckAt != 0u) return;
     for (; idx < hi; idx += per * kBlock) {
       XupHead<CH> h;
-      xup_head<D, CH, REC>(m, idx, h);
+      xup_head<D, CH, REC>(m, pos(idx), h);
       xupdate_node<D, RESID, TS, CH>(m, sc, xBar, z, u, x, h, pv);
       if constexpr (RESID) r2 += pv[2];
     }
@@ -355,8 +373,15 @@
 
 __global__ void __launch_bounds__(kRed) k_reduce_steps(const double* __restrict__ partA, size_t stride, int nbA,
                                                         const double* __restrict__ partB, int nbB, int n,
-                                                        double* __restrict__ results) {
+                                                        double* __restrict__ results,
+                                                        const unsigned* __restrict__ stuck,
+                                                        double* __restrict__ stuckOut) {
   const int i = blockIdx.x;
+  if (stuck) {
+    const unsigned at = *stuck;
+    if (i == 0 && threadIdx.x == 0) *stuckOut = (double)at;
+    if (at != 0u) return;
+  }
   if (i < n)
     reduce_set(partA + (size_t)i * stride, nbA, results + (size_t)i * 2 * kNumPartials);
   else
@@ -366,8 +391,10 @@
 constexpr int kRedLanes = 256;
 __global__ void __launch_bounds__(kRedLanes) k_reduce_split(const double* __restrict__ partA, size_t stride, int nbA,
                                                             int nA, const double* __restrict__ partB, int nbB,
-                                                            double* __restrict__ scratch) {
+                                                            double* __restrict__ scratch,
+                                                            const unsigned* __restrict__ stuck) {
   __shared__ double red[kRedLanes / 64][kNumPartials];
+  if (stuck && *stuck != 0u) return;
   const int q = (int)blockIdx.x / kRedSplit, r = (int)blockIdx.x % kRedSplit;
   const bool isA = q < nA;
   const double* p = isA ? partA + (size_t)q * stride : partB;
@@ -397,8 +424,15 @@
 }
 __global__ void __launch_bounds__(64) k_reduce_combine(const double* __restrict__ scratch, int nA,
                                                        double* __restrict__ outA, size_t outStride,
-                                                       double* __restrict__ outB) {
+                                                       double* __restrict__ outB,
+                                                       const unsigned* __restrict__ stuck,
+                                                       double* __restrict__ stuckOut) {
   const int q = (int)blockIdx.x, t = (int)threadIdx.x;
+  if (stuck) {
+    const unsigned at = *stuck;
+    if (q == 0 && t == 0) *stuckOut = (double)at;
+    if (at != 0u) return;
+  }
   if (t >= kNumPartials) return;
   const double* base = scratch + (size_t)q * kRedSplit * kNumPartials + t;
   double acc = base[0];
@@ -478,6 +512,7 @@
   const bool ts = useTslot && m.tslot;
   const bool rem = m.remote != nullptr;
   const bool rec = m.xrec != nullptr;
+  const bool loop = D == 2 && (m.stuck || m.xupRev);
   auto needCols = [&](int ch) {
     if (rec && m.xslotCh < ch) throw std::logic_error("launch_xupdate: the slot table has fewer columns than the chunk");
   };
@@ -504,14 +539,18 @@
       constexpr bool TS = decltype(tsT)::value, RS = decltype(residT)::value;
       constexpr int CH = decltype(chT)::value;
       needCols(CH);
-      if (rec && m.xupEarly)
-        hipLaunchKernelGGL((k_xupdate_sweep<D, TS, CH, RS, true, true>), g, dim3(kBlock), 0, st, m, sc, xBar, z, u, x, n8,
-                           part);
-      else if (rec)
-        hipLaunchKernelGGL((k_xupdate_sweep<D, TS, CH, RS, true, false>), g, dim3(kBlock), 0, st, m, sc, xBar, z, u, x, n8,
-                           part);
-      else
-        hipLaunchKernelGGL((k_xupdate_sweep<D, TS, CH, RS>), g, dim3(kBlock), 0, st, m, sc, xBar, z, u, x, n8, part);
+      dispatch_bool(loop, [&](auto lp) {
+        constexpr bool LP = D == 2 && decltype(lp)::value;
+        if (rec && m.xupEarly)
+          hipLaunchKernelGGL((k_xupdate_sweep<D, TS, CH, RS, true, true, LP>), g, dim3(kBlock), 0, st, m, sc, xBar, z, u,
+                             x, n8, part);
+        else if (rec)
+          hipLaunchKernelGGL((k_xupdate_sweep<D, TS, CH, RS, true, false, LP>), g, dim3(kBlock), 0, st, m, sc, xBar, z, u,
+                             x, n8, part);
+        else
+          hipLaunchKernelGGL((k_xupdate_sweep<D, TS, CH, RS, false, false, LP>), g, dim3(kBlock), 0, st, m, sc, xBar, z,
+                             u, x, n8, part);
+      });
     };
     using T = std::true_type;
     using F = std::false_type;
@@ -532,8 +571,11 @@
   dispatch_bool(resid, [&](auto r) {
     dispatch_bool(ts, [&](auto t) {
       dispatch_bool(rec, [&](auto rc) {
-        hipLaunchKernelGGL((k_xupdate<D, decltype(r)::value, decltype(t)::value, false, false, false, decltype(rc)::value>),
-                           dim3(*nblocks), dim3(kBlock), 0, st, m, sc, xBar, z, u, x, partials, k.xcdMap);
+        dispatch_bool(loop, [&](auto lp) {
+          hipLaunchKernelGGL((k_xupdate<D, decltype(r)::value, decltype(t)::value, false, false, false,
+                                        decltype(rc)::value, D == 2 && decltype(lp)::value>),
+                             dim3(*nblocks), dim3(kBlock), 0, st, m, sc, xBar, z, u, x, partials, k.xcdMap);
+        });
       });
     });
   });
@@ -555,11 +597,13 @@
 }
 static bool split_ok(const RedWork& w, int nblocks) { return w.scratch && nblocks >= w.splitMin; }
 static void reduce_split(const double* partA, size_t stride, int nbA, int nA, double* outA, size_t outStride,
-                         const double* partB, int nbB, double* outB, const RedWork& w, hipStream_t st) {
+                         const double* partB, int nbB, double* outB, const RedWork& w, hipStream_t st,
+                         const unsigned* stuck = nullptr, double* stuckOut = nullptr) {
   const int sets = nA + (nbB >= 0 ? 1 : 0);
   hipLaunchKernelGGL(k_reduce_split, dim3(sets * kRedSplit), dim3(kRedLanes), 0, st, partA, stride, nbA, nA, partB,
-                     nbB, w.scratch);
-  hipLaunchKernelGGL(k_reduce_combine, dim3(sets), dim3(64), 0, st, w.scratch, nA, outA, outStride, outB);
+                     nbB, w.scratch, stuck);
+  hipLaunchKernelGGL(k_reduce_combine, dim3(sets), dim3(64), 0, st, w.scratch, nA, outA, outStride, outB, stuck,
+                     stuckOut);
 }
 void launch_reduce_partials(const double* partials, int nblocks, double* out, hipStream_t st, const RedWork& w) {
   if (split_ok(w, nblocks))
@@ -568,12 +612,13 @@
     hipLaunchKernelGGL(k_reduce_partials, dim3(1), dim3(kRed), 0, st, partials, nblocks, out, partials, nblocks, out);
 }
 void launch_reduce_steps(const double* partA, size_t stride, int nbA, const double* partB, int nbB, int n,
-                         double* results, hipStream_t st, const RedWork& w) {
+                         double* results, hipStream_t st, const RedWork& w, const unsigned* stuck, double* stuckOut) {
   if (split_ok(w, nbA) && n + 1 <= kRedSets)
     reduce_split(partA, stride, nbA, n, results, (size_t)2 * kNumPartials, partB, nbB,
-                 results + (size_t)(n - 1) * 2 * kNumPartials + kNumPartials, w, st);
+                 results + (size_t)(n - 1) * 2 * kNumPartials + kNumPartials, w, st, stuck, stuckOut);
   else
-    hipLaunchKernelGGL(k_reduce_steps, dim3(n + 1), dim3(kRed), 0, st, partA, stride, nbA, partB, nbB, n, results);
+    hipLaunchKernelGGL(k_reduce_steps, dim3(n + 1), dim3(kRed), 0, st, partA, stride, nbA, partB, nbB, n, results,
+                       stuck, stuckOut);
 }
 void launch_reduce_partials2(const double* partials, int nblocks, double* out, const double* partials2, int nblocks2,
                              double* out2, hipStream_t st, const RedWork& w) {
diff --git a/mm-admm_amd/python/mmadmm_amd.py b/mm-admm_amd/python/mmadmm_amd.py
--- a/mm-admm_amd/python/mmadmm_amd.py
+++ b/mm-admm_amd/python/mmadmm_amd.py
@@ -43,7 +43,7 @@
                 ("regrid_fallbacks", ctypes.c_longlong), ("monitor_iso", ctypes.c_int),
                 ("t_exchange_ms", ctypes.c_double), ("n_exchange", ctypes.c_longlong),
                 ("halo_send_bytes", ctypes.c_double), ("halo_recv_bytes", ctypes.c_double),
-                ("interior_nodes", ctypes.c_int), ("overlap", ctypes.c_int)]
+                ("interior_nodes", ctypes.c_int), ("overlap", ctypes.c_int), ("tie_replays", ctypes.c_longlong)]
 
     def as_dict(self):
         return {k: getattr(self, k) for k, _ in self._fields_}
diff --git a/profiles/r10/tie_opt/step_gaps.py b/profiles/r10/tie_opt/step_gaps.py
--- /dev/null
+++ b/profiles/r10/tie_opt/step_gaps.py
@@ -0,0 +1,35 @@
+import csv
+import statistics
+import sys
+
+rows = []
+with open(sys.argv[1]) as f:
+    for r in csv.DictReader(f):
+        rows.append((int(r["Start_Timestamp"]), int(r["End_Timestamp"]), r["Kernel_Name"],
+                     int(r.get("Grid_Size") or r["Grid_Size_X"])))
+rows.sort()
+steps, cur = [], []
+for r in rows:
+    cur.append(r)
+    if "k_reduce_combine" in r[2] or "k_reduce_steps" in r[2]:
+        steps.append(cur)
+        cur = []
+C3_GRID = 1997632
+steady = [s for s in steps if sum(1 for r in s if "k_prox_lds" in r[2] and r[3] == C3_GRID) == 10]
+if not steady:
+    sys.exit("no steady C3 step in the trace")
+n = [len(s) for s in steady]
+busy = [sum(r[1] - r[0] for r in s) / 1e3 for s in steady]
+gaps = [sum(max(0, b[0] - a[1]) for a, b in zip(s, s[1:])) / 1e3 for s in steady]
+span = [(s[-1][1] - s[0][0]) / 1e3 for s in steady]
+print(f"steady C3 steps: {len(steady)}")
+print(f"launches per step: median {statistics.median(n)} (min {min(n)}, max {max(n)})")
+print(f"kernel time per step: median {statistics.median(busy):.1f} us")
+print(f"gaps between the step's kernels: median {statistics.median(gaps):.1f} us (min {min(gaps):.1f}, max {max(gaps):.1f})")
+print(f"first launch to last end: median {statistics.median(span):.1f} us")
+names = {}
+for s in steady:
+    for r in s:
+        names[r[2][:70]] = names.get(r[2][:70], 0) + 1
+for k, v in sorted(names.items(), key=lambda kv: -kv[1]):
+    print(f"  {v / len(steady):6.2f} per step  {k}")
diff --git a/profiles/r10/tie_opt/tie_counts.py b/profiles/r10/tie_opt/tie_counts.py
--- /dev/null
+++ b/profiles/r10/tie_opt/tie_counts.py
@@ -0,0 +1,23 @@
+import json
+import os
+import sys
+
+ROOT = os.path.dirname(os.path.dirname(os.path.dirname(os.path.dirname(os.path.abspath(__file__)))))
+sys.path.insert(0, os.path.join(ROOT, "mm-admm_amd", "python"))
+import mmadmm_amd as mx
+
+WORK = [("c3", lambda: mx.MeshData.hexdisc(577, 0.5, 0.5, 0.5), 50.0, 23),
+        ("c2", lambda: mx.MeshData.rect(2, 223), 50.0, 23),
+        ("bfgs_heavy_rho1", lambda: mx.MeshData.rect(2, 707), 1.0, 5)]
+for name, mk, rho, steps in WORK:
+    m = mk()
+    E = mx.Engine(mx.Mesh(m.Xp, m.F, m.mask, mx.BuiltinMonitor(2, 1), rho=rho, tau=0.5), 0.055)
+    assert E.options()["MMX_TIE_OPT"] == "1", "run with MMX_TIE_OPT=1: every step with a queued block replays"
+    per_step = []
+    for _ in range(steps):
+        before = E.stats()["tie_replays"]
+        E.step(10, -1.0)
+        per_step.append(E.stats()["tie_replays"] - before)
+    print(json.dumps({"workload": name, "nodes": E.nP, "simplices": E.nF, "steps": steps,
+                      "steps_with_queued_blocks": sum(per_step), "per_step": per_step}), flush=True)
+    E.close()
```
